# BoxLib-Codes/VARDEN

Measured on AMD Instinct MI355X. Metric: cells*steps/sec on advance_timestep, higher is better.
Workload: dtype f64; 1 GPU; 3D 256x256x256 single-level variable-density bubble, 1 box(es) of 256^3, MAC+HG projection each step (BASELINE.json configs[1]); parallelism=single GPU, cells=16777216

## Files before the change

### varden_amd/csrc/advance.hip

```cpp
#include "vdn_dev.h"
#include <chrono>
#include <cmath>

static double wall() { return std::chrono::duration<double>(std::chrono::steady_clock::now().time_since_epoch()).count(); }
static void sync() { HIPCHK(hipStreamSynchronize(ctx().stream)); }


static void restrict_and_fill(int nlev, vdn_multifab **mf, int icomp, int bcomp, int nc, bool same_boundary, const vdn_bc_tower *bct) {
  if (nlev == 1) mf_restrict_and_fill(mf[0], icomp, bcomp, nc, same_boundary, bct);
  else ml_restrict_and_fill(nlev, mf, icomp, bcomp, nc, same_boundary, bct);
}

static void dbg_phase_hash(const char *tag, int nlevs, vdn_multifab **mfs, int per_level = 1, bool whole = false) {
  if (!sw().phase_hash) return;
  HIPCHK(hipStreamSynchronize(ctx().stream));
  unsigned long long h = 1469598103934665603ull;
  for (int n = 0; n < nlevs; n++) for (int q = 0; q < per_level; q++) {
    const vdn_multifab *m = mfs[per_level == 1 ? n : 3 * n + q];
    if (!m) continue;
    std::vector<unsigned long long> buf(m->bytes / 8);
    HIPCHK(hipMemcpy(buf.data(), m->base, m->bytes, hipMemcpyDeviceToHost));
    for (int b = 0; b < m->nfabs(); b++) {
      const FV &f = m->fabs[b]; vdn_box vb = m->vbox[b];
      if (whole) for (int d = 0; d < 3; d++) { vb.lo[d] -= m->ng; vb.hi[d] += m->ng; }
      const size_t off = (size_t)(f.p - m->base);
      unsigned long long hb = 1469598103934665603ull;
      for (int c = 0; c < m->nc; c++)
        for (int k = vb.lo[2]; k <= vb.hi[2] + m->nodal[2]; k++) for (int j = vb.lo[1]; j <= vb.hi[1] + m->nodal[1]; j++) for (int i = vb.lo[0]; i <= vb.hi[0] + m->nodal[0]; i++) {
          { const unsigned long long v_ = buf[off + (size_t)(i - f.a0) + (size_t)f.n0 * ((size_t)(j - f.a1) + (size_t)f.n1 * (size_t)(k - f.a2)) + (size_t)c * (size_t)f.sc]; hb ^= v_; hb *= 1099511628211ull; }
          const unsigned long long v = buf[off + (size_t)(i - f.a0) + (size_t)f.n0 * ((size_t)(j - f.a1) + (size_t)f.n1 * (size_t)(k - f.a2)) + (size_t)c * (size_t)f.sc];
          h ^= v; h *= 1099511628211ull;
        }
      if (whole) fprintf(stderr, "PHASEBOX %-20s lev %d box %3d (%d,%d,%d)-(%d,%d,%d) %016llx\n", tag, n, b, m->vbox[b].lo[0], m->vbox[b].lo[1], m->vbox[b].lo[2], m->vbox[b].hi[0], m->vbox[b].hi[1], m->vbox[b].hi[2], hb);
    }
  }
  fprintf(stderr, "PHASE %-22s %016llx\n", tag, h);
  if (per_level == 3) {
    for (int n = 0; n < nlevs; n++) for (int q = 0; q < 3; q++) {
      const vdn_multifab *m = mfs[3 * n + q];
      std::vector<unsigned long long> buf(m->bytes / 8);
      HIPCHK(hipMemcpy(buf.data(), m->base, m->bytes, hipMemcpyDeviceToHost));
      for (int b = 0; b < m->nfabs(); b++) {
        const FV &f = m->fabs[b]; const vdn_box &vb = m->vbox[b];
        const size_t off = (size_t)(f.p - m->base);
        unsigned long long hb = 1469598103934665603ull; long nan = 0;
        for (int k = vb.lo[2]; k <= vb.hi[2] + m->nodal[2]; k++) for (int j = vb.lo[1]; j <= vb.hi[1] + m->nodal[1]; j++) for (int i = vb.lo[0]; i <= vb.hi[0] + m->nodal[0]; i++) {
          const unsigned long long v = buf[off + (size_t)(i - f.a0) + (size_t)f.n0 * ((size_t)(j - f.a1) + (size_t)f.n1 * (size_t)(k - f.a2))];
          hb ^= v; hb *= 1099511628211ull;
          double dv; memcpy(&dv, &v, 8); if (dv != dv) nan++;
        }
        fprintf(stderr, "PHASEBOX %-20s lev %d dir %d box %3d (%d,%d,%d)-(%d,%d,%d) %016llx nan %ld\n", tag, n, q, b, vb.lo[0], vb.lo[1], vb.lo[2], vb.hi[0], vb.hi[1], vb.hi[2], hb, nan);
      }
    }
  }
}
extern "C" int vdn_advance_timestep(int istep, vdn_layout *mla, vdn_multifab **sold, vdn_multifab **uold,
                                    vdn_multifab **snew, vdn_multifab **unew, vdn_multifab **gp, vdn_multifab **p,
                                    vdn_multifab **ext_vel_force, vdn_multifab **ext_scal_force,
                                    const vdn_bc_tower *bct, double dt, double time, const double *dx,
                                    int press_comp, int proj_type) {
  VDN_TRY
  (void)istep; (void)time;
  REQUIRE(ctx().inited, "vdn_init has not been called");
  REQUIRE(mla && mla->nlev >= 1 && mla->nlev <= VDN_MAXLEV, "advance_timestep: 1..%d levels are implemented (nlevel = %d)", VDN_MAXLEV, mla ? mla->nlev : -1);
  const vdn_params &P = ctx().prm;
  const int dm = P.dm, nscal = P.nscal, nlevs = mla->nlev;
  const bool viscous = P.visc_coef > 0.0, diffusive = P.diff_coef > 0.0;
  REQUIRE(nlevs == 1 || dm == 3, "advance_timestep: multi-level hierarchies are implemented for dm = 3");
  REQUIRE(press_comp == dm + nscal + 1, "press_comp must be dm+nscal+1 (got %d)", press_comp);
  for (int n = 0; n < nlevs; n++) {
    REQUIRE(uold[n]->ng >= 3 && sold[n]->ng >= 3 && unew[n]->ng >= 3 && snew[n]->ng >= 3, "state needs ng_cell = 3");
    REQUIRE(gp[n]->ng >= 1 && p[n]->ng >= 1 && ext_vel_force[n]->ng >= 1 && ext_scal_force[n]->ng >= 1, "gp/p/ext forces need ng = 1");
    REQUIRE(sold[n]->nc == nscal, "sold must have nscal (= %d) components (got %d)", nscal, sold[n]->nc);
  }
  dbg_phase_hash("uold at entry", nlevs, uold); dbg_phase_hash("sold at entry", nlevs, sold); dbg_phase_hash("gp at entry", nlevs, gp);
  dbg_phase_hash("uold+ghosts at entry", nlevs, uold, 1, true); dbg_phase_hash("sold+ghosts at entry", nlevs, sold, 1, true); dbg_phase_hash("gp+ghosts at entry", nlevs, gp, 1, true);
  Prof prof_advance("advance");
  arena_reset();
  arena_reserve_for(mla);
  const double t_begin = wall();
  #define DXL(n) (dx + (n) * dm)

  vdn_multifab *mac_rhs[VDN_MAXLEV], *rhohalf[VDN_MAXLEV], *umac[3 * VDN_MAXLEV] = { nullptr }, *lapu[VDN_MAXLEV] = { nullptr };
  for (int n = 0; n < nlevs; n++) {
    mac_rhs[n] = mf_temp(mla, n, 1, 1, -1, true, 0.0);
    rhohalf[n] = mf_temp(mla, n, dm, 1, -1, false, 0.0);
    mf_setval(rhohalf[n], 0.0, 0, 1, true);
    for (int d = 0; d < dm; d++) umac[3 * n + d] = mf_temp(mla, n, 1, 1, d, true, 1.e20);
    if (viscous) {
      lapu[n] = mf_temp(mla, n, dm, 0, -1, true, 0.0);
      for (int c = 0; c < dm; c++) k_explicit_diffusive_term(lapu[n], uold[n], c, c, DXL(n), bct);
    }
  }
  if (viscous) for (int n = nlevs - 1; n >= 1; n--) ml_cc_restriction(lapu[n - 1], lapu[n], 0, dm);
  ctx().drop_step_caches();
  if (nlevs == 1 && dm == 3 && god_per_box(uold[0]) && !sw().no_slope_cache) {
    const int nb = uold[0]->nfabs();
    for (int d = 0; d < 3; d++) ctx().slope_cache[d].assign(nb, nullptr);
    ctx().slope_src.assign(nb, nullptr); ctx().macmax_cache.assign(nb, nullptr); ctx().macmax_src.assign(nb, nullptr);
    for (int ib = 0; ib < nb; ib++) {
      const vdn_box &b = uold[0]->vbox[ib];
      const size_t fld = (size_t)(b.hi[0] - b.lo[0] + 3) * (b.hi[1] - b.lo[1] + 3) * (b.hi[2] - b.lo[2] + 3) * sizeof(double);
      for (int d = 0; d < 3; d++) ctx().slope_cache[d][ib] = (double *)arena_alloc(fld * 3);
      ctx().macmax_cache[ib] = (double *)arena_alloc(256);
    }
  }

  const bool force_reuse = !sw().no_force_reuse;
  const bool keep_vel_force = force_reuse && !(viscous && P.diffusion_type == 2);
  vdn_multifab *vel_force0[VDN_MAXLEV] = { nullptr };
  if (keep_vel_force) for (int n = 0; n < nlevs; n++) vel_force0[n] = mf_temp(mla, n, dm, 1, -1, false, 0.0);
  {
    Prof pr("advance_premac");
    size_t mark = arena_mark();
    vdn_multifab *vel_force[VDN_MAXLEV];
    for (int n = 0; n < nlevs; n++) {
      vel_force[n] = keep_vel_force ? vel_force0[n] : mf_temp(mla, n, dm, 1, -1, false, 0.0);
      k_mkvelforce(vel_force[n], ext_vel_force[n], sold[n], gp[n], lapu[n], 1.0);
    }
    restrict_and_fill(nlevs, vel_force, 0, bct->extrap_comp0(), dm, true, bct);
    for (int n = 0; n < nlevs; n++) k_velpred(uold[n], umac + 3 * n, vel_force[n], DXL(n), dt, bct);
    for (int d = 0; d < dm; d++) mf_fill_boundary(umac[d]);
    for (int n = 1; n < nlevs; n++) for (int d = 0; d < dm; d++) { ml_create_umac_grown(umac[3 * n + d], umac[3 * (n - 1) + d], d); mf_fill_boundary(umac[3 * n + d]); }
    for (int n = nlevs - 1; n >= 1; n--) for (int d = 0; d < dm; d++) ml_edge_restriction(umac[3 * (n - 1) + d], umac[3 * n + d], d);
    dbg_phase_hash("vel_force", nlevs, vel_force); dbg_phase_hash("umac after velpred", nlevs, umac, 3);
    if (!keep_vel_force) for (int n = nlevs - 1; n >= 0; n--) mf_temp_free(vel_force[n]);
    arena_release(mark);
  }

  sync(); double t0 = wall();
  { Prof pr("MAC_Project");
  do_macproject(mla, umac, sold, mac_rhs, dx, bct, press_comp - 1);
  }
  sync(); ctx().step_sec[2] = wall() - t0;
  dbg_phase_hash("umac after MAC", nlevs, umac, 3);

  t0 = wall();
  {
    Prof pr("Scalar_update");
    size_t mark = arena_mark();
    int is_cons[VDN_MAXCOMP]; is_cons[0] = 1; for (int c = 1; c < nscal; c++) is_cons[c] = 0;
    vdn_multifab *scal_force[VDN_MAXLEV], *divu[VDN_MAXLEV], *sflux[3 * VDN_MAXLEV], *sedge[3 * VDN_MAXLEV], *laps[VDN_MAXLEV] = { nullptr };
    if (diffusive) {
      for (int n = 0; n < nlevs; n++) {
        laps[n] = mf_temp(mla, n, nscal, 0, -1, true, 0.0);
        for (int c = 1; c < nscal; c++) k_explicit_diffusive_term(laps[n], sold[n], c, dm + c, DXL(n), bct);
      }
      for (int n = nlevs - 1; n >= 1; n--) ml_cc_restriction(laps[n - 1], laps[n], 1, nscal - 1);
    }
    for (int n = 0; n < nlevs; n++) {
      scal_force[n] = mf_temp(mla, n, nscal, 1, -1, false, 0.0);
      divu[n] = mac_rhs[n];
      for (int d = 0; d < dm; d++) { sflux[3 * n + d] = mf_temp(mla, n, nscal, 0, d, nlevs > 1, 0.0); sedge[3 * n + d] = mf_temp(mla, n, nscal, 0, d, false, 0.0); }
      k_mkscalforce(scal_force[n], ext_scal_force[n], laps[n], 1.0);
    }
    restrict_and_fill(nlevs, scal_force, 0, bct->extrap_comp0(), nscal, true, bct);
    bool s_updated = false;
    for (int n = 0; n < nlevs; n++) {
      MkUpdate U; U.snew = snew[n]; U.fmode = 0;
      const bool try_upd = force_reuse && nlevs == 1 && dm == 3 && !diffusive;
      s_updated = k_mkflux(sold[n], sedge + 3 * n, sflux + 3 * n, umac + 3 * n, scal_force[n], divu[n], DXL(n), dt, bct, false, is_cons, try_upd ? &U : nullptr);
      if (diffusive || !force_reuse) k_mkscalforce(scal_force[n], ext_scal_force[n], laps[n], 0.0);
    }
    for (int n = nlevs - 1; n >= 1; n--) for (int c = 0; c < nscal; c++) if (is_cons[c]) for (int d = 0; d < dm; d++) ml_edge_restriction(sflux[3 * (n - 1) + d], sflux[3 * n + d], d, c);
    if (diffusive || !force_reuse) restrict_and_fill(nlevs, scal_force, 0, bct->extrap_comp0(), nscal, true, bct);
    dbg_phase_hash("sedge after mkflux", nlevs, sedge, 3); dbg_phase_hash("sflux restricted", nlevs, sflux, 3); dbg_phase_hash("scal_force", nlevs, scal_force);
    if (!s_updated) for (int n = 0; n < nlevs; n++) k_update(sold[n], umac + 3 * n, sedge + 3 * n, sflux + 3 * n, scal_force[n], snew[n], DXL(n), dt, false, is_cons);
    dbg_phase_hash("snew before r_and_f", nlevs, snew);
    restrict_and_fill(nlevs, snew, 0, dm, nscal, false, bct);
    if (diffusive) {
      const double visc_mu = (P.diffusion_type == 1) ? 0.5 * dt * P.diff_coef : dt * P.diff_coef;
      for (int c = 1; c < nscal; c++) {
        if (nlevs == 1) do_diff_scalar_solve(mla, snew[0], laps[0], dx, visc_mu, bct, c, dm + c);
        else do_ml_diff_scalar_solve(mla, snew, laps, dx, visc_mu, bct, c, dm + c);
      }
    }
    arena_release(mark);
  }
  sync(); ctx().step_sec[0] = wall() - t0;
  dbg_phase_hash("snew after scalars", nlevs, snew);

  { Prof pr("make_at_halftime"); for (int n = 0; n < nlevs; n++) k_make_at_halftime(rhohalf[n], sold[n], snew[n], 0, 0); }
  restrict_and_fill(nlevs, rhohalf, 0, dm + 0, 1, false, bct);
  if (viscous && P.diffusion_type == 2) for (int n = 0; n < nlevs; n++) mf_setval(lapu[n], 0.0, 0, dm, true);

  t0 = wall();
  {
    Prof pr("Velocity_update");
    size_t mark = arena_mark();
    int is_cons[3] = { 0, 0, 0 };
    vdn_multifab *vel_force[VDN_MAXLEV], *uflux[3 * VDN_MAXLEV], *uedge[3 * VDN_MAXLEV];
    for (int n = 0; n < nlevs; n++) {
      vel_force[n] = keep_vel_force ? vel_force0[n] : mf_temp(mla, n, dm, 1, -1, false, 0.0);
      for (int d = 0; d < dm; d++) { uflux[3 * n + d] = mf_temp(mla, n, dm, 0, d, false, 0.0); uedge[3 * n + d] = mf_temp(mla, n, dm, 0, d, false, 0.0); }
      if (!keep_vel_force) k_mkvelforce(vel_force[n], ext_vel_force[n], sold[n], gp[n], lapu[n], 1.0);
    }
    if (!keep_vel_force) restrict_and_fill(nlevs, vel_force, 0, bct->extrap_comp0(), dm, true, bct);
    const bool fuse_force = force_reuse && nlevs == 1 && dm == 3;
    bool u_updated = false;
    for (int n = 0; n < nlevs; n++) {
      MkUpdate U; U.snew = unew[n]; U.fmode = 1; U.ext = ext_vel_force[n]; U.gp = gp[n]; U.rho = rhohalf[n]; U.lapu0 = P.visc_coef * 0.0 * 0.0;
      const bool try_upd = fuse_force && !viscous && P.boussinesq == 0;
      u_updated = k_mkflux(uold[n], uedge + 3 * n, uflux + 3 * n, umac + 3 * n, vel_force[n], mac_rhs[n], DXL(n), dt, bct, true, is_cons, try_upd ? &U : nullptr);
      if (!fuse_force) k_mkvelforce(vel_force[n], ext_vel_force[n], rhohalf[n], gp[n], lapu[n], 0.0);
    }
    dbg_phase_hash("uedge after mkflux", nlevs, uedge, 3); dbg_phase_hash("vel_force (update)", nlevs, vel_force);
    if (u_updated) {  }
    else if (fuse_force) k_update_velforce(uold[0], umac, uedge, ext_vel_force[0], rhohalf[0], gp[0], lapu[0], 0.0, unew[0], DXL(0), dt);
    else {
      restrict_and_fill(nlevs, vel_force, 0, bct->extrap_comp0(), dm, true, bct);
      for (int n = 0; n < nlevs; n++) k_update(uold[n], umac + 3 * n, uedge + 3 * n, uflux + 3 * n, vel_force[n], unew[n], DXL(n), dt, true, is_cons);
    }
    dbg_phase_hash("unew before r_and_f", nlevs, unew);
    restrict_and_fill(nlevs, unew, 0, 0, dm, false, bct);
    dbg_phase_hash("unew after update", nlevs, unew);
    if (viscous) {
      const double visc_mu = (P.diffusion_type == 1) ? 0.5 * dt * P.visc_coef : dt * P.visc_coef;
      if (nlevs == 1) do_visc_solve(mla, unew[0], lapu[0], rhohalf[0], mac_rhs[0], dx, visc_mu, bct);
      else do_ml_visc_solve(mla, unew, lapu, rhohalf, mac_rhs, dx, visc_mu, bct);
    }
    arena_release(mark);
  }
  sync(); ctx().step_sec[1] = wall() - t0;
  dbg_phase_hash("unew after viscous", nlevs, unew);

  t0 = wall();
  { Prof pr("HG_Project");
  do_hgproject(proj_type, mla, unew, uold, rhohalf, p, gp, dx, dt, bct, press_comp - 1); }
  sync(); ctx().step_sec[3] = wall() - t0;
  dbg_phase_hash("unew after HG", nlevs, unew); dbg_phase_hash("p after HG", nlevs, p); dbg_phase_hash("gp after HG", nlevs, gp);
  #undef DXL

  arena_reset();
  ctx().drop_step_caches();
  ctx().step_sec[4] = wall() - t_begin;
  if (P.verbose >= 1 && ctx().rank == 0) {
    printf(" Timing summary:\n Scalar   update: %g seconds\n Velocity update: %g seconds\n  MAC Projection: %g seconds\n   HG Projection: %g seconds\n\n",
           ctx().step_sec[0], ctx().step_sec[1], ctx().step_sec[2], ctx().step_sec[3]);
  }
  VDN_CATCH
}

extern "C" int vdn_estdt(int lev, const vdn_multifab *u, const vdn_multifab *s, const vdn_multifab *gp,
                         const vdn_multifab *ext, const double *dx, double dtold, double *dt_out) {
  VDN_TRY
  (void)lev;
  double m[6];
  k_estdt_max(u, s, gp, ext, m);
  for (int q = 0; q < 6; q++) REQUIRE(m[q] < HUGE_VAL, "estdt: non-finite velocity or pressure-gradient term (the state has blown up)");
  const double eps = (double)1.0e-8f;
  double dt = 1.e20;
  if (m[0] > eps) dt = fmin(dt, dx[0] / m[0]);
  if (m[1] > eps) dt = fmin(dt, dx[1] / m[1]);
  const int dm = ctx().prm.dm;
  if (dm == 3 && m[2] > eps) dt = fmin(dt, dx[2] / m[2]);
  if (m[3] > eps) dt = fmin(dt, sqrt(2.0 * dx[0] / m[3]));
  if (m[4] > eps) dt = fmin(dt, sqrt(2.0 * dx[1] / m[4]));
  if (dm == 3 && m[5] > eps) dt = fmin(dt, sqrt(2.0 * dx[2] / m[5]));
  if (dt == 1.e20) { dt = fmin(dx[0], dx[1]); if (dm == 3) dt = fmin(dt, dx[2]); }
  dt = dt * ctx().prm.cflfac;
  if (dtold > 0.0) dt = fmin(dt, ctx().prm.max_dt_growth * dtold);
  *dt_out = dt;
  VDN_CATCH
}

extern "C" int vdn_hgproject(int proj_type, vdn_layout *mla, vdn_multifab **unew, vdn_multifab **uold,
                             vdn_multifab **rhohalf, vdn_multifab **p, vdn_multifab **gp,
                             const double *dx, double dt, const vdn_bc_tower *bct, int press_comp) {
  VDN_TRY
  REQUIRE(mla && mla->nlev <= VDN_MAXLEV, "hgproject: at most %d levels are implemented (nlevel = %d)", VDN_MAXLEV, mla ? mla->nlev : -1);
  arena_reset(); arena_reserve_for(mla);
  do_hgproject(proj_type, mla, unew, uold, rhohalf, p, gp, dx, dt, bct, press_comp - 1);
  arena_reset();
  VDN_CATCH
}
extern "C" int vdn_macproject(vdn_layout *mla, vdn_multifab **umac, vdn_multifab **rho, vdn_multifab **mac_rhs,
                              const double *dx, const vdn_bc_tower *bct, int bc_comp) {
  VDN_TRY
  REQUIRE(mla && mla->nlev <= VDN_MAXLEV, "macproject: at most %d levels are implemented (nlevel = %d)", VDN_MAXLEV, mla ? mla->nlev : -1);
  arena_reset(); arena_reserve_for(mla);
  do_macproject(mla, umac, rho, mac_rhs, dx, bct, bc_comp - 1);
  arena_reset();
  VDN_CATCH
}

#define HOOK_BEGIN(mf) VDN_TRY REQUIRE(ctx().inited, "vdn_init has not been called"); arena_reset(); arena_reserve_for((mf)->la);
#define HOOK_END arena_reset(); VDN_CATCH

extern "C" int vdn_k_slope(const vdn_multifab *s, vdn_multifab *slope, int dir, int bccomp, const vdn_bc_tower *bct) {
  HOOK_BEGIN(s) k_slope(s, slope, dir, bccomp, bct); HOOK_END
}
extern "C" int vdn_k_velpred(const vdn_multifab *u, vdn_multifab **umac, const vdn_multifab *force, const double *dx, double dt,
                             const vdn_bc_tower *bct) {
  HOOK_BEGIN(u)
  k_velpred(u, umac, force, dx, dt, bct);
  for (int d = 0; d < ctx().prm.dm; d++) mf_fill_boundary(umac[d]);
  HOOK_END
}
extern "C" int vdn_k_mkflux(const vdn_multifab *s, vdn_multifab **sedge, vdn_multifab **flux, vdn_multifab **umac,
                            const vdn_multifab *force, const vdn_multifab *mac_rhs, const double *dx, double dt,
                            const vdn_bc_tower *bct, int is_vel, const int *is_cons) {
  HOOK_BEGIN(s) k_mkflux(s, sedge, flux, umac, force, mac_rhs, dx, dt, bct, is_vel != 0, is_cons); HOOK_END
}
extern "C" int vdn_k_update(const vdn_multifab *sold, vdn_multifab **umac, vdn_multifab **sedge, vdn_multifab **flux,
                            const vdn_multifab *force, vdn_multifab *snew, const double *dx, double dt,
                            int is_vel, const int *is_cons, const vdn_bc_tower *bct) {
  HOOK_BEGIN(sold)
  k_update(sold, umac, sedge, flux, force, snew, dx, dt, is_vel != 0, is_cons);
  mf_restrict_and_fill(snew, 0, is_vel ? 0 : bct->dm, snew->nc, false, bct);
  HOOK_END
}
extern "C" int vdn_k_mkvelforce(vdn_multifab *vf, const vdn_multifab *ext, const vdn_multifab *s, const vdn_multifab *gp,
                                const vdn_multifab *lapu, double visc_fac, const vdn_bc_tower *bct) {
  HOOK_BEGIN(vf)
  k_mkvelforce(vf, ext, s, gp, lapu, visc_fac);
  mf_restrict_and_fill(vf, 0, bct->extrap_comp0(), vf->nc, true, bct);
  HOOK_END
}
// ... 71 lines not shown
```

### varden_amd/csrc/mg_cc.hip

```cpp
#include "vdn_dev.h"
#include "mg_stop.h"
#include "krylov_wg.h"
#include "krylov_grid.h"
#include <chrono>
#include <tuple>
#include <algorithm>

struct CLev {
  int n[3]; int PX, PY; long sz;
  double hi2[3];
  double *phi, *rh, *res, *b[3];
  double *alpha;
  const double *rho;
  int fold[3][2];
  double cmu;
};
DEVI long cidx(const CLev &L, int i, int j, int k) { return (long)(i + 16) + (long)L.PX * ((long)(j + 1) + (long)L.PY * (long)(k + 1)); }

DEVI double beta_of(double ra, double rb, bool at_face, int e) {
  double v = 2.0 / (ra + rb);
  if (at_face) { if (e == VDN_BC_NEU) v = 0.0; else if (e == VDN_BC_DIR) v = 2.0 * v; }
  return v;
}
template <bool RHO = false> DEVI void cc_apply(const CLev &L, long c, double &Ap, double &diag, int i = 0, int j = 0, int k = 0) {
// ... 868 lines not shown
  const long sy = F.PX, sz = (long)F.PX * F.PY;
  const long f = cidx(F, 2 * i, 2 * j, 2 * k);
  double s = src[f] + src[f + 1] + src[f + sy] + src[f + sy + 1] + src[f + sz] + src[f + sz + 1] + src[f + sz + sy] + src[f + sz + sy + 1];
  dst[cidx(C, i, j, k)] = s * 0.125;
}

__global__ void kk_cc_store(CLev L, FV phi, int lo0, int lo1, int lo2, int ebc00, int ebc01, int ebc10, int ebc11, int ebc20, int ebc21, int add = 0, FV acc = FV()) {
  const int i = (int)(blockIdx.x * blockDim.x + threadIdx.x) - 1;
  const int j = (int)(blockIdx.y * blockDim.y + threadIdx.y) - 1;
  const int k = (int)blockIdx.z - 1;
  if (i > L.n[0] || j > L.n[1] || k > L.n[2]) return;
  const int out = (i < 0) + (i == L.n[0]) + (j < 0) + (j == L.n[1]) + (k < 0) + (k == L.n[2]);
  if (out > 1) return;
  double v;
  if (out == 0) v = L.phi[cidx(L, i, j, k)];
  else {
    int e; int qi = i, qj = j, qk = k;
    if (i < 0) { e = ebc00; qi = 0; } else if (i == L.n[0]) { e = ebc01; qi = L.n[0] - 1; }
    else if (j < 0) { e = ebc10; qj = 0; } else if (j == L.n[1]) { e = ebc11; qj = L.n[1] - 1; }
    else if (k < 0) { e = ebc20; qk = 0; } else { e = ebc21; qk = L.n[2] - 1; }
    if (e == VDN_BC_NEU) v = L.phi[cidx(L, qi, qj, qk)];
    else if (e == VDN_BC_DIR) v = -L.phi[cidx(L, qi, qj, qk)];
    else v = L.phi[cidx(L, i, j, k)];
  }
  fv_at(phi, lo0 + i, lo1 + j, lo2 + k) = v;
  if (add && out == 0) fv_at(acc, lo0 + i, lo1 + j, lo2 + k) = fv_get(acc, lo0 + i, lo1 + j, lo2 + k) + v;
}


__global__ void kk_cc_restrict_pack(CLev F, const double *r, double *buf, long off, int nx, int ny, int nz) {
  const int i = blockIdx.x * blockDim.x + threadIdx.x;
  const int j = blockIdx.y * blockDim.y + threadIdx.y;
  const int k = blockIdx.z;
  if (i >= nx || j >= ny) return;
  const long sy = F.PX, sz = (long)F.PX * F.PY;
  const long f = cidx(F, 2 * i, 2 * j, 2 * k);
  double s = r[f] + r[f + 1] + r[f + sy] + r[f + sy + 1] + r[f + sz] + r[f + sz + 1] + r[f + sz + sy] + r[f + sz + sy + 1];
  buf[off + i + (long)nx * (j + (long)ny * k)] = s * 0.125;
}
__global__ void kk_cc_coarsen_b_pack(CLev F, double *buf, long off, int nx, int ny, int nz) {
  const int i = blockIdx.x * blockDim.x + threadIdx.x;
  const int j = blockIdx.y * blockDim.y + threadIdx.y;
  const int k = blockIdx.z;
  if (i > nx || j > ny || k > nz) return;
  const long sy = F.PX, sz = (long)F.PX * F.PY;
  const long f = cidx(F, 2 * i, 2 * j, 2 * k);
  const long o1 = off + (long)(nx + 1) * ny * nz, o2 = o1 + (long)nx * (ny + 1) * nz;
  if (j < ny && k < nz) buf[off + i + (long)(nx + 1) * (j + (long)ny * k)] = (F.b[0][f] + F.b[0][f + sy] + F.b[0][f + sz] + F.b[0][f + sz + sy]) * 0.25;
  if (i < nx && k < nz) buf[o1 + i + (long)nx * (j + (long)(ny + 1) * k)] = (F.b[1][f] + F.b[1][f + 1] + F.b[1][f + sz] + F.b[1][f + sz + 1]) * 0.25;
  if (i < nx && j < ny) buf[o2 + i + (long)nx * (j + (long)ny * k)] = (F.b[2][f] + F.b[2][f + 1] + F.b[2][f + sy] + F.b[2][f + sy + 1]) * 0.25;
}
__global__ void kk_cc_unpack_rh(CLev T, double *dst, const double *buf, const GBox *gb) {
  const GBox g = gb[blockIdx.z];
  const int tot = g.n[0] * g.n[1] * g.n[2];
  for (int t = blockIdx.x * blockDim.x + threadIdx.x; t < tot; t += gridDim.x * blockDim.x) {
    const int i = t % g.n[0], j = (t / g.n[0]) % g.n[1], k = t / (g.n[0] * g.n[1]);
    const long cc = cidx(T, g.c0[0] + i, g.c0[1] + j, g.c0[2] + k);
    dst[cc] = buf[g.off + t];
    T.phi[cc] = 0.0;
  }
}
__global__ void kk_cc_unpack_b(CLev T, const double *buf, const GBox *gb) {
  const GBox g = gb[blockIdx.z];
  const int nx = g.n[0], ny = g.n[1], nz = g.n[2];
  const long n0 = (long)(nx + 1) * ny * nz, n1 = (long)nx * (ny + 1) * nz, n2 = (long)nx * ny * (nz + 1);
  for (long t = blockIdx.x * blockDim.x + threadIdx.x; t < n0 + n1 + n2; t += gridDim.x * blockDim.x) {
    int d; long u = t;
    if (u < n0) d = 0; else if (u < n0 + n1) { d = 1; u -= n0; } else { d = 2; u -= n0 + n1; }
    const int ex = nx + (d == 0), ey = ny + (d == 1);
    const int i = (int)(u % ex), j = (int)((u / ex) % ey), k = (int)(u / ((long)ex * ey));
    T.b[d][cidx(T, g.c0[0] + i, g.c0[1] + j, g.c0[2] + k)] = buf[g.off + t];
  }
}
__global__ void kk_cc_prolong_tail(CLev F, CLev T, int c00, int c01, int c02) {
  const int i = blockIdx.x * blockDim.x + threadIdx.x;
  const int j = blockIdx.y * blockDim.y + threadIdx.y;
  const int k = blockIdx.z;
  if (i >= F.n[0] || j >= F.n[1]) return;
  const long f = cidx(F, i, j, k);
  F.phi[f] = F.phi[f] + T.phi[cidx(T, c00 + (i >> 1), c01 + (j >> 1), c02 + (k >> 1))];
}

struct ProlongLinArgs { int c0[3]; int e[3][2]; };
__global__ void kk_cc_prolong_lin(CLev F, CLev C, ProlongLinArgs A) {
  const int i = blockIdx.x * blockDim.x + threadIdx.x;
  const int j = blockIdx.y * blockDim.y + threadIdx.y;
  const int k = blockIdx.z;
  if (i >= F.n[0] || j >= F.n[1]) return;
  const int I = A.c0[0] + (i >> 1), J = A.c0[1] + (j >> 1), K = A.c0[2] + (k >> 1);
  const long sy = C.PX, sz = (long)C.PX * C.PY;
  const long c = cidx(C, I, J, K);
  const double p0 = C.phi[c];
  double px, py, pz;
  #define NBV(out, q, odd, n, elo, ehi, stride)                                                             \
    { const int m = (q) + ((odd) ? 1 : -1);                                                                 \
      const int t = m < 0 ? (elo) : (m >= (n) ? (ehi) : VDN_BC_INT);                                         \
      out = (t == VDN_BC_NEU) ? p0 : ((t == VDN_BC_DIR) ? -p0 : C.phi[c + ((odd) ? (stride) : -(stride))]); }
  NBV(px, I, i & 1, C.n[0], A.e[0][0], A.e[0][1], 1L)
  NBV(py, J, j & 1, C.n[1], A.e[1][0], A.e[1][1], sy)
  NBV(pz, K, k & 1, C.n[2], A.e[2][0], A.e[2][1], sz)
  #undef NBV
  F.phi[cidx(F, i, j, k)] = 0.25 * (((p0 + px) + py) + pz);
}

struct CBox { CLev L; int lo[3]; int gidx; int hmask = 63;
              CSplit sp;  };
struct CDLev { std::vector<CBox> boxes; XPlan *halo = nullptr; int ng[3];  bool single_box = false;
               bool res_restricted = false;
               bool split = false;
               XPlan *shalo[2] = { nullptr, nullptr };
               std::vector<XBoxInfo> xb; vdn_box lpd; unsigned long la_uid = 0; int la_lev = 0;       };
struct CCMG {
  std::vector<CDLev> dlev;
  std::vector<CLev> tail;
  int per[3];
  double *d_nrm;
  MgGather g_rh, g_b; GBox *d_gb_rh = nullptr, *d_gb_b = nullptr;
  double *sendbuf = nullptr, *recvbuf = nullptr;
  MgKrylov kry; int kry_singular = 0;
  CcKrylov krylov(const CLev &L) const { return CcKrylov{ L, { per[0], per[1], per[2] }, kry_singular }; }
};

static dim3 g3(int nx, int ny, int nz, dim3 b) { return dim3((nx + b.x - 1) / b.x, (ny + b.y - 1) / b.y, nz); }
static const dim3 BLK(64, 4, 1);

template <int ADD> static inline void launch_gsrb_split(const CBox &B, int color, hipStream_t st, const CLev &C, int k0 = 0, int k1 = -1, int hm = 0) {
  const CLev &L = B.L;
  if (k1 < 0) k1 = L.n[2];
  const dim3 g((unsigned)((L.n[0] / 4 + 63) / 64), (unsigned)((L.n[1] + 7) / 8), (unsigned)(k1 - k0));
  if (L.cmu > 0.0) hipLaunchKernelGGL((kk_cc_gsrb_rho_split<ADD, true>), g, dim3(64, 8, 1), 0, st, L, B.sp, color, C, (sw().mac_kflip && color) ? 1 : 0, k0, hm);
  else hipLaunchKernelGGL((kk_cc_gsrb_rho_split<ADD, false>), g, dim3(64, 8, 1), 0, st, L, B.sp, color, C, (sw().mac_kflip && color) ? 1 : 0, k0, hm);
}
static inline void launch_residual_split_rst(const CLev &L, const CSplit &S, double *nrm, const CLev &C, int Ka, int Kb, hipStream_t st) {
  const dim3 g((unsigned)((L.n[0] / 4 + 63) / 64), (unsigned)((L.n[1] / 2 + 3) / 4), (unsigned)std::min(Kb - Ka, 16));
  if (L.cmu > 0.0) hipLaunchKernelGGL(kk_cc_residual_rho_split_rst<true>, g, BLK, 0, st, L, S, nrm, C, Ka, Kb);
  else hipLaunchKernelGGL(kk_cc_residual_rho_split_rst<false>, g, BLK, 0, st, L, S, nrm, C, Ka, Kb);
}
static inline void launch_gsrb_split_shell(const CBox &B, int color, hipStream_t st, int hm) {
  if (!hm) return;
  const CLev &L = B.L;
  const int m = std::max(L.n[0], std::max(L.n[1], L.n[2]));
  hipLaunchKernelGGL(kk_cc_gsrb_split_shell, dim3((unsigned)((m + 63) / 64), (unsigned)((m + 3) / 4), (unsigned)__builtin_popcount(hm)), dim3(64, 4, 1), 0, st, L, B.sp, color, hm);
}
static void cc_to_split(const CDLev &DL, int what) {
  for (const CBox &B : DL.boxes) {
    const CLev &L = B.L;
    const dim3 g((unsigned)((B.sp.PXH + 63) / 64), (unsigned)((L.n[1] + 2 + 3) / 4), (unsigned)(L.n[2] + 2));
    hipLaunchKernelGGL(kk_cc_to_split, g, BLK, 0, ctx().stream, L, B.sp, what);
  }
}
static void cc_from_split(const CDLev &DL) {
  for (const CBox &B : DL.boxes) hipLaunchKernelGGL(kk_cc_from_split, g3(B.L.n[0] / 2, B.L.n[1], B.L.n[2], BLK), BLK, 0, ctx().stream, B.L, B.sp);
}
static void split_halo(const CDLev &DL, int colour, hipStream_t st = nullptr) { if (DL.shalo[colour]) xplan_run(DL.shalo[colour], st); }
static bool cc_split_ok(const CCMG &M) {
  if (!sw().mac_split || !sw().mg_restrict_fused || !sw().mg_prolong_fused || M.dlev.size() < 2 || ctx().prm.mg_nu1 < 1 || ctx().prm.mg_nu2 < 1) return false;
  const CDLev &D0 = M.dlev[0];
  if (D0.boxes.empty() || D0.boxes.size() != M.dlev[1].boxes.size()) return false;
  long cells = 0;
  for (const CBox &B : D0.boxes) {
    const CLev &L = B.L;
    if (!((L.rho || (L.cmu > 0.0 && L.alpha)) && cc_pair_level_z(L) && L.n[0] % 4 == 0)) return false;
    for (int d = 0; d < 3; d++) if (B.lo[d] & 1) return false;
    cells += (long)L.n[0] * L.n[1] * L.n[2];
  }
  for (int d = 0; d < 3; d++) if (D0.ng[d] & 1) return false;
  return cells >= sw().mac_split_min;
}
static int g_mac_level_form = 0;
extern "C" int vdn_last_mac_level_form(void) { return g_mac_level_form; }
static XPlan *cc_split_plan(const CDLev &D0, int colour, const int per[3]);
static void cc_split_setup(CCMG &M) {
  CDLev &D0 = M.dlev[0];
  for (CBox &B : D0.boxes) {
    const CLev &L = B.L;
    CSplit &S = B.sp;
    const int off = 16, rnd = 16;
    S.off = off;
    S.PXH = ((L.n[0] / 2 + off + 2 + rnd - 1) / rnd) * rnd; S.sy = S.PXH; S.sz = (long)S.PXH * (L.n[1] + 2); S.tot = S.sz * (L.n[2] + 2);
    double *base = (double *)arena_alloc(sizeof(double) * S.tot * 6);
    for (int c = 0; c < 2; c++) { S.phi[c] = base + c * S.tot; S.rh[c] = base + (2 + c) * S.tot; S.rho[c] = base + (4 + c) * S.tot; }
  }
  D0.split = true;
  if (D0.halo) for (int c = 0; c < 2; c++) D0.shalo[c] = cc_split_plan(D0, c, M.per);
  cc_to_split(D0, 2 | 4);
// ... 24 lines not shown
static const int CC_HALO = 4;

static XPlan *cc_split_plan(const CDLev &D0, int colour, const int per[3]) {
  std::vector<XBoxInfo> xb = D0.xb;
  size_t li = 0;
  GraphKey hk;
  for (XBoxInfo &x : xb) {
    const int nh = (x.vhi[0] - x.vlo[0] + 1) / 2;
    x.vlo[0] /= 2; x.vhi[0] = x.vlo[0] + nh - 1;
    if (x.owner == ctx().rank) {
      const CBox &B = D0.boxes[li++];
      const CSplit &S = B.sp;
      FV f; f.p = S.phi[colour]; f.a0 = x.vlo[0] - S.off; f.a1 = x.vlo[1] - 1; f.a2 = x.vlo[2] - 1; f.n0 = S.PXH; f.n1 = B.L.n[1] + 2; f.n2 = B.L.n[2] + 2; f.sc = S.tot;
      x.fv = f; hk.put(f.p); hk.put(S.tot);
    }
  }
  vdn_box lpd = D0.lpd; lpd.hi[0] = (lpd.hi[0] + 1) / 2 - 1;
  const MgHaloKey key{ D0.la_uid, (const void *)D0.boxes[0].sp.phi[colour], D0.la_lev, 1000 + colour, CC_HALO, per[0] | (per[1] << 1) | (per[2] << 2), hk.h };
  return mg_halo_plan(key, xb, lpd, per, sw().cc_halo_faces);
}

int mg_agglom(const vdn_layout *la, int lev) {
  if (sw().mg_agglom > 0) return sw().mg_agglom;
  bool all_local = true;
  for (int o : la->owner[lev]) if (o != ctx().rank) all_local = false;
  return (all_local && !comm_active()) ? 128 : 64;
}

MgPlan mg_plan_of(const vdn_layout *la, int lev) {
  return mg_plan(la->boxes[lev].data(), la->owner[lev].data(), (int)la->boxes[lev].size(), la->pd[lev], ctx().nranks, ctx().rank, mg_agglom(la, lev));
}
static void cc_build(CCMG &M, const vdn_multifab *rh, const double *dx, const int bc[3][2], bool has_alpha) {
  Prof prof_("cc_build");
  const vdn_layout *la = rh->la; const int lev = rh->lev;
  const int nb = (int)la->boxes[lev].size();
  for (int d = 0; d < 3; d++) M.per[d] = (bc[d][0] == VDN_BC_PER);
  const MgPlan P = mg_plan_of(la, lev);
  REQUIRE(P.err.empty(), "cc multigrid: %s", P.err.c_str());
  double h[3] = { dx[0], dx[1], dx[2] };
  for (const MgDistLevel &PL : P.dist) {
    const int *n = PL.n;
    CDLev DL;
    std::vector<XBoxInfo> xb;
    for (int g = 0; g < nb; g++) {
      XBoxInfo x; memset(&x, 0, sizeof x);
      const int *lo = PL.lo[g].data();
      for (int d = 0; d < 3; d++) { x.vlo[d] = lo[d]; x.vhi[d] = lo[d] + n[d] - 1; }
      x.owner = la->owner[lev][g];
      if (x.owner == ctx().rank) {
        CBox B; B.L = cc_alloc_lev(n, h, has_alpha); B.gidx = g;
        for (int d = 0; d < 3; d++) B.lo[d] = lo[d];
        x.fv = cc_phi_view(B.L, lo);
        DL.boxes.push_back(B);
      }
      xb.push_back(x);
    }
    vdn_box lpd; for (int d = 0; d < 3; d++) { lpd.lo[d] = 0; lpd.hi[d] = PL.ng[d] - 1; DL.ng[d] = PL.ng[d]; }
    for (CBox &B : DL.boxes) {
      B.hmask = 0;
      for (int d = 0; d < 3; d++) {
        if (B.lo[d] > 0 || M.per[d]) B.hmask |= 1 << (2 * d);
        if (B.lo[d] + B.L.n[d] < DL.ng[d] || M.per[d]) B.hmask |= 2 << (2 * d);
      }
    }
    if (nb > 1 || M.per[0] || M.per[1] || M.per[2]) {
      GraphKey hk; for (const CBox &B : DL.boxes) { hk.put(B.L.phi); hk.put(B.L.sz); }
      const MgHaloKey key{ la->uid, DL.boxes.empty() ? nullptr : (const void *)DL.boxes[0].L.phi, lev, (int)M.dlev.size(), CC_HALO, M.per[0] | (M.per[1] << 1) | (M.per[2] << 2), hk.h };
      DL.halo = mg_halo_plan(key, xb, lpd, M.per, sw().cc_halo_faces);
    }
    DL.single_box = (nb == 1);
    DL.xb = xb; DL.lpd = lpd; DL.la_uid = la->uid; DL.la_lev = lev;
    M.dlev.push_back(DL);
    for (int d = 0; d < 3; d++) h[d] *= 2.0;
  }
  if (!P.tail.empty()) {
    for (const auto &tn : P.tail) {
      M.tail.push_back(cc_alloc_lev(tn.data(), h, has_alpha));
      for (int d = 0; d < 3; d++) h[d] *= 2.0;
    }
    const int *cn = P.cn;
    M.g_rh = P.gather((long)cn[0] * cn[1] * cn[2]);
    M.g_b = P.gather((long)(cn[0] + 1) * cn[1] * cn[2] + (long)cn[0] * (cn[1] + 1) * cn[2] + (long)cn[0] * cn[1] * (cn[2] + 1));
    M.d_gb_rh = (GBox *)arena_alloc(nb * sizeof(GBox)); M.d_gb_b = (GBox *)arena_alloc(nb * sizeof(GBox));
    HIPCHK(hipMemcpyAsync(M.d_gb_rh, M.g_rh.gb.data(), nb * sizeof(GBox), hipMemcpyHostToDevice, ctx().stream));
    HIPCHK(hipMemcpyAsync(M.d_gb_b, M.g_b.gb.data(), nb * sizeof(GBox), hipMemcpyHostToDevice, ctx().stream));
    HIPCHK(hipStreamSynchronize(ctx().stream));
    M.sendbuf = (double *)arena_alloc(sizeof(double) * M.g_b.cnt);
    M.recvbuf = (double *)arena_alloc(sizeof(double) * M.g_b.cnt * ctx().nranks);
  }
  M.d_nrm = (double *)arena_alloc(256);
  const int method = mg_krylov_method(ctx().prm.mg_bottom_solver);
  if (method && P.whole_bottom) {
    const CLev &B = !M.tail.empty() ? M.tail.back() : M.dlev.back().boxes[0].L;
    bool dir = false;
    for (int d = 0; d < 3; d++) for (int sd = 0; sd < 2; sd++) if (bc[d][sd] == VDN_BC_DIR) dir = true;
    M.kry_singular = (!has_alpha && !dir) ? 1 : 0;
    GraphKey k; k.put(0); k.put(method); k.put(B.n); k.put(has_alpha); k.put(M.kry_singular); k.put(ctx().prm.mg_bottom_solver_eps);
    mg_krylov_setup(M.kry, method, B.sz, std::max(B.n[0], std::max(B.n[1], B.n[2])), (long)B.n[0] * B.n[1] * B.n[2], k);
  }
}
static void cc_halo(CCMG &M, CDLev &DL) { if (DL.halo) xplan_run(DL.halo); }
static const long SMALL_LEVEL_CELLS = 8L * 8 * 8;
static void cc_gsrb_d(CCMG &M, CDLev &DL, int nsweeps) {
  if (DL.single_box && DL.boxes.size() == 1 && (long)DL.ng[0] * DL.ng[1] * DL.ng[2] <= SMALL_LEVEL_CELLS) {
    hipLaunchKernelGGL(kk_cc_bottom, dim3(1), dim3(1024), 0, ctx().stream, DL.boxes[0].L, nsweeps, M.per[0], M.per[1], M.per[2]);
    return;
  }
  const int ov_env = sw().overlap;
  static const long ov_min = 1L << 20;
  bool overlap = DL.halo && (ov_env == 1 || (ov_env != 0 && xplan_has_remote(DL.halo)));
  if (overlap) {
    long cells = 0;
    for (const CBox &B : DL.boxes) cells = std::max(cells, (long)B.L.n[0] * B.L.n[1] * B.L.n[2]);
    if (cells < ov_min && ov_env != 1) overlap = false;
  }
  VdnCtx &c = ctx();
  if (DL.split) {
    for (int s = 0; s < nsweeps; s++) for (int color = 0; color < 2; color++) {
      if (!overlap) {
        split_halo(DL, 1 - color);
        for (const CBox &B : DL.boxes) launch_gsrb_split<0>(B, color, c.stream, B.L);
        continue;
      }
      HIPCHK(hipEventRecord(c.ev_main, c.stream));
      HIPCHK(hipStreamWaitEvent(c.halo_stream, c.ev_main, 0));
      split_halo(DL, 1 - color, c.halo_stream);
      HIPCHK(hipEventRecord(c.ev_halo, c.halo_stream));
      for (const CBox &B : DL.boxes) launch_gsrb_split<0>(B, color, c.stream, B.L, 0, -1, B.hmask);
      HIPCHK(hipStreamWaitEvent(c.stream, c.ev_halo, 0));
      for (const CBox &B : DL.boxes) launch_gsrb_split_shell(B, color, c.stream, B.hmask);
    }
    return;
  }
  for (int s = 0; s < nsweeps; s++) for (int color = 0; color < 2; color++) {
    if (!overlap) {
      cc_halo(M, DL);
      for (const CBox &B : DL.boxes) launch_gsrb(B.L, (color + B.lo[0] + B.lo[1] + B.lo[2]) & 1, c.stream);
      continue;
    }
    HIPCHK(hipEventRecord(c.ev_main, c.stream));
    HIPCHK(hipStreamWaitEvent(c.halo_stream, c.ev_main, 0));
    xplan_run(DL.halo, c.halo_stream);
    HIPCHK(hipEventRecord(c.ev_halo, c.halo_stream));
    for (const CBox &B : DL.boxes) launch_gsrb(B.L, (color + B.lo[0] + B.lo[1] + B.lo[2]) & 1, c.stream, B.hmask);
    HIPCHK(hipStreamWaitEvent(c.stream, c.ev_halo, 0));
    for (const CBox &B : DL.boxes) launch_gsrb_shell(B.L, (color + B.lo[0] + B.lo[1] + B.lo[2]) & 1, c.stream, B.hmask);
  }
}
static void cc_residual_d(CCMG &M, CDLev &DL, bool norm, bool reduce = true) {
  if (norm) HIPCHK(hipMemsetAsync(M.d_nrm, 0, sizeof(double), ctx().stream));
  DL.res_restricted = false;
  if (DL.split) {
    split_halo(DL, 1);
    for (size_t b = 0; b < DL.boxes.size(); b++) {
      const CBox &B = DL.boxes[b]; const CLev &L = B.L;
      launch_residual_split_rst(L, B.sp, norm ? M.d_nrm : nullptr, M.dlev[1].boxes[b].L, 0, L.n[2] / 2, ctx().stream);
    }
    DL.res_restricted = true;
    if (norm && reduce) comm_allreduce_max_dev(M.d_nrm, 1);
    return;
  }
  cc_halo(M, DL);
  {
    const size_t l = &DL - &M.dlev[0];
    if (sw().mg_restrict_fused && DL.single_box && DL.boxes.size() == 1 && l + 1 < M.dlev.size() && M.dlev[l + 1].boxes.size() == 1) {
      const CLev &L = DL.boxes[0].L;
      if (L.rho && cc_pair_level_z(L)) {
        const dim3 g((unsigned)((L.n[0] / 2 + 63) / 64), (unsigned)((L.n[1] / 2 + 3) / 4), (unsigned)std::min(L.n[2] / 2, 16));
        hipLaunchKernelGGL(kk_cc_residual_rho_pair_rst, g, BLK, 0, ctx().stream, L, norm ? M.d_nrm : nullptr, M.dlev[l + 1].boxes[0].L);
        DL.res_restricted = true;
        if (norm && reduce) comm_allreduce_max_dev(M.d_nrm, 1);
        return;
      }
    }
  }
  for (const CBox &B : DL.boxes) {
    const dim3 g = g3(B.L.n[0], B.L.n[1], norm ? std::min(B.L.n[2], 16) : B.L.n[2], BLK);
    if (B.L.rho && cc_pair_level(B.L))
      hipLaunchKernelGGL(kk_cc_residual_rho_pair, dim3((unsigned)((B.L.n[0] / 2 + 63) / 64), (unsigned)((B.L.n[1] / 2 + 3) / 4), g.z), BLK, 0, ctx().stream, B.L, norm ? M.d_nrm : nullptr);
    else if (B.L.rho) hipLaunchKernelGGL(kk_cc_residual_rho, g, BLK, 0, ctx().stream, B.L, norm ? M.d_nrm : nullptr);
    else hipLaunchKernelGGL(kk_cc_residual, g, BLK, 0, ctx().stream, B.L, norm ? M.d_nrm : nullptr);
  }
  if (norm && reduce) comm_allreduce_max_dev(M.d_nrm, 1);
}

static void cc_periodic_t(const CCMG &M, const CLev &L) {
  if (!(M.per[0] || M.per[1] || M.per[2])) return;
  int m = std::max(L.n[0], std::max(L.n[1], L.n[2]));
  hipLaunchKernelGGL(kk_cc_periodic, g3(m, m, 6, BLK), BLK, 0, ctx().stream, L, M.per[0], M.per[1], M.per[2]);
}
static void cc_gsrb_t(const CCMG &M, const CLev &L, int nsweeps) {
  if ((long)L.n[0] * L.n[1] * L.n[2] <= SMALL_LEVEL_CELLS) {
    hipLaunchKernelGGL(kk_cc_bottom, dim3(1), dim3(1024), 0, ctx().stream, L, nsweeps, M.per[0], M.per[1], M.per[2]);
    return;
  }
  for (int s = 0; s < nsweeps; s++) for (int color = 0; color < 2; color++) {
    cc_periodic_t(M, L);
    launch_gsrb(L, color, ctx().stream);
  }
}
static void cc_bottom_t(const CCMG &M, const CLev &L) {
  if (M.kry.w) { mg_krylov_visit(M.kry, 0, ctx().prm.mg_bottom_solver_eps, M.krylov(L)); return; }
  const int N = std::max(L.n[0], std::max(L.n[1], L.n[2]));
  const int ns = std::max(ctx().prm.mg_nub, N * N);
  hipLaunchKernelGGL(kk_cc_bottom, dim3(1), dim3(1024), 0, ctx().stream, L, ns, M.per[0], M.per[1], M.per[2]);
}
static bool cc_small_end(const CCMG &M, int dl, int tl) {
  if (!sw().mg_tailcycle) return false;
  static const long tail_cells = SMALL_LEVEL_CELLS;
  const vdn_params &P = ctx().prm;
  CcTailArgs T; memset(&T, 0, sizeof T);
  int nl = 0;
  if (dl >= 0) {
    if (!M.tail.empty() && !(ctx().nranks == 1 && M.dlev.back().single_box)) return false;
    for (int m = dl; m < (int)M.dlev.size(); m++) {
      const CDLev &D = M.dlev[m];
      if (!(D.single_box && D.boxes.size() == 1 && !D.boxes[0].L.rho && (long)D.ng[0] * D.ng[1] * D.ng[2] <= tail_cells) || nl == CC_TAIL_MAX) return false;
      T.L[nl++] = D.boxes[0].L;
    }
  }
  for (int m = tl; m < (int)M.tail.size(); m++) {
    const CLev &L = M.tail[m];
    if ((long)L.n[0] * L.n[1] * L.n[2] > tail_cells || nl == CC_TAIL_MAX) return false;
    T.L[nl++] = L;
  }
  if (nl < 2) return false;
  const CLev &B = T.L[nl - 1];
  const int N = std::max(B.n[0], std::max(B.n[1], B.n[2]));
  T.nlev = nl; T.nu1 = P.mg_nu1; T.nu2 = P.mg_nu2; T.nbot = std::max(P.mg_nub, N * N);
  for (int d = 0; d < 3; d++) T.per[d] = M.per[d];
  if (M.kry.w) hipLaunchKernelGGL(kk_cc_tailcycle<true>, dim3(1), dim3(1024), 0, ctx().stream, T, KrylovTailArgs{ mg_krylov_args(M.kry, 0, P.mg_bottom_solver_eps), M.kry.method, M.kry_singular });
  else hipLaunchKernelGGL(kk_cc_tailcycle<false>, dim3(1), dim3(1024), 0, ctx().stream, T, NoKrylovTailArgs{});
  return true;
// ... 9 lines not shown
static void cc_vcycle_t(const CCMG &M, int l) {
  const vdn_params &P = ctx().prm;
  if (cc_small_end(M, -1, l)) return;
  const CLev &L = M.tail[l];
  if (l == (int)M.tail.size() - 1) { cc_bottom_t(M, L); return; }
  const CLev &C = M.tail[l + 1];
  if (cc_lds_tail_level(M, l)) {
    const dim3 g((unsigned)(L.n[0] / LT), (unsigned)(L.n[1] / LT), (unsigned)(L.n[2] / LT));
    if (L.alpha) hipLaunchKernelGGL(kk_cc_lds_down<true>, g, dim3(1024), 0, ctx().stream, L, C);
    else hipLaunchKernelGGL(kk_cc_lds_down<false>, g, dim3(1024), 0, ctx().stream, L, C);
    cc_vcycle_t(M, l + 1);
    if (L.alpha) hipLaunchKernelGGL(kk_cc_lds_up<true>, g, dim3(1024), 0, ctx().stream, L, C);
    else hipLaunchKernelGGL(kk_cc_lds_up<false>, g, dim3(1024), 0, ctx().stream, L, C);
    return;
  }
  cc_gsrb_t(M, L, P.mg_nu1);
  cc_periodic_t(M, L);
  hipLaunchKernelGGL(kk_cc_residual, g3(L.n[0], L.n[1], L.n[2], BLK), BLK, 0, ctx().stream, L, (double *)nullptr);
  hipLaunchKernelGGL(kk_cc_restrict, g3(C.n[0], C.n[1], C.n[2], BLK), BLK, 0, ctx().stream, L, C);
  cc_vcycle_t(M, l + 1);
  hipLaunchKernelGGL(kk_cc_prolong, g3(L.n[0], L.n[1], L.n[2], BLK), BLK, 0, ctx().stream, L, C);
  cc_gsrb_t(M, L, P.mg_nu2);
}

static void cc_restrict_down(CCMG &M, int l) {
  CDLev &DL = M.dlev[l];
  if (DL.res_restricted) { DL.res_restricted = false; return; }
  if (l + 1 < (int)M.dlev.size()) {
    CDLev &DC = M.dlev[l + 1];
    for (size_t b = 0; b < DL.boxes.size(); b++) {
      const CLev &C = DC.boxes[b].L;
      hipLaunchKernelGGL(kk_cc_restrict, g3(C.n[0], C.n[1], C.n[2], BLK), BLK, 0, ctx().stream, DL.boxes[b].L, C);
    }
  } else {
    const CLev &T = M.tail[0];
    for (size_t b = 0; b < DL.boxes.size(); b++) {
      const CLev &F = DL.boxes[b].L;
      const int nx = F.n[0] / 2, ny = F.n[1] / 2, nz = F.n[2] / 2;
      hipLaunchKernelGGL(kk_cc_restrict_pack, g3(nx, ny, nz, BLK), BLK, 0, ctx().stream, F, (const double *)F.res, M.sendbuf, M.g_rh.loc_off[b], nx, ny, nz);
    }
    comm_allgather_dev(M.sendbuf, M.recvbuf, M.g_rh.cnt);
    hipLaunchKernelGGL(kk_cc_unpack_rh, dim3(4, 1, (unsigned)M.g_rh.gb.size()), dim3(256), 0, ctx().stream, T, T.rh, M.recvbuf, M.d_gb_rh);
  }
}
static void cc_prolong_up(CCMG &M, int l) {
  CDLev &DL = M.dlev[l];
  for (size_t b = 0; b < DL.boxes.size(); b++) {
    const CBox &B = DL.boxes[b];
    if (l + 1 < (int)M.dlev.size())
      hipLaunchKernelGGL(kk_cc_prolong, g3(B.L.n[0], B.L.n[1], B.L.n[2], BLK), BLK, 0, ctx().stream, B.L, M.dlev[l + 1].boxes[b].L);
    else
      hipLaunchKernelGGL(kk_cc_prolong_tail, g3(B.L.n[0], B.L.n[1], B.L.n[2], BLK), BLK, 0, ctx().stream, B.L, M.tail[0], B.lo[0] / 2, B.lo[1] / 2, B.lo[2] / 2);
  }
}
static void cc_prolong_smooth(CCMG &M, int l, int nsweeps) {
  CDLev &DL = M.dlev[l];
  if (DL.split) {
    if (DL.halo) cc_halo(M, M.dlev[l + 1]);
    for (size_t b = 0; b < DL.boxes.size(); b++) launch_gsrb_split<1>(DL.boxes[b], 0, ctx().stream, M.dlev[l + 1].boxes[b].L);
    split_halo(DL, 0);
    for (size_t b = 0; b < DL.boxes.size(); b++) launch_gsrb_split<2>(DL.boxes[b], 1, ctx().stream, M.dlev[l + 1].boxes[b].L);
    if (nsweeps > 1) cc_gsrb_d(M, DL, nsweeps - 1);
    return;
  }
  const bool ok = sw().mg_prolong_fused && nsweeps >= 1 && DL.single_box && DL.boxes.size() == 1 && !DL.halo && l + 1 < (int)M.dlev.size() && M.dlev[l + 1].boxes.size() == 1 &&
                  !(M.per[0] || M.per[1] || M.per[2]) && DL.boxes[0].L.rho && cc_pair_level_z(DL.boxes[0].L);
  if (!ok) { cc_prolong_up(M, l); cc_gsrb_d(M, DL, nsweeps); return; }
  const CLev &L = DL.boxes[0].L, &C = M.dlev[l + 1].boxes[0].L;
  const dim3 g((unsigned)((L.n[0] / 2 + 63) / 64), (unsigned)((L.n[1] / 2 + 3) / 4), (unsigned)L.n[2]), blk(64, 4, 1);
  hipLaunchKernelGGL(kk_cc_gsrb_rho_pair_t<1>, g, blk, 0, ctx().stream, L, 0, 0, C, 0);
  hipLaunchKernelGGL(kk_cc_gsrb_rho_pair_t<2>, g, blk, 0, ctx().stream, L, 1, 0, C, sw().mac_kflip ? 1 : 0);
  if (nsweeps > 1) cc_gsrb_d(M, DL, nsweeps - 1);
}
static int mac_slab(const CLev &L) {
  if (sw().mac_slab >= 0) return sw().mac_slab;
  const long fit = (long)(200.0e6 / (24.0 * L.n[0] * L.n[1]));
  return (int)std::max(8L, std::min((long)(L.n[2] + 1) / 2, fit));
}
static void cc_split_run(CCMG &M, CDLev &DL, bool prolong, int nsweeps, bool residual, bool norm, bool reduce) {
  const CBox &B0 = DL.boxes[0];
  const CLev &L = B0.L, &C = M.dlev[1].boxes[0].L;
  hipStream_t st = ctx().stream;
  const int R = 2 * nsweeps, n2 = L.n[2], nK = n2 / 2, slab = mac_slab(L);
  if (residual && norm) HIPCHK(hipMemsetAsync(M.d_nrm, 0, sizeof(double), st));
  DL.res_restricted = false;
  std::vector<int> done(R + 1, 0);
  for (int top = slab + R; ; top += slab) {
    for (int p = 0; p < R; p++) {
      const int hi = p == 0 ? std::min(top, n2) : (done[p - 1] == n2 ? n2 : done[p - 1] - 1);
      if (hi <= done[p]) continue;
      const int add = prolong ? (p == 0 ? 1 : p == 1 ? 2 : 0) : 0;
      if (add == 1) launch_gsrb_split<1>(B0, p & 1, st, C, done[p], hi);
      else if (add == 2) launch_gsrb_split<2>(B0, p & 1, st, C, done[p], hi);
      else launch_gsrb_split<0>(B0, p & 1, st, L, done[p], hi);
      done[p] = hi;
    }
    if (residual) {
      const int hiK = done[R - 1] == n2 ? nK : std::max(0, (done[R - 1] - 1) / 2);
      if (hiK > done[R]) {
        launch_residual_split_rst(L, B0.sp, norm ? M.d_nrm : nullptr, C, done[R], hiK, st);
        done[R] = hiK;
      }
    }
    if (done[R - 1] == n2 && (!residual || done[R] == nK)) break;
  }
  if (residual) { DL.res_restricted = true; if (norm && reduce) comm_allreduce_max_dev(M.d_nrm, 1); }
}
static void cc_fine_seq(CCMG &M, bool after_coarse, bool residual, bool norm, bool reduce = true) {
  const vdn_params &P = ctx().prm;
  CDLev &D0 = M.dlev[0];
  if (D0.split && !D0.halo && D0.boxes.size() == 1 && mac_slab(D0.boxes[0].L) > 0 && residual) { cc_split_run(M, D0, after_coarse, (after_coarse ? P.mg_nu2 : 0) + P.mg_nu1, true, norm, reduce); return; }
  if (after_coarse) cc_prolong_smooth(M, 0, P.mg_nu2);
  cc_gsrb_d(M, D0, P.mg_nu1);
  if (residual) cc_residual_d(M, D0, norm, reduce);
}
static bool cc_lds_level(const CCMG &M, int l) {
  static const int nmax_ = 64;
  const vdn_params &P = ctx().prm;
  if (!sw().mg_lds || l < 1 || l + 1 >= (int)M.dlev.size() || P.mg_nu1 != 2 || P.mg_nu2 != 2 || M.per[0] || M.per[1] || M.per[2]) return false;
  const CDLev &D = M.dlev[l], &DC = M.dlev[l + 1];
  if (!(D.single_box && D.boxes.size() == 1 && !D.halo && DC.single_box && DC.boxes.size() == 1)) return false;
  const CLev &L = D.boxes[0].L;
  if (L.rho) return false;
  for (int d = 0; d < 3; d++) if (L.n[d] % LT || L.n[d] < 2 * LT || L.n[d] > nmax_ || D.boxes[0].lo[d] != 0 || DC.boxes[0].L.n[d] * 2 != L.n[d]) return false;
  return true;
}
static void cc_vcycle_d(CCMG &M, int l) {
  const vdn_params &P = ctx().prm;
  CDLev &DL = M.dlev[l];
  const bool last = (l == (int)M.dlev.size() - 1);
  if (cc_small_end(M, l, 0)) return;
  if (last && M.tail.empty()) {
    if (M.kry.w && DL.single_box && DL.boxes.size() == 1) {
      mg_krylov_visit(M.kry, 0, P.mg_bottom_solver_eps, M.krylov(DL.boxes[0].L));
      return;
    }
    const int N = std::max(DL.ng[0], std::max(DL.ng[1], DL.ng[2]));
    cc_gsrb_d(M, DL, std::max(P.mg_nub, N * N));
    return;
  }
  if (!last && cc_lds_level(M, l)) {
    const CLev &L = DL.boxes[0].L, &C = M.dlev[l + 1].boxes[0].L;
    const dim3 g((unsigned)(L.n[0] / LT), (unsigned)(L.n[1] / LT), (unsigned)(L.n[2] / LT));
    if (L.alpha) hipLaunchKernelGGL(kk_cc_lds_down<true>, g, dim3(1024), 0, ctx().stream, L, C);
    else hipLaunchKernelGGL(kk_cc_lds_down<false>, g, dim3(1024), 0, ctx().stream, L, C);
    cc_vcycle_d(M, l + 1);
    if (L.alpha) hipLaunchKernelGGL(kk_cc_lds_up<true>, g, dim3(1024), 0, ctx().stream, L, C);
    else hipLaunchKernelGGL(kk_cc_lds_up<false>, g, dim3(1024), 0, ctx().stream, L, C);
    return;
  }
  cc_gsrb_d(M, DL, P.mg_nu1);
  cc_residual_d(M, DL, false);
  cc_restrict_down(M, l);
  if (last) cc_vcycle_t(M, 0); else cc_vcycle_d(M, l + 1);
  cc_prolong_smooth(M, l, P.mg_nu2);
}

static long cc_level_cells(const CCMG &M, int g) {
  const int nd = (int)M.dlev.size();
  if (g < nd) return (long)M.dlev[g].ng[0] * M.dlev[g].ng[1] * M.dlev[g].ng[2];
  const CLev &T = M.tail[g - nd];
  return (long)T.n[0] * T.n[1] * T.n[2];
}
static void cc_cycle_at(CCMG &M, int g) {
  const vdn_params &P = ctx().prm;
  const int nd = (int)M.dlev.size();
  if (g < nd) {
    CDLev &DL = M.dlev[g];
    cc_gsrb_d(M, DL, P.mg_nu1);
    cc_residual_d(M, DL, false);
    cc_restrict_down(M, g);
    if (g + 1 < nd) cc_vcycle_d(M, g + 1); else cc_vcycle_t(M, 0);
    cc_prolong_up(M, g); cc_gsrb_d(M, DL, P.mg_nu2);
    return;
  }
  const CLev &L = M.tail[g - nd], &C = M.tail[g - nd + 1];
  cc_gsrb_t(M, L, P.mg_nu1);
  cc_periodic_t(M, L);
  hipLaunchKernelGGL(kk_cc_residual, g3(L.n[0], L.n[1], L.n[2], BLK), BLK, 0, ctx().stream, L, (double *)nullptr);
  hipLaunchKernelGGL(kk_cc_restrict, g3(C.n[0], C.n[1], C.n[2], BLK), BLK, 0, ctx().stream, L, C);
  cc_vcycle_t(M, g - nd + 1);
  hipLaunchKernelGGL(kk_cc_prolong, g3(L.n[0], L.n[1], L.n[2], BLK), BLK, 0, ctx().stream, L, C);
  cc_gsrb_t(M, L, P.mg_nu2);
}
static void cc_fmg(CCMG &M, const int bc[3][2]) {
  const int nd = (int)M.dlev.size(), ntot = nd + (int)M.tail.size();
  int ls = -1;
  for (int g = 1; g < ntot; g++) if (cc_level_cells(M, g) >= 4096) ls = g;
  if (ls < 1 || ls + 1 >= ntot) return;
  hipStream_t st = ctx().stream;
  for (int g = 0; g < ls; g++) {
    if (g + 1 < nd) {
      for (size_t b = 0; b < M.dlev[g].boxes.size(); b++) {
        CLev F = M.dlev[g].boxes[b].L; F.res = F.rh;
        const CLev &C = M.dlev[g + 1].boxes[b].L;
        hipLaunchKernelGGL(kk_cc_restrict, g3(C.n[0], C.n[1], C.n[2], BLK), BLK, 0, st, F, C);
      }
    } else if (g + 1 == nd) {
      const CDLev &DL = M.dlev[g]; const CLev &T = M.tail[0];
      for (size_t b = 0; b < DL.boxes.size(); b++) {
        const CLev &F = DL.boxes[b].L;
        const int nx = F.n[0] / 2, ny = F.n[1] / 2, nz = F.n[2] / 2;
        hipLaunchKernelGGL(kk_cc_restrict_pack, g3(nx, ny, nz, BLK), BLK, 0, st, F, (const double *)F.rh, M.sendbuf, M.g_rh.loc_off[b], nx, ny, nz);
      }
      comm_allgather_dev(M.sendbuf, M.recvbuf, M.g_rh.cnt);
      hipLaunchKernelGGL(kk_cc_unpack_rh, dim3(4, 1, (unsigned)M.g_rh.gb.size()), dim3(256), 0, st, T, T.rh, M.recvbuf, M.d_gb_rh);
    } else {
      CLev F = M.tail[g - nd]; F.res = F.rh;
      const CLev &C = M.tail[g - nd + 1];
      hipLaunchKernelGGL(kk_cc_restrict, g3(C.n[0], C.n[1], C.n[2], BLK), BLK, 0, st, F, C);
    }
  }
  if (ls < nd) cc_vcycle_d(M, ls); else cc_vcycle_t(M, ls - nd);
  cc_cycle_at(M, ls);
  for (int g = ls - 1; g >= 0; g--) {
    if (g + 1 < nd) {
      CDLev &DC = M.dlev[g + 1];
      cc_halo(M, DC);
      for (size_t b = 0; b < M.dlev[g].boxes.size(); b++) {
        const CLev &F = M.dlev[g].boxes[b].L; const CBox &CB = DC.boxes[b];
        ProlongLinArgs A;
        for (int d = 0; d < 3; d++) { A.c0[d] = 0; A.e[d][0] = (CB.lo[d] == 0) ? bc[d][0] : VDN_BC_INT; A.e[d][1] = (CB.lo[d] + CB.L.n[d] == DC.ng[d]) ? bc[d][1] : VDN_BC_INT; }
        hipLaunchKernelGGL(kk_cc_prolong_lin, g3(F.n[0], F.n[1], F.n[2], BLK), BLK, 0, st, F, CB.L, A);
      }
    } else {
      const CLev &T = M.tail[g + 1 - nd];
      cc_periodic_t(M, T);
      ProlongLinArgs A;
      for (int d = 0; d < 3; d++) { A.c0[d] = 0; A.e[d][0] = bc[d][0]; A.e[d][1] = bc[d][1]; }
      if (g >= nd) { const CLev &F = M.tail[g - nd]; hipLaunchKernelGGL(kk_cc_prolong_lin, g3(F.n[0], F.n[1], F.n[2], BLK), BLK, 0, st, F, T, A); }
      else for (const CBox &B : M.dlev[g].boxes) {
        for (int d = 0; d < 3; d++) A.c0[d] = B.lo[d] / 2;
        hipLaunchKernelGGL(kk_cc_prolong_lin, g3(B.L.n[0], B.L.n[1], B.L.n[2], BLK), BLK, 0, st, B.L, T, A);
      }
    }
    if (g > 0) cc_cycle_at(M, g);
  }
}

struct CcKeep { bool built = false; CCMG M; };
CcKeep *cc_keep_new() { return new CcKeep; }
void cc_keep_free(CcKeep *k) { delete k; }

static void cc_key_lev(GraphKey &k, const CLev &L) {
  k.put(L.n); k.put(L.PX); k.put(L.PY); k.put(L.sz); k.put(L.hi2); k.put(L.phi); k.put(L.rh); k.put(L.res); k.put(L.b); k.put(L.alpha);
  k.put(L.rho); k.put(L.fold); k.put(L.cmu);
}
static unsigned long long cc_graph_key(const CCMG &M, int what) {
  const vdn_params &P = ctx().prm;
  GraphKey k; k.put(what); k.put(P.mg_nu1); k.put(P.mg_nu2); k.put(P.mg_nub); k.put(M.per); k.put(M.d_nrm);
  k.put(M.sendbuf); k.put(M.recvbuf); k.put(M.d_gb_rh); k.put(M.d_gb_b); k.put(M.g_rh.cnt); k.put(M.g_b.cnt);
  for (const CDLev &DL : M.dlev) {
    k.put(xplan_serial(DL.halo)); k.put(DL.ng); k.put(DL.single_box); k.put(DL.res_restricted);
    k.put(DL.split); k.put(xplan_serial(DL.shalo[0])); k.put(xplan_serial(DL.shalo[1]));
    for (const CBox &B : DL.boxes) { cc_key_lev(k, B.L); k.put(B.lo); if (DL.split) { k.put(B.sp.PXH); k.put(B.sp.off); k.put(B.sp.phi); k.put(B.sp.rh); k.put(B.sp.rho); } }
  }
  for (const CLev &L : M.tail) cc_key_lev(k, L);
  for (long o : M.g_rh.loc_off) k.put(o);
  if (M.kry.w) { k.put(M.kry.w); k.put(M.kry.method); k.put(M.kry_singular); k.put(M.kry.maxit); k.put(P.mg_bottom_solver_eps); }
  if (M.kry.part) { k.put(M.kry.part); k.put(M.kry.budget); }
  return k.h;
}
template <class Body> static void cc_run_cycle(CCMG &M, int what, Body body) {
  if (!graphs_enabled()) { body(); return; }
  const unsigned long long key = cc_graph_key(M, what);
  if (graph_replay(key)) return;
  graph_begin();
  try { body(); } catch (...) { graph_abort(); throw; }
  graph_end(key);
}

static int cc_fmg_what(const int bc[3][2]) {
  int code = 0;
  for (int d = 0; d < 3; d++) for (int sd = 0; sd < 2; sd++) code = code * 4 + (bc[d][sd] + 1);
  return 3 + 4 * code;
}
struct CcFaces { int e[3][2]; };
static CcFaces cc_domain_faces(const vdn_multifab *mf, size_t b, const int bc[3][2]) {
  const vdn_box &bx = mf->vbox[b], &pd = mf->la->pd[mf->lev];
  CcFaces F;
  for (int d = 0; d < 3; d++) {
    F.e[d][0] = (bx.lo[d] == pd.lo[d]) ? bc[d][0] : VDN_BC_INT;
    F.e[d][1] = (bx.hi[d] == pd.hi[d]) ? bc[d][1] : VDN_BC_INT;
  }
  return F;
}
static void cc_coarsen_coeffs(CCMG &M, bool has_alpha, bool from_rho) {
  for (size_t l = 1; l < M.dlev.size(); l++)
    for (size_t b = 0; b < M.dlev[l].boxes.size(); b++) {
      const CLev &F = M.dlev[l - 1].boxes[b].L, &C = M.dlev[l].boxes[b].L;
      if (l == 1 && from_rho) hipLaunchKernelGGL(kk_cc_coarsen_b_rho, g3(C.n[0] + 1, C.n[1] + 1, C.n[2] + 1, BLK), BLK, 0, ctx().stream, F, C);
      else hipLaunchKernelGGL(kk_cc_coarsen_b, g3(C.n[0] + 1, C.n[1] + 1, C.n[2] + 1, BLK), BLK, 0, ctx().stream, F, C);
      if (has_alpha) hipLaunchKernelGGL(kk_cc_coarsen_cell, g3(C.n[0], C.n[1], C.n[2], BLK), BLK, 0, ctx().stream, F, (const double *)F.alpha, C, C.alpha);
    }
  if (M.tail.empty()) return;
  CDLev &DL = M.dlev.back();
  for (size_t b = 0; b < DL.boxes.size(); b++) {
    const CLev &F = DL.boxes[b].L;
    const int nx = F.n[0] / 2, ny = F.n[1] / 2, nz = F.n[2] / 2;
    hipLaunchKernelGGL(kk_cc_coarsen_b_pack, g3(nx + 1, ny + 1, nz + 1, BLK), BLK, 0, ctx().stream, F, M.sendbuf, M.g_b.loc_off[b], nx, ny, nz);
  }
  comm_allgather_dev(M.sendbuf, M.recvbuf, M.g_b.cnt);
  hipLaunchKernelGGL(kk_cc_unpack_b, dim3(4, 1, (unsigned)M.g_b.gb.size()), dim3(256), 0, ctx().stream, M.tail[0], M.recvbuf, M.d_gb_b);
  if (has_alpha) {
    for (size_t b = 0; b < DL.boxes.size(); b++) {
      const CLev &F = DL.boxes[b].L;
      const int nx = F.n[0] / 2, ny = F.n[1] / 2, nz = F.n[2] / 2;
      hipLaunchKernelGGL(kk_cc_restrict_pack, g3(nx, ny, nz, BLK), BLK, 0, ctx().stream, F, (const double *)F.alpha, M.sendbuf, M.g_rh.loc_off[b], nx, ny, nz);
    }
    comm_allgather_dev(M.sendbuf, M.recvbuf, M.g_rh.cnt);
    hipLaunchKernelGGL(kk_cc_unpack_rh, dim3(4, 1, (unsigned)M.g_rh.gb.size()), dim3(256), 0, ctx().stream, M.tail[0], M.tail[0].alpha, M.recvbuf, M.d_gb_rh);
  }
  for (size_t l = 1; l < M.tail.size(); l++) {
    const CLev &C = M.tail[l];
    hipLaunchKernelGGL(kk_cc_coarsen_b, g3(C.n[0] + 1, C.n[1] + 1, C.n[2] + 1, BLK), BLK, 0, ctx().stream, M.tail[l - 1], C);
    if (has_alpha) hipLaunchKernelGGL(kk_cc_coarsen_cell, g3(C.n[0], C.n[1], C.n[2], BLK), BLK, 0, ctx().stream, M.tail[l - 1], (const double *)M.tail[l - 1].alpha, C, C.alpha);
  }
}
static void cc_setup(CCMG &M, vdn_multifab *rh, vdn_multifab *phi, const vdn_multifab *alpha, vdn_multifab **beta, const double *dx, const int bc[3][2],
                     const vdn_multifab *rho = nullptr, double const_beta = 0.0) {
  REQUIRE(phi->ng >= 1, "cc multigrid: phi needs one ghost cell");
  cc_build(M, rh, dx, bc, alpha != nullptr);
  CDLev &D0 = M.dlev[0];
  const bool from_rho = rho && !alpha && !sw().mac_stored_beta && rho->ng >= 1;
  for (size_t b = 0; b < D0.boxes.size(); b++) {
    CLev &L0 = D0.boxes[b].L;
    const vdn_box &bx = rh->vbox[b];
    const CcFaces F = cc_domain_faces(rh, b, bc);
    const auto &e = F.e;
    hipLaunchKernelGGL(kk_cc_load, g3(L0.n[0] + 1, L0.n[1] + 1, L0.n[2] + 1, BLK), BLK, 0, ctx().stream, L0, rh->fabs[b], phi->fabs[b],
                       alpha ? alpha->fabs[b] : rh->fabs[b], beta[0]->fabs[b], beta[1]->fabs[b], beta[2]->fabs[b], bx.lo[0], bx.lo[1], bx.lo[2],
                       e[0][0], e[0][1], e[1][0], e[1][1], e[2][0], e[2][1]);
    hipLaunchKernelGGL(kk_cc_load_rh, g3(L0.n[0], L0.n[1], L0.n[2], BLK), BLK, 0, ctx().stream, L0, rh->fabs[b], phi->fabs[b],
                       bx.lo[0], bx.lo[1], bx.lo[2], e[0][0], e[0][1], e[1][0], e[1][1], e[2][0], e[2][1]);
    if (from_rho) {
      double *r = (double *)arena_alloc(sizeof(double) * L0.sz);
      hipLaunchKernelGGL(kk_cc_load_rho, g3(L0.n[0] + 2, L0.n[1] + 2, L0.n[2] + 2, BLK), BLK, 0, ctx().stream, L0, r, rho->fabs[b], bx.lo[0], bx.lo[1], bx.lo[2]);
      L0.rho = r;
      for (int d = 0; d < 3; d++) { L0.fold[d][0] = e[d][0]; L0.fold[d][1] = e[d][1]; }
    }
    if (const_beta > 0.0 && alpha) {
      L0.cmu = const_beta;
      for (int d = 0; d < 3; d++) { L0.fold[d][0] = e[d][0]; L0.fold[d][1] = e[d][1]; }
    }
  }
  cc_coarsen_coeffs(M, alpha != nullptr, false);
}
static double cc_setup_fast(CCMG &M, CcFast *fast, const double *dx, const int bc[3][2]) {
  const vdn_multifab *rho = fast->rho;
  cc_build(M, rho, dx, bc, false);
  REQUIRE(M.dlev.size() >= 2, "cc_setup_fast: needs a second distributed level");
  CDLev &D0 = M.dlev[0];
  HIPCHK(hipMemsetAsync(M.d_nrm, 0, sizeof(double), ctx().stream));
  for (size_t b = 0; b < D0.boxes.size(); b++) {
    CLev &L0 = D0.boxes[b].L;
    const vdn_box &bx = rho->vbox[b];
    const CcFaces F = cc_domain_faces(rho, b, bc);
    const auto &e = F.e;
    double *r = (double *)arena_alloc(sizeof(double) * L0.sz);
    hipLaunchKernelGGL(kk_cc_load_rho, g3(L0.n[0] + 2, L0.n[1] + 2, L0.n[2] + 2, BLK), BLK, 0, ctx().stream, L0, r, rho->fabs[b], bx.lo[0], bx.lo[1], bx.lo[2]);
    L0.rho = r;
    for (int d = 0; d < 3; d++) { L0.fold[d][0] = e[d][0]; L0.fold[d][1] = e[d][1]; }
    hipLaunchKernelGGL(kk_cc_load_divumac, g3(L0.n[0], L0.n[1], std::min(L0.n[2], 16), BLK), BLK, 0, ctx().stream, L0, fast->um[0]->fabs[b], fast->um[1]->fabs[b], fast->um[2]->fabs[b],
                       fast->mac_rhs->fabs[b], 1.0 / dx[0], 1.0 / dx[1], 1.0 / dx[2], bx.lo[0], bx.lo[1], bx.lo[2], e[0][0], e[0][1], e[1][0], e[1][1], e[2][0], e[2][1], M.d_nrm);
  }
  comm_allreduce_max_dev(M.d_nrm, 1);
  const double bnorm = read_scalar1(M.d_nrm);
  cc_coarsen_coeffs(M, false, true);
  return bnorm;
}
static void cc_reload(CCMG &M, vdn_multifab *rh, vdn_multifab *phi, const int bc[3][2], bool zero_guess = false) {
  CDLev &D0 = M.dlev[0];
  for (size_t b = 0; b < D0.boxes.size(); b++) {
    CLev &L0 = D0.boxes[b].L;
    const vdn_box &bx = rh->vbox[b];
    const CcFaces F = cc_domain_faces(rh, b, bc);
    const auto &e = F.e;
    if (zero_guess) { if (!D0.split) HIPCHK(hipMemsetAsync(L0.phi, 0, sizeof(double) * L0.sz, ctx().stream)); }
    else hipLaunchKernelGGL(kk_cc_load_phi, g3(L0.n[0], L0.n[1], L0.n[2], BLK), BLK, 0, ctx().stream, L0, phi->fabs[b], bx.lo[0], bx.lo[1], bx.lo[2]);
    hipLaunchKernelGGL(kk_cc_load_rh, g3(L0.n[0], L0.n[1], L0.n[2], BLK), BLK, 0, ctx().stream, L0, rh->fabs[b], phi->fabs[b],
                       bx.lo[0], bx.lo[1], bx.lo[2], e[0][0], e[0][1], e[1][0], e[1][1], e[2][0], e[2][1], zero_guess ? 1 : 0);
  }
  if (D0.split) {
    cc_to_split(D0, zero_guess ? 2 : 3);
    if (zero_guess) for (const CBox &B : D0.boxes) HIPCHK(hipMemsetAsync(B.sp.phi[0], 0, sizeof(double) * 2 * B.sp.tot, ctx().stream));
  }
}
static void cc_store(CCMG &M, vdn_multifab *phi, const int bc[3][2], vdn_multifab *add_to = nullptr) {
  CDLev &D0 = M.dlev[0];
  cc_halo(M, D0);
  for (size_t b = 0; b < D0.boxes.size(); b++) {
    const CLev &L0 = D0.boxes[b].L;
    const vdn_box &bx = phi->vbox[b];
    const CcFaces F = cc_domain_faces(phi, b, bc);
    const auto &e = F.e;
    hipLaunchKernelGGL(kk_cc_store, g3(L0.n[0] + 2, L0.n[1] + 2, L0.n[2] + 2, BLK), BLK, 0, ctx().stream, L0, phi->fabs[b],
                       bx.lo[0], bx.lo[1], bx.lo[2], e[0][0], e[0][1], e[1][0], e[1][1], e[2][0], e[2][1], add_to ? 1 : 0, add_to ? add_to->fabs[b] : phi->fabs[b]);
  }
}

static void cc_coarse_correction(CCMG &M) {
  cc_restrict_down(M, 0);
  if (M.dlev.size() > 1) cc_vcycle_d(M, 1); else cc_vcycle_t(M, 0);
}
int cc_solve(CcRequest &q) {
  Prof prof_("mac_multigrid");
  if (ctx().prm.dm == 2) return cc2_solve(q);
  const vdn_params &P = ctx().prm;
  CcKeep *keep = q.keep; CcFast *fast = q.fast;
  const bool fixed = q.fixed_cycles > 0;
  REQUIRE(q.dx && q.bc && q.fixed_cycles >= 0, "cc_solve: dx, bc and fixed_cycles >= 0");
  if (fast) REQUIRE(!keep && !q.alpha && !fixed && fast->rho && fast->rho->ng >= 1, "cc_solve: bad use of the fast path");
  else REQUIRE(q.rh && q.phi && q.beta, "cc_solve: rh, phi and beta");
  size_t mark = arena_mark();
  CCMG M_local;
  CCMG &M = keep ? keep->M : M_local;
  double bnorm_fast = 0.0;
  if (fast) {
    bnorm_fast = cc_setup_fast(M, fast, q.dx, q.bc);
    if (cc_split_ok(M)) cc_split_setup(M);
    g_mac_level_form = M.dlev[0].split ? 1 : 0;
  }
  else if (keep && keep->built) { cc_reload(M, q.rh, q.phi, q.bc, q.zero_guess); g_mac_level_form = M.dlev[0].split ? 1 : 0; }
  else {
    cc_setup(M, q.rh, q.phi, q.alpha, q.beta, q.dx, q.bc, q.rho, q.const_beta);
    g_mac_level_form = 0;
    if (keep && fixed && (!q.alpha || q.const_beta > 0.0) && cc_split_ok(M)) { cc_split_setup(M); cc_to_split(M.dlev[0], 1); g_mac_level_form = 1; }
    else if (!keep && !fixed && q.alpha && q.const_beta > 0.0 && cc_split_ok(M)) { cc_split_setup(M); g_mac_level_form = 1; }
  }
  if (!fixed || !(keep && keep->built)) mg_krylov_begin(M.kry, 0, M.kry.w != nullptr);
  if (keep) keep->built = true;
  CDLev &D0 = M.dlev[0];
  const bool single = (M.dlev.size() == 1 && M.tail.empty());
  const int nbot = std::max(P.mg_nub, std::max(D0.ng[0], std::max(D0.ng[1], D0.ng[2])) * std::max(D0.ng[0], std::max(D0.ng[1], D0.ng[2])));
  if (fixed) {
    for (int c = 0; c < q.fixed_cycles; c++) {
      if (single) { cc_gsrb_d(M, D0, nbot); continue; }
      cc_run_cycle(M, 2, [&] {
        const bool slabs = D0.split && !D0.halo && D0.boxes.size() == 1 && mac_slab(D0.boxes[0].L) > 0;
        if (slabs) cc_split_run(M, D0, false, P.mg_nu1, true, false, false);
        else { cc_gsrb_d(M, D0, P.mg_nu1); cc_residual_d(M, D0, false); }
        cc_coarse_correction(M);
        if (slabs) cc_split_run(M, D0, true, P.mg_nu2, false, false, false);
        else cc_prolong_smooth(M, 0, P.mg_nu2);
      });
    }
    if (D0.split) cc_from_split(D0);
    cc_store(M, q.phi, q.bc, q.add_to);
    q.cycles = q.fixed_cycles; q.res0 = 0.0; q.res = 0.0;
    if (!keep) arena_release(mark);
    return 0;
  }
  const double bnorm = fast ? bnorm_fast : mf_norm_inf(q.rh, 0, 1);
  const bool fmg = fast ? P.mac_fmg != 0 : q.fmg;
  if (fmg && bnorm != 0.0 && !single && bnorm < HUGE_VAL) cc_run_cycle(M, cc_fmg_what(q.bc), [&] { cc_fmg(M, q.bc); });
  if (D0.split) cc_to_split(D0, 1);
  const int gn[3] = { D0.ng[0], D0.ng[1], D0.ng[2] };
  const MgStop s = mg_stop_loop(0, gn, fast && !single && bnorm < HUGE_VAL, fast && !single, q, bnorm, M.d_nrm,
    [&](bool blind) {
      if (single) cc_gsrb_d(M, D0, nbot); else cc_fine_seq(M, false, blind, true, false);
      if (!blind) cc_residual_d(M, D0, true);
    },
    [&] {
      if (single) { cc_gsrb_d(M, D0, nbot); cc_residual_d(M, D0, true); }
      else cc_run_cycle(M, 1, [&] { cc_coarse_correction(M); cc_fine_seq(M, true, true, true); });
    },
    [&](int n) {
      cc_run_cycle(M, 8 + 4 * n, [&] {
        for (int c = 0; c < n; c++) { cc_coarse_correction(M); cc_fine_seq(M, true, true, true, false); norm_hist_push(M.d_nrm); }
      });
    },
    [&] { return read_scalar1(M.d_nrm); });
  if (s.overshot) { arena_release(mark); return mg_repeat_unpredicted([&] { return cc_solve(q); }); }
  if (D0.split) cc_from_split(D0);
  if (fast) {
    cc_halo(M, D0);
    fast->phi_view.clear();
    for (size_t b = 0; b < D0.boxes.size(); b++) fast->phi_view.push_back(cc_phi_view(D0.boxes[b].L, fast->rho->vbox[b].lo));
  } else cc_store(M, q.phi, q.bc);
  q.cycles = s.cycles; q.res0 = bnorm; q.res = s.res;
  if (!keep && !fast) arena_release(mark);
  return s.conv ? 0 : 1;
}

void cc_smooth(vdn_multifab *rh, vdn_multifab *phi, vdn_multifab **beta, const double *dx, const int bc[3][2], int nsweeps) {
  size_t mark = arena_mark();
  CCMG M; cc_setup(M, rh, phi, nullptr, beta, dx, bc);
  cc_gsrb_d(M, M.dlev[0], nsweeps);
  cc_store(M, phi, bc);
  arena_release(mark);
}

void cc_bench_smoother(vdn_multifab *rh, vdn_multifab *phi, vdn_multifab **beta, const vdn_multifab *rho, const double *dx, const int bc[3][2],
                       int nlaunch, double *avg_ms, long *cells, int slab_sweeps) {
  size_t mark = arena_mark();
  CCMG M; cc_setup(M, rh, phi, nullptr, beta, dx, bc, rho);
  REQUIRE(M.dlev[0].boxes.size() == 1, "smoother probe: one local box expected");
  const CLev &L = M.dlev[0].boxes[0].L;
  hipStream_t st = ctx().stream;
  hipEvent_t e0, e1; HIPCHK(hipEventCreate(&e0)); HIPCHK(hipEventCreate(&e1));
  CDLev &D0 = M.dlev[0];
  if (cc_split_ok(M)) { cc_split_setup(M); cc_to_split(D0, 1); }
  g_mac_level_form = D0.split ? 1 : 0;
  auto pass = [&](int w) { if (D0.split) launch_gsrb_split<0>(D0.boxes[0], w & 1, st, L); else launch_gsrb(L, w & 1, st); };
  const bool slabs = slab_sweeps > 0 && D0.split && !D0.halo && mac_slab(L) > 0;
  if (slab_sweeps > 0 && !slabs) { *avg_ms = 0.0; *cells = 0; HIPCHK(hipEventDestroy(e0)); HIPCHK(hipEventDestroy(e1)); arena_release(mark); return; }
  const int nrun = slabs ? std::max(1, nlaunch / (2 * slab_sweeps)) : 0;
  if (slabs) nlaunch = nrun * 2 * slab_sweeps;
  for (int w = 0; w < 4; w++) pass(w);
  HIPCHK(hipEventRecord(e0, st));
  if (slabs) for (int w = 0; w < nrun; w++) cc_split_run(M, D0, false, slab_sweeps, false, false, false);
  else for (int w = 0; w < nlaunch; w++) pass(w);
  HIPCHK(hipEventRecord(e1, st));
  HIPCHK(hipEventSynchronize(e1));
  float ms = 0; HIPCHK(hipEventElapsedTime(&ms, e0, e1));
  *avg_ms = (double)ms / nlaunch; *cells = (long)L.n[0] * L.n[1] * L.n[2];
  HIPCHK(hipEventDestroy(e0)); HIPCHK(hipEventDestroy(e1));
  arena_release(mark);
}

struct divumac_K { FV um; FV vm; FV wm; FV macrhs; FV rh; double dxi0; double dxi1; double dxi2;
  __device__ void cell(int i, int j, int k) const {
    double div = (fv_get(um, i + 1, j, k) - fv_get(um, i, j, k)) * dxi0
               + (fv_get(vm, i, j + 1, k) - fv_get(vm, i, j, k)) * dxi1
               + (fv_get(wm, i, j, k + 1) - fv_get(wm, i, j, k)) * dxi2;
    fv_at(rh, i, j, k) = div * -1.0 + fv_get(macrhs, i, j, k);
  } };

struct mk_mac_coeffs_K { FV rho; FV bx; FV by; FV bz; int h0; int h1; int h2;
  __device__ void cell(int i, int j, int k) const {
    const double r0 = fv_get(rho, i, j, k);
    if (j <= h1 && k <= h2) fv_at(bx, i, j, k) = 2.0 / (r0 + fv_get(rho, i - 1, j, k));
    if (i <= h0 && k <= h2) fv_at(by, i, j, k) = 2.0 / (r0 + fv_get(rho, i, j - 1, k));
    if (i <= h0 && j <= h1) fv_at(bz, i, j, k) = 2.0 / (r0 + fv_get(rho, i, j, k - 1));
  } };

struct UmacArgs { int lo[3], hi[3]; int ebc[3][2]; double dx[3]; };
struct mkumac_K { FV um; FV vm; FV wm; FV phi; FV bx; FV by; FV bz; UmacArgs A;
  __device__ void cell(int i, int j, int k) const {
    const double p0 = fv_get(phi, i, j, k);
    if (j <= A.hi[1] && k <= A.hi[2]) {
      int side = (i == A.lo[0]) ? 0 : (i == A.hi[0] + 1 ? 1 : -1);
      if (!(side >= 0 && A.ebc[0][side] == VDN_BC_NEU)) {
        double g = (p0 - fv_get(phi, i - 1, j, k)) / A.dx[0];
        fv_at(um, i, j, k) = fv_get(um, i, j, k) - fv_get(bx, i, j, k) * g;
      }
    }
    if (i <= A.hi[0] && k <= A.hi[2]) {
      int side = (j == A.lo[1]) ? 0 : (j == A.hi[1] + 1 ? 1 : -1);
      if (!(side >= 0 && A.ebc[1][side] == VDN_BC_NEU)) {
        double g = (p0 - fv_get(phi, i, j - 1, k)) / A.dx[1];
        fv_at(vm, i, j, k) = fv_get(vm, i, j, k) - fv_get(by, i, j, k) * g;
      }
    }
    if (i <= A.hi[0] && j <= A.hi[1]) {
// ... 159 lines not shown
```

### varden_amd/csrc/mg_nd.hip

```cpp
#include "vdn_dev.h"
#include "mg_stop.h"
#include "krylov_wg.h"
#include "krylov_grid.h"
#include "nd_lds_plan.h"
#include <tuple>
#include <algorithm>

struct NLev {
  int n[3]; int PX, PY; long sz;
  double f[3];
  double *phi, *tmp, *b, *res, *sig;
  int dirlo[3], dirhi[3];
  int per[3];
};
DEVI long nidx(const NLev &L, int i, int j, int k) { return (long)(i + 16) + (long)L.PX * ((long)(j + 1) + (long)L.PY * (long)(k + 1)); }
DEVI bool nd_is_dir(const NLev &L, int i, int j, int k) {
  return (i == 0 && L.dirlo[0]) || (i == L.n[0] && L.dirhi[0]) || (j == 0 && L.dirlo[1]) || (j == L.n[1] && L.dirhi[1]) ||
         (k == 0 && L.dirlo[2]) || (k == L.n[2] && L.dirhi[2]);
}
DEVI bool nd_is_shell(const NLev &L, int i, int j, int k, int hm) {
  return ((hm & 1) && i == 0) || ((hm & 2) && i == L.n[0]) || ((hm & 4) && j == 0) || ((hm & 8) && j == L.n[1]) ||
         ((hm & 16) && k == 0) || ((hm & 32) && k == L.n[2]);
}

// ... 1057 lines not shown
  const int u = (int)(blockIdx.x * blockDim.x + threadIdx.x) - 1, v = (int)(blockIdx.y * blockDim.y + threadIdx.y) - 1;
  const int face = blockIdx.z, d = face >> 1, side = face & 1;
  const int da = d == 0 ? 1 : 0, db = d == 2 ? 1 : 2;
  if (u > L.n[da] + 1 || v > L.n[db] + 1) return;
  int q[3]; q[d] = side ? L.n[d] + 1 : -1; q[da] = u; q[db] = v;
  const long c = nidx(L, q[0], q[1], q[2]);
  a0[c] = 0.0; if (a1) a1[c] = 0.0; if (a2) a2[c] = 0.0;
}
static NLev nd_alloc_lev(const int n[3], const double h[3]) {
  NLev L;
  for (int d = 0; d < 3; d++) { L.n[d] = n[d]; L.f[d] = 1.0 / (36.0 * (h[d] * h[d])); L.dirlo[d] = L.dirhi[d] = L.per[d] = 0; }
  L.PX = ((n[0] + 18 + 15) / 16) * 16; L.PY = n[1] + 3; L.sz = (long)L.PX * L.PY * (n[2] + 3);
  double *base = (double *)arena_alloc(sizeof(double) * L.sz * 5);
  L.phi = base; L.tmp = base + L.sz; L.b = base + 2 * L.sz; L.res = base + 3 * L.sz; L.sig = base + 4 * L.sz;
  if (sw().nd_lean && (long)(n[0] + 1) * (n[1] + 1) * (n[2] + 1) >= (1L << 21)) {
    const int m = std::max(n[0], std::max(n[1], n[2])) + 3;
    hipLaunchKernelGGL(kk_nd_zero_shell, dim3((m + 63) / 64, (m + 3) / 4, 6), dim3(64, 4, 1), 0, ctx().stream, L, L.phi, L.tmp, L.res);
    HIPCHK(hipMemsetAsync(L.sig, 0, sizeof(double) * L.sz, ctx().stream));
  } else HIPCHK(hipMemsetAsync(base, 0, sizeof(double) * L.sz * 5, ctx().stream));
  return L;
}
static FV nd_view(const NLev &L, double *p, const int lo[3], int extra ) {
  FV f; f.p = p; f.a0 = lo[0] - 16; f.a1 = lo[1] - 1; f.a2 = lo[2] - 1; f.n0 = L.PX; f.n1 = L.PY; f.n2 = L.n[2] + extra; f.sc = L.sz;
  return f;
}

static void nd_build(NDMG &M, const vdn_multifab *coeffs, const double *dx, const int bc[3][2]) {
  Prof prof_("nd_build");
  const vdn_layout *la = coeffs->la; const int lev = coeffs->lev;
  const int nb = (int)la->boxes[lev].size();
  for (int d = 0; d < 3; d++) M.per[d] = (bc[d][0] == VDN_BC_PER);
  const MgPlan P = mg_plan_of(la, lev);
  REQUIRE(P.err.empty(), "nodal multigrid: %s", P.err.c_str());
  const int perbits = M.per[0] | (M.per[1] << 1) | (M.per[2] << 2);
  double h[3] = { dx[0], dx[1], dx[2] };
  for (const MgDistLevel &PL : P.dist) {
    const int *n = PL.n;
    NDLev DL;
    std::vector<XBoxInfo> xa, xb2, xr, xs;
    vdn_box lpd; for (int d = 0; d < 3; d++) { lpd.lo[d] = 0; lpd.hi[d] = PL.ng[d] - 1; DL.ng[d] = PL.ng[d]; }
    for (int g = 0; g < nb; g++) {
      XBoxInfo x; memset(&x, 0, sizeof x);
      const int *lo = PL.lo[g].data();
      for (int d = 0; d < 3; d++) { x.vlo[d] = lo[d]; x.vhi[d] = lo[d] + n[d]; }
      x.owner = la->owner[lev][g];
      XBoxInfo xc = x; for (int d = 0; d < 3; d++) xc.vhi[d] = lo[d] + n[d] - 1;
      XBoxInfo xA = x, xB = x, xR = x;
      if (x.owner == ctx().rank) {
        NBox B; B.L = nd_alloc_lev(n, h); for (int d = 0; d < 3; d++) B.lo[d] = lo[d];
        for (int d = 0; d < 3; d++) {
          B.L.dirlo[d] = (lo[d] == 0 && bc[d][0] == VDN_BC_DIR); B.L.dirhi[d] = (lo[d] + n[d] == lpd.hi[d] + 1 && bc[d][1] == VDN_BC_DIR);
        }
        B.hmask = 0;
        for (int d = 0; d < 3; d++) {
          if (lo[d] > 0 || M.per[d]) B.hmask |= 1 << (2 * d);
          if (lo[d] + n[d] < lpd.hi[d] + 1 || M.per[d]) B.hmask |= 2 << (2 * d);
        }
        B.A = B.L.phi; B.B = B.L.tmp;
        xA.fv = nd_view(B.L, B.A, lo, 3); xB.fv = nd_view(B.L, B.B, lo, 3); xR.fv = nd_view(B.L, B.L.res, lo, 3); xc.fv = nd_view(B.L, B.L.sig, lo, 3);
        DL.boxes.push_back(B);
      }
      xa.push_back(xA); xb2.push_back(xB); xr.push_back(xR); xs.push_back(xc);
    }
    if (nb > 1 || perbits) {
      const void *p0 = DL.boxes.empty() ? nullptr : (const void *)DL.boxes[0].A;
      GraphKey hk; for (const NBox &B : DL.boxes) { hk.put(B.A); hk.put(B.L.sz); }
      auto get = [&](int which, const std::vector<XBoxInfo> &xv) { return mg_halo_plan(MgHaloKey{ la->uid, p0, lev, (int)M.dlev.size(), which, perbits, hk.h }, xv, lpd, M.per, false); };
      DL.halo_A = get(0, xa); DL.halo_B = get(1, xb2); DL.halo_res = get(2, xr); DL.halo_sig = get(3, xs);
    }
    DL.single_box = (nb == 1); for (int d = 0; d < 3; d++) DL.per[d] = M.per[d];
    M.dlev.push_back(DL);
    for (int d = 0; d < 3; d++) h[d] *= 2.0;
  }
  if (!P.tail.empty()) {
    for (const auto &tn : P.tail) {
      NLev T = nd_alloc_lev(tn.data(), h);
      for (int d = 0; d < 3; d++) { T.dirlo[d] = (bc[d][0] == VDN_BC_DIR); T.dirhi[d] = (bc[d][1] == VDN_BC_DIR); T.per[d] = M.per[d]; h[d] *= 2.0; }
      M.tail.push_back(T);
    }
    const int *cn = P.cn;
    M.g_nodes = P.gather((long)(cn[0] + 1) * (cn[1] + 1) * (cn[2] + 1)); M.g_cells = P.gather((long)cn[0] * cn[1] * cn[2]);
    std::vector<GBox> gb = M.g_nodes.gb; gb.insert(gb.end(), M.g_cells.gb.begin(), M.g_cells.gb.end());
    M.d_gb = (GBox *)arena_alloc(2 * nb * sizeof(GBox));
    HIPCHK(hipMemcpyAsync(M.d_gb, gb.data(), 2 * nb * sizeof(GBox), hipMemcpyHostToDevice, ctx().stream));
    HIPCHK(hipStreamSynchronize(ctx().stream));
    M.sendbuf = (double *)arena_alloc(sizeof(double) * M.g_nodes.cnt);
    M.recvbuf = (double *)arena_alloc(sizeof(double) * M.g_nodes.cnt * ctx().nranks);
  }
  M.d_nrm = (double *)arena_alloc(256);
  const int method = mg_krylov_method(ctx().prm.hg_bottom_solver);
  if (method && P.whole_bottom) {
    const NLev &B = !M.tail.empty() ? M.tail.back() : M.dlev.back().boxes[0].L;
    GraphKey k; k.put(1); k.put(method); k.put(B.n); k.put(B.dirlo); k.put(B.dirhi); k.put(ctx().prm.hg_bottom_solver_eps);
    mg_krylov_setup(M.kry, method, B.sz, std::max(B.n[0], std::max(B.n[1], B.n[2])) + 1, (long)(B.n[0] + 1) * (B.n[1] + 1) * (B.n[2] + 1), k);
  }
}

static void nd_halo_phi(NDLev &DL) { XPlan *P = DL.flip ? DL.halo_B : DL.halo_A; if (P) xplan_run(P); }
static bool nd_halo_begin(NDLev &DL) {
  XPlan *P = DL.flip ? DL.halo_B : DL.halo_A;
  if (!P) return false;
  const int ov_env = sw().overlap;
  static const long ov_min = 1L << 20;
  long nodes = 0;
  for (const NBox &B : DL.boxes) nodes = std::max(nodes, (long)B.L.n[0] * B.L.n[1] * B.L.n[2]);
  if (!(ov_env == 1 || (ov_env != 0 && xplan_has_remote(P) && nodes >= ov_min))) { xplan_run(P); return false; }
  VdnCtx &c = ctx();
  HIPCHK(hipEventRecord(c.ev_main, c.stream));
  HIPCHK(hipStreamWaitEvent(c.halo_stream, c.ev_main, 0));
  xplan_run(P, c.halo_stream);
  HIPCHK(hipEventRecord(c.ev_halo, c.halo_stream));
  return true;
}
static void nd_halo_end() { VdnCtx &c = ctx(); HIPCHK(hipStreamWaitEvent(c.stream, c.ev_halo, 0)); }
static const long SMALL_LEVEL_NODES = 9L * 9 * 9;
struct NdOm { double om, om1, om2; int nsp; double at(int s) const { return s < nsp ? (s == 0 ? om1 : om2) : om; } };
static bool g_nd_iso = true;
static bool nd_isotropic(const double *dx) {
  const double lo = std::min(dx[0], std::min(dx[1], dx[2])), hi = std::max(dx[0], std::max(dx[1], dx[2]));
  return hi <= 1.25 * lo;
}
static NdOm nd_om(bool pre, int nsweeps) {
  const vdn_params &P = ctx().prm;
  NdOm o{ P.hg_omega, 0.0, 0.0, 0 };
  if (g_nd_iso && pre && nsweeps == 2 && P.hg_nu1 == 2 && P.hg_omega_pre1 > 0.0 && P.hg_omega_pre2 > 0.0) { o.om1 = P.hg_omega_pre1; o.om2 = P.hg_omega_pre2; o.nsp = 2; }
  return o;
}
static void nd_jacobi_d(NDLev &DL, int nsweeps, bool pre = false, const NLev *pro = nullptr) {
  const NdOm om = nd_om(pre, nsweeps);
  NdOmegaScope scope_;
  if (DL.single_box && DL.boxes.size() == 1 && (long)(DL.ng[0] + 1) * (DL.ng[1] + 1) * (DL.ng[2] + 1) <= SMALL_LEVEL_NODES) {
    NBox &B = DL.boxes[0];
    NLev Lp = B.L;
    for (int d = 0; d < 3; d++) Lp.per[d] = DL.per[d];
    hipLaunchKernelGGL(kk_nd_bottom, dim3(1), dim3(1024), 0, ctx().stream, Lp, B.L.phi, B.L.tmp, nsweeps, om.om, om.om1, om.om2, om.nsp);
    if (nsweeps & 1) { std::swap(B.L.phi, B.L.tmp); DL.flip = !DL.flip; }
    return;
  }
  for (int s = 0; s < nsweeps; s++) {
    g_nd_omega_now = om.at(s);
    const bool ov = nd_halo_begin(DL);
    for (NBox &B : DL.boxes) nd_launch_march<0>(B.L, B.L.phi, B.L.tmp, nullptr, 0, DL.rev, s == 0 ? pro : nullptr);
    DL.rev ^= 1;
    if (ov) {
      nd_halo_end();
      for (NBox &B : DL.boxes) nd_launch_shell<0>(B.L, B.L.phi, B.L.tmp, nullptr, B.hmask);
    }
    for (NBox &B : DL.boxes) std::swap(B.L.phi, B.L.tmp);
    DL.flip = !DL.flip;
  }
}
static void nd_residual_d(NDMG &M, NDLev &DL, bool norm, bool reduce = true) {
  if (norm) HIPCHK(hipMemsetAsync(M.d_nrm, 0, sizeof(double), ctx().stream));
  DL.res_restricted = false;
  {
    const size_t l = &DL - &M.dlev[0];
    if (sw().nd_restrict_fused && DL.single_box && DL.boxes.size() == 1 && !DL.halo_res && !(DL.per[0] || DL.per[1] || DL.per[2]) && l + 1 < M.dlev.size() && M.dlev[l + 1].boxes.size() == 1) {
      const NLev &L = DL.boxes[0].L;
      if (nd_wide_even_level(L)) {
        nd_halo_phi(DL);
        NdPairGrid G = nd_pair_grid(L, 4, L.n[2] / 2 + 1, true, 2048, 0);
        G.rev = sw().nd_rev ? DL.rev : 0; DL.rev ^= 1;
        hipLaunchKernelGGL((kk_nd_march_pair_rst<4>), dim3(G.nmain + G.gyr * G.gz), NBLK, 0, ctx().stream, L, (const double *)L.phi, L.res, G, norm ? M.d_nrm : nullptr);
        DL.res_restricted = true;
        if (norm && reduce) comm_allreduce_max_dev(M.d_nrm, 1);
        return;
      }
    }
  }
  const bool ov = nd_halo_begin(DL);
  for (NBox &B : DL.boxes)
    nd_launch_march<1>(B.L, B.L.phi, B.L.res, norm ? M.d_nrm : nullptr, ov ? B.hmask : 0, DL.rev);
  DL.rev ^= 1;
  if (ov) {
    nd_halo_end();
    for (NBox &B : DL.boxes) nd_launch_shell<1>(B.L, B.L.phi, B.L.res, norm ? M.d_nrm : nullptr, B.hmask);
  }
  if (DL.halo_res) xplan_run(DL.halo_res);
  if (norm && reduce) comm_allreduce_max_dev(M.d_nrm, 1);
}

static void nd_fill_nodes(const NLev &L, double *a) {
  if (!(L.per[0] || L.per[1] || L.per[2])) return;
  hipLaunchKernelGGL(kk_nd_fill_nodes, ng3(L.n[0] + 3, L.n[1] + 3, L.n[2] + 3), NBLK, 0, ctx().stream, L, a);
}
static void nd_jacobi_t(NLev &L, int nsweeps, bool pre = false) {
  const NdOm om = nd_om(pre, nsweeps);
  NdOmegaScope scope_;
  if ((long)(L.n[0] + 1) * (L.n[1] + 1) * (L.n[2] + 1) <= SMALL_LEVEL_NODES) {
    hipLaunchKernelGGL(kk_nd_bottom, dim3(1), dim3(1024), 0, ctx().stream, L, L.phi, L.tmp, nsweeps, om.om, om.om1, om.om2, om.nsp);
    if (nsweeps & 1) std::swap(L.phi, L.tmp);
    return;
  }
  for (int s = 0; s < nsweeps; s++) {
    g_nd_omega_now = om.at(s);
    nd_fill_nodes(L, L.phi);
    nd_launch_march<0>(L, L.phi, L.tmp, nullptr);
    std::swap(L.phi, L.tmp);
  }
}
static void nd_bottom_t(const NDMG &M, NLev &L) {
  if (M.kry.w) { mg_krylov_visit(M.kry, 1, ctx().prm.hg_bottom_solver_eps, NdKrylov{ L, L.phi }); return; }
  const int N = std::max(L.n[0], std::max(L.n[1], L.n[2]));
  const int ns = std::max(ctx().prm.hg_nub, 2 * N * N);
  hipLaunchKernelGGL(kk_nd_bottom, dim3(1), dim3(1024), 0, ctx().stream, L, L.phi, L.tmp, ns, ctx().prm.hg_omega);
  if (ns & 1) std::swap(L.phi, L.tmp);
}
static bool nd_small_end(NDMG &M, int dl, int tl);
static void nd_vcycle_t(NDMG &M, int l) {
  const vdn_params &P = ctx().prm;
  NLev &L = M.tail[l];
  if (l == 0) HIPCHK(hipMemsetAsync(L.phi, 0, sizeof(double) * L.sz, ctx().stream));
  if (nd_small_end(M, -1, l)) return;
  if (l == (int)M.tail.size() - 1) { nd_bottom_t(M, L); return; }
  NLev &C = M.tail[l + 1];
  nd_jacobi_t(L, P.hg_nu1, true);
  nd_fill_nodes(L, L.phi);
  nd_launch_march<1>(L, L.phi, L.res, nullptr);
  nd_fill_nodes(L, L.res);
  hipLaunchKernelGGL(kk_nd_restrict, ng3(C.n[0] + 1, C.n[1] + 1, C.n[2] + 1), NBLK, 0, ctx().stream, L, C);
  nd_vcycle_t(M, l + 1);
  nd_fill_nodes(C, C.phi);
  nd_launch_prolong(L, C, 0, 0, 0);
  nd_jacobi_t(L, P.hg_nu2);
}

static void nd_restrict_down(NDMG &M, int l) {
  NDLev &DL = M.dlev[l];
  if (l + 1 < (int)M.dlev.size()) {
    NDLev &DC = M.dlev[l + 1];
    for (size_t b = 0; b < DL.boxes.size(); b++) {
      NLev &C = DC.boxes[b].L;
      if (DL.res_restricted) hipLaunchKernelGGL(kk_nd_rst_y, ng3(C.n[0] + 1, C.n[1] + 1, C.n[2] + 1), NBLK, 0, ctx().stream, DL.boxes[b].L, (const double *)DL.boxes[b].L.res, C);
      else hipLaunchKernelGGL(kk_nd_restrict, ng3(C.n[0] + 1, C.n[1] + 1, C.n[2] + 1), NBLK, 0, ctx().stream, DL.boxes[b].L, C);
    }
    DL.res_restricted = false;
// ... 224 lines not shown
NdKeep *nd_keep_new() { return new NdKeep; }
void nd_keep_free(NdKeep *k) { delete k; }
int nd_solve(NdRequest &q) {
  Prof prof_("hg_multigrid");
  if (ctx().prm.dm == 2) return nd2_solve(q);
  const vdn_params &P = ctx().prm;
  vdn_multifab *rh = q.rh, *phi = q.phi, *add_to = q.add_to; const vdn_multifab *u = q.u; const double *dx = q.dx;
  NdKeep *keep = q.keep; NdFast *fast = q.fast;
  const bool fixed_cycles = q.fixed_cycles > 0;
  REQUIRE(dx && q.bc && q.fixed_cycles >= 0, "nodal multigrid: dx, bc and fixed_cycles >= 0");
  if (fast) REQUIRE(fast->rhohalf && u && u->ng >= 1 && u->nc >= 3 && !keep && !fixed_cycles, "nodal multigrid: the fast path needs rhohalf and u with a ghost cell");
  else REQUIRE(rh && phi && q.coeffs && rh->ng >= 1 && phi->ng >= 1 && q.coeffs->ng >= 1, "nodal multigrid: rh, phi, coeffs need one ghost layer");
  if (u && !fast) REQUIRE(u->ng >= 1 && u->nc >= 3, "nodal multigrid: u needs a ghost cell");
  if (q.rh_is_b) REQUIRE(fixed_cycles && !u && !fast, "nodal multigrid: rh_is_b is the fixed-cycle correction solve's");
  const vdn_multifab *coeffs = fast ? fast->rhohalf : q.coeffs;
  g_nd_iso = nd_isotropic(dx);
  hipStream_t st = ctx().stream;
  size_t mark = arena_mark();
  NDMG M_local;
  NDMG &M = keep ? keep->M : M_local;
  const bool rebuild = !(keep && keep->built);
  if (rebuild) nd_build(M, coeffs, dx, q.bc);
  NDLev &D0 = M.dlev[0];
  if (!fixed_cycles || rebuild) mg_krylov_begin(M.kry, 1, M.kry.w != nullptr);
  M.pro_levels = 0; g_nd_pro_levels = 0;
  M.lds_levels = 0; g_nd_lds_levels = 0;
  if (rebuild) {
  for (size_t b = 0; b < D0.boxes.size(); b++) {
    NLev &L0 = D0.boxes[b].L; const vdn_box &bx = coeffs->vbox[b];
    if (fast) {
      hipLaunchKernelGGL(kk_nd_load_sigma_rho, ng3(L0.n[0] + 2, L0.n[1] + 2, L0.n[2] + 2), NBLK, 0, st, L0, fast->rhohalf->fabs[b], bx.lo[0], bx.lo[1], bx.lo[2]);
    } else
    hipLaunchKernelGGL(kk_nd_load_sigma, ng3(L0.n[0] + 2, L0.n[1] + 2, L0.n[2] + 2), NBLK, 0, st, L0, coeffs->fabs[b], bx.lo[0], bx.lo[1], bx.lo[2]);
  }
  if (fast && D0.halo_sig) xplan_run(D0.halo_sig);
  for (size_t l = 1; l < M.dlev.size(); l++) {
    for (size_t b = 0; b < M.dlev[l].boxes.size(); b++) {
      NLev &C = M.dlev[l].boxes[b].L;
      hipLaunchKernelGGL(kk_nd_coarsen_sigma, ng3(C.n[0], C.n[1], C.n[2]), NBLK, 0, st, M.dlev[l - 1].boxes[b].L, C);
    }
    if (M.dlev[l].halo_sig) xplan_run(M.dlev[l].halo_sig);
  }
  if (!M.tail.empty()) {
    NDLev &DL = M.dlev.back();
    const int nb = (int)M.g_nodes.gb.size();
    for (size_t b = 0; b < DL.boxes.size(); b++) {
      const NLev &F = DL.boxes[b].L;
      hipLaunchKernelGGL(kk_nd_coarsen_sigma_pack, ng3(F.n[0] / 2, F.n[1] / 2, F.n[2] / 2), NBLK, 0, st, F, M.sendbuf, M.g_cells.loc_off[b], F.n[0] / 2, F.n[1] / 2, F.n[2] / 2);
    }
    comm_allgather_dev(M.sendbuf, M.recvbuf, M.g_cells.cnt);
    hipLaunchKernelGGL(kk_nd_unpack, dim3(4, 1, (unsigned)nb), dim3(256), 0, st, M.tail[0], M.tail[0].sig, M.recvbuf, M.d_gb + nb, 0);
    hipLaunchKernelGGL(kk_nd_fill_cells, ng3(M.tail[0].n[0] + 2, M.tail[0].n[1] + 2, M.tail[0].n[2] + 2), NBLK, 0, st, M.tail[0], M.tail[0].sig);
    for (size_t l = 1; l < M.tail.size(); l++) {
      NLev &C = M.tail[l];
      hipLaunchKernelGGL(kk_nd_coarsen_sigma, ng3(C.n[0], C.n[1], C.n[2]), NBLK, 0, st, M.tail[l - 1], C);
      hipLaunchKernelGGL(kk_nd_fill_cells, ng3(C.n[0] + 2, C.n[1] + 2, C.n[2] + 2), NBLK, 0, st, C, C.sig);
    }
  }
  }
  if (keep) keep->built = true;
  if (u && !fast) {
    std::vector<std::pair<nd_divu_K, Range3>> v;
    for (size_t b = 0; b < D0.boxes.size(); b++) {
      const vdn_box &bx = coeffs->vbox[b];
      Range3 r; for (int d = 0; d < 3; d++) { r.lo[d] = bx.lo[d]; r.hi[d] = bx.hi[d] + 1; }
      v.push_back({ nd_divu_K{ u->fabs[b], rh->fabs[b], 0.25 / dx[0], 0.25 / dx[1], 0.25 / dx[2] }, r });
    }
    launch_cells(v, st);
  }
  HIPCHK(hipMemsetAsync(M.d_nrm, 0, 2 * sizeof(double), st));
  for (size_t b = 0; b < D0.boxes.size(); b++) {
    NLev &L0 = D0.boxes[b].L; const vdn_box &bx = coeffs->vbox[b];
    if (fast) {
      hipLaunchKernelGGL(kk_nd_load_divu, ng3(L0.n[0] + 1, L0.n[1] + 1, std::min(L0.n[2] + 1, 16)), NBLK, 0, st, L0, u->fabs[b], 0.25 / dx[0], 0.25 / dx[1], 0.25 / dx[2],
                         bx.lo[0], bx.lo[1], bx.lo[2], M.d_nrm);
    } else if (q.rh_is_b) {
      hipLaunchKernelGGL(kk_nd_load_b, ng3(L0.n[0] + 1, L0.n[1] + 1, std::min(L0.n[2] + 1, 16)), NBLK, 0, st, L0, rh->fabs[b], bx.lo[0], bx.lo[1], bx.lo[2]);
    } else
    hipLaunchKernelGGL(kk_nd_load, ng3(L0.n[0] + 1, L0.n[1] + 1, std::min(L0.n[2] + 1, 16)), NBLK, 0, st, L0, rh->fabs[b], phi->fabs[b], bx.lo[0], bx.lo[1], bx.lo[2], M.d_nrm);
  }
  comm_allreduce_max_dev(M.d_nrm, 2);
  const bool single = (M.dlev.size() == 1 && M.tail.empty());
  double bnorm = 1.0, p0max = 1.0;
  if (!fixed_cycles) { const double *sc = read_scalars(M.d_nrm, 2); bnorm = sc[0]; p0max = sc[1]; }
  if (P.hg_fmg && bnorm != 0.0 && !single && (fixed_cycles ? q.fmg_start : (p0max == 0.0 && bnorm < HUGE_VAL))) nd_fmg(M);
  auto correct = [&] {
    nd_restrict_down(M, 0);
    if (M.dlev.size() > 1) nd_vcycle_d(M, 1); else nd_vcycle_t(M, 0);
    nd_prolong_smooth(M, 0);
  };
  MgStop s;
  if (fixed_cycles) {
    for (int c = 0; c < q.fixed_cycles; c++) {
      if (single) { nd_jacobi_d(M.dlev[0], nd_bottom_sweeps_global(M.dlev[0])); continue; }
      nd_run_cycle(M, 2, [&] { nd_jacobi_d(M.dlev[0], P.hg_nu1, true); nd_residual_d(M, M.dlev[0], false); correct(); });
      s.cycles++;
    }
    s.conv = true;
  } else {
    const int gn[3] = { M.dlev[0].ng[0], M.dlev[0].ng[1], M.dlev[0].ng[2] };
    s = mg_stop_loop(1, gn, fast && !single && p0max == 0.0, fast && !single, q, bnorm, M.d_nrm,
      [&](bool blind) {
        nd_jacobi_d(M.dlev[0], single ? nd_bottom_sweeps_global(M.dlev[0]) : P.hg_nu1, !single);
        nd_residual_d(M, M.dlev[0], true, !blind);
      },
      [&] {
        if (single) { nd_jacobi_d(M.dlev[0], nd_bottom_sweeps_global(M.dlev[0])); nd_residual_d(M, M.dlev[0], true); }
        else nd_run_cycle(M, 1, [&] { correct(); nd_jacobi_d(M.dlev[0], P.hg_nu1, true); nd_residual_d(M, M.dlev[0], true); });
      },
      [&](int n) {
        nd_run_cycle(M, 8 + 4 * n, [&] {
          for (int c = 0; c < n; c++) { correct(); nd_jacobi_d(M.dlev[0], P.hg_nu1, true); nd_residual_d(M, M.dlev[0], true, false); norm_hist_push(M.d_nrm); }
        });
      },
      [&] { return read_scalar1(M.d_nrm); });
    if (s.overshot) { arena_release(mark); return mg_repeat_unpredicted([&] { return nd_solve(q); }); }
  }
  NDLev &DF = M.dlev[0];
  nd_halo_phi(DF);
  if (fast) fast->phi_view.clear();
  for (size_t b = 0; b < DF.boxes.size(); b++) {
    NLev &L0 = DF.boxes[b].L; const vdn_box &bx = coeffs->vbox[b];
    if (fast) { fast->phi_view.push_back(nd_view(L0, L0.phi, bx.lo, 3)); continue; }
    if (add_to) hipLaunchKernelGGL(kk_nd_store_add, ng3(L0.n[0] + 3, L0.n[1] + 3, L0.n[2] + 3), NBLK, 0, st, L0, phi->fabs[b], add_to->fabs[b], bx.lo[0], bx.lo[1], bx.lo[2]);
    else
    hipLaunchKernelGGL(kk_nd_store, ng3(L0.n[0] + 3, L0.n[1] + 3, L0.n[2] + 3), NBLK, 0, st, L0, phi->fabs[b], bx.lo[0], bx.lo[1], bx.lo[2]);
  }
  q.cycles = s.cycles; q.res0 = bnorm; q.res = s.res;
  g_nd_pro_levels = M.pro_levels;
  g_nd_lds_levels = M.lds_levels;
  if (!keep && !fast) arena_release(mark);
  return s.conv ? 0 : 1;
}

struct UvecArgs { int lo[3], hi[3], ng; int phys[3][2]; double dt, dtinv; int proj_type; };
struct create_uvec_K { FV unew; FV uold; FV rhohalf; FV gp; UvecArgs A;
  __device__ void cell(int i, int j, int k) const {
    const int q[3] = { i, j, k };
    bool g1 = true;
  #pragma unroll
    for (int d = 0; d < 3; d++) if (q[d] < A.lo[d] - 1 || q[d] > A.hi[d] + 1) g1 = false;
    bool wall_plane = false, inlet_plane = false;
  #pragma unroll
    for (int d = 0; d < 3; d++) {
      if (q[d] == A.lo[d] - 1) { int p = A.phys[d][0]; if (p == VDN_SLIP_WALL || p == VDN_NO_SLIP_WALL) wall_plane = true; if (p == VDN_INLET) inlet_plane = true; }
      if (q[d] == A.hi[d] + 1) { int p = A.phys[d][1]; if (p == VDN_SLIP_WALL || p == VDN_NO_SLIP_WALL) wall_plane = true; if (p == VDN_INLET) inlet_plane = true; }
    }
  #pragma unroll
    for (int m = 0; m < 3; m++) {
      double gpv = 0.0;
      if (g1) { gpv = fv_get(gp, i, j, k, m); if (inlet_plane) { gpv = 0.0; fv_at(gp, i, j, k, m) = 0.0; } }
      if (wall_plane) { fv_at(unew, i, j, k, m) = 0.0; continue; }
      if (!g1) continue;
      double v = fv_get(unew, i, j, k, m);
      if (A.proj_type == VDN_PRESSURE_ITERS) v = (v - fv_get(uold, i, j, k, m)) * A.dtinv;
      else if (A.proj_type == VDN_REGULAR_TIMESTEP) v = v + A.dt * gpv / fv_get(rhohalf, i, j, k, 0);
      fv_at(unew, i, j, k, m) = v;
    }
  } };

struct coeffs_K { FV coeffs; FV rhohalf;
  __device__ void cell(int i, int j, int k) const {
    fv_at(coeffs, i, j, k) = 1.0 / fv_get(rhohalf, i, j, k, 0);
  } };

DEVI double gphi_of(const FV &phi, int i, int j, int k, int m, double dxi) {
  #define P(a, b, c) fv_get(phi, i + (a), j + (b), k + (c))
  if (m == 0) return 0.25 * (P(1, 0, 0) + P(1, 1, 0) + P(1, 0, 1) + P(1, 1, 1) - P(0, 0, 0) - P(0, 1, 0) - P(0, 0, 1) - P(0, 1, 1)) * dxi;
  if (m == 1) return 0.25 * (P(0, 1, 0) + P(1, 1, 0) + P(0, 1, 1) + P(1, 1, 1) - P(0, 0, 0) - P(1, 0, 0) - P(0, 0, 1) - P(1, 0, 1)) * dxi;
  return 0.25 * (P(0, 0, 1) + P(1, 0, 1) + P(0, 1, 1) + P(1, 1, 1) - P(0, 0, 0) - P(1, 0, 0) - P(0, 1, 0) - P(1, 1, 0)) * dxi;
  #undef P
}

struct HgUpdArgs { int hi[3]; double dt, dtinv, dxi[3]; int proj_type; };
struct hg_update_K { FV unew; FV uold; FV gp; FV rhohalf; FV p; FV phi; HgUpdArgs A;
  __device__ void cell(int i, int j, int k) const {
    const bool cell = i <= A.hi[0] && j <= A.hi[1] && k <= A.hi[2];
    if (cell) {
      const double rho = fv_get(rhohalf, i, j, k, 0);
    #pragma unroll
      for (int m = 0; m < 3; m++) {
        const double gph = gphi_of(phi, i, j, k, m, A.dxi[m]);
        double v = fv_get(unew, i, j, k, m) - gph / rho;
        if (A.proj_type == VDN_PRESSURE_ITERS) v = fv_get(uold, i, j, k, m) + A.dt * v;
        fv_at(unew, i, j, k, m) = v;
        if (A.proj_type == VDN_PRESSURE_ITERS) fv_at(gp, i, j, k, m) = fv_get(gp, i, j, k, m) + gph;
        else if (A.proj_type == VDN_REGULAR_TIMESTEP) fv_at(gp, i, j, k, m) = A.dtinv * gph;
      }
    }
    if (A.proj_type == VDN_PRESSURE_ITERS) fv_at(p, i, j, k) = fv_get(p, i, j, k) + fv_get(phi, i, j, k);
    else if (A.proj_type == VDN_REGULAR_TIMESTEP) fv_at(p, i, j, k) = A.dtinv * fv_get(phi, i, j, k);
  } };


static void hg_level_pre(int proj_type, vdn_multifab *un, const vdn_multifab *uo, const vdn_multifab *rhh, vdn_multifab *gpp, vdn_multifab *coeffs,
                         double dt, const vdn_bc_tower *bct) {
  hipStream_t st = ctx().stream;
  REQUIRE(un->ng >= 1 && gpp->ng >= 1 && rhh->ng >= 1, "hgproject: ghost widths");
// ... 768 lines not shown
```

### varden_amd/csrc/mg_stop.h

```cpp
#pragma once
#include "vdn_internal.h"

inline bool mg_converged(double rn, double bnorm, double rel_eps, double abs_eps) { return (rn <= rel_eps * bnorm && bnorm < HUGE_VAL) || rn <= abs_eps; }

struct MgStop { int cycles = 0; double res = 0.0; bool conv = false, overshot = false; };
template <class First, class Cycle, class Blind, class Read>
MgStop mg_stop_loop(int solver, const int gn[3], bool predict, bool remember, const MgRequest &q, double bnorm, const double *d_nrm,
                    First first, Cycle cycle, Blind blind, Read read) {
  MgStop s;
  s.conv = (bnorm == 0.0);
  const int pred = (predict && !s.conv) ? std::min(mg_predict_get(solver, gn), std::min(q.max_iter, 63)) : 0;
  if (!s.conv) {
    first(pred >= 2);
    if (pred >= 2) {
      norm_hist_reset(); norm_hist_push(d_nrm);
      blind(pred - 1);
      const double *h = norm_hist_read(pred);
      int stop = -1;
      for (int c = 0; c < pred && stop < 0; c++)
        if (mg_converged(h[c], bnorm, q.rel_eps, q.abs_eps) || !(h[c] < HUGE_VAL)) stop = c;
      if (stop >= 0 && stop < pred - 1) { s.overshot = true; return s; }
      s.cycles = pred - 1; s.res = h[pred - 1];
    } else s.res = read();
  }
  while (!s.conv) {
    if (mg_converged(s.res, bnorm, q.rel_eps, q.abs_eps)) { s.conv = true; break; }
    if (s.cycles >= q.max_iter || !(s.res < HUGE_VAL) || !(bnorm < HUGE_VAL)) break;
    cycle();
    s.cycles++;
    s.res = read();
  }
  if (s.conv && remember && s.cycles >= 1) mg_predict_set(solver, gn, s.cycles);
  return s;
}
template <class Solve> int mg_repeat_unpredicted(Solve solve) {
  struct Off { Off() { g_mg_predict_off++; } ~Off() { g_mg_predict_off--; } } off_;
  return solve();
}
```

### varden_amd/csrc/runtime.hip

```cpp
#include "vdn_dev.h"
#include <algorithm>
#include <chrono>
#include <map>
#include <tuple>

static VdnCtx g_ctx;
VdnCtx &ctx() { return g_ctx; }
static thread_local char g_err[1024] = "";

void vdn_set_error(const char *fmt, ...) { va_list ap; va_start(ap, fmt); vsnprintf(g_err, sizeof g_err, fmt, ap); va_end(ap); }
void vdn_fail(const char *fmt, ...) {
  char buf[1024]; va_list ap; va_start(ap, fmt); vsnprintf(buf, sizeof buf, fmt, ap); va_end(ap);
  throw VdnErr(buf);
}

static std::vector<vdn_multifab *> g_temp_mfs;
void arena_reset() {
  dbg_sync(16);
  for (vdn_multifab *m : g_temp_mfs) delete m;
  g_temp_mfs.clear();
  if (sw().arena_poison && g_ctx.arena && g_ctx.arena_peak > 0) HIPCHK(hipMemsetAsync(g_ctx.arena, 0xFF, std::min(g_ctx.arena_peak + (size_t)(64 << 20), g_ctx.arena_bytes), g_ctx.stream));
  g_ctx.arena_off = 0;
  g_ctx.drop_step_caches();
}
// ... 92 lines not shown
  if (off + bytes > c.arena_bytes) arena_map_to(off + bytes);
  c.arena_off = off + bytes;
  if (c.arena_off > c.arena_peak) c.arena_peak = c.arena_off;
  return c.arena + off;
}

extern "C" void vdn_params_default(vdn_params *p) {
  memset(p, 0, sizeof *p);
  p->dm = 3; p->nscal = 2; p->slope_order = 4; p->use_minion = 0; p->boussinesq = 0;
  p->stencil_order = 2; p->diffusion_type = 1; p->verbose = 0; p->mg_verbose = 0; p->prob_type = 1;
  p->visc_coef = 0.0; p->diff_coef = 0.0; p->cflfac = 0.8; p->max_dt_growth = 1.1;
  p->mg_nu1 = 2; p->mg_nu2 = 2; p->mg_nub = 8; p->mg_max_iter = 100;
  p->hg_max_iter = 100; p->hg_nu1 = 2; p->hg_nu2 = 1; p->hg_nub = 8; p->hg_omega = 0.9;
  p->mac_rel_eps = 1.0e-10; p->hg_rel_eps = -1.0; p->abort_on_max_iter = 1; p->hg_fmg = 1; p->mac_fmg = 1; p->hg_omega_pre1 = 1.45; p->hg_omega_pre2 = 0.7; p->hg_omega_fac1 = 1.6; p->hg_omega_fac2 = 0.9; p->hg_omega_fac3 = 0.65; p->mg_predict = 1;
  p->mg_bottom_solver = -1; p->hg_bottom_solver = -1; p->max_mg_bottom_nlevels = 1000;
  p->mg_bottom_solver_eps = 1.0e-3; p->hg_bottom_solver_eps = 1.0e-3;
}

#include <dlfcn.h>
#include <thread>
static int (*g_roctx_push)(const char *) = nullptr;
static int (*g_roctx_pop)() = nullptr;
void prof_load() {
  static bool tried = false;
  if (tried) return;
  tried = true;
  if (sw().no_roctx) return;
  for (const char *n : { "librocprofiler-sdk-roctx.so.1", "librocprofiler-sdk-roctx.so", "libroctx64.so.4", "libroctx64.so" }) {
    void *h = dlopen(n, RTLD_NOW | RTLD_LOCAL);
    if (!h) continue;
    *(void **)(&g_roctx_push) = dlsym(h, "roctxRangePushA");
    *(void **)(&g_roctx_pop) = dlsym(h, "roctxRangePop");
    if (g_roctx_push && g_roctx_pop) return;
    g_roctx_push = nullptr; g_roctx_pop = nullptr;
  }
}
Prof::Prof(const char *name) : on(g_roctx_push != nullptr) { if (on) g_roctx_push(name); }
Prof::~Prof() { if (on) g_roctx_pop(); }

static Switches g_sw;
const Switches &sw() { static const bool filled = (switches_read(g_sw), true); (void)filled; return g_sw; }
const Switches &sw_live() { sw(); switches_read(g_sw, true); return g_sw; }
extern "C" const char *vdn_build_flavour(void) {
#ifdef VDN_TESTING_BUILD
  return "testing";
#else
  return "release";
#endif
}
extern char **environ;
static void env_warn_unknown() {
  static bool done = false;
  if (done) return;
  done = true;
  for (char **e = environ; e && *e; e++) {
    if (strncmp(*e, "VDN_", 4) != 0 || !strncmp(*e, "VDN_BENCH_", 10) || !strncmp(*e, "VDN_WORKER_", 11)) continue;
    const char *eq = strchr(*e, '=');
    const size_t len = eq ? (size_t)(eq - *e) : strlen(*e);
    bool known = false;
    for (const SwitchInfo &s : switch_table) if (strlen(s.name) == len && !strncmp(s.name, *e, len)) known = true;
    if (!strncmp(*e, "VDN_LIB_FLAVOUR", 15)) continue;
    if (!known) fprintf(stderr, "varden_amd: warning: environment variable %.*s is not a switch of this library (vdn_debug_switches lists them)\n", (int)len, *e);
#ifndef VDN_TESTING_BUILD
    else fprintf(stderr, "varden_amd: note: %.*s is set but this is the release build: launch-form switches are compiled out (libvarden_amd_testing.so reads them)\n", (int)len, *e);
#endif
  }
}
#ifdef VDN_TESTING_BUILD
unsigned nd_last_prolong_levels();
extern "C" unsigned vdn_nd_prolong_fused_levels(void) { return nd_last_prolong_levels(); }
unsigned nd_last_lds_levels();
extern "C" unsigned vdn_nd_lds_levels(void) { return nd_last_lds_levels(); }
#endif
extern "C" const char *vdn_debug_switches(void) {
  static std::string out;
#ifndef VDN_TESTING_BUILD
  if (out.empty()) out = "release build: the switches below are compiled out, every launch form is the default one (libvarden_amd_testing.so reads them)\n";
#endif
  if (out.find(std::string(switch_table[0].name) + " ") == std::string::npos) for (const SwitchInfo &s : switch_table) { const char *v = switch_raw(s); out += s.name; out += v ? std::string(" = ") + v : std::string(" (unset)"); out += ": "; out += s.doc; out += "\n"; }
  return out.c_str();
}

bool g_capturing_now();
__global__ void k_publish(double *host_view, const double *dev, int n, unsigned long long seq) {
  if ((int)threadIdx.x < n) host_view[threadIdx.x] = dev[threadIdx.x];
  __syncthreads();
  if (threadIdx.x == 0) { __threadfence_system(); *reinterpret_cast<volatile unsigned long long *>(host_view + 64) = seq; }
}
const double *read_scalars(const double *dev, int n) {
  VdnCtx &c = g_ctx;
  REQUIRE(n >= 1 && n <= 64, "read_scalars: 1..64 values");
  static unsigned long long seq = 0;
  const bool poll = sw().poll >= 0 ? sw().poll != 0 : c.nranks == 1;
  ++seq;
  dbg_sync(8);
  hipLaunchKernelGGL(k_publish, dim3(1), dim3(64), 0, c.stream, c.h_scal_dev, dev, n, seq);
  if (poll && !g_capturing_now()) {
    volatile unsigned long long *flag = reinterpret_cast<volatile unsigned long long *>(c.h_scal + 64);
    for (unsigned long spins = 1;; spins++) {
      if (*flag == seq) { __sync_synchronize(); return c.h_scal; }
      __builtin_ia32_pause();
      if ((spins & 0xfff) == 0) {
        const hipError_t q = hipStreamQuery(c.stream);
        if (q == hipSuccess) break;
        if (q != hipErrorNotReady) HIPCHK(q);
        if (spins > 0x40000) std::this_thread::yield();
      }
    }
  }
  HIPCHK(hipStreamSynchronize(c.stream));
  return c.h_scal;
}

__global__ void k_hist_push(double *hist, const double *nrm) {
  int *cnt = reinterpret_cast<int *>(hist + 64);
  const int c = *cnt;
  if (c < 64) hist[c] = *nrm;
  *cnt = c + 1;
}
void norm_hist_reset() { HIPCHK(hipMemsetAsync(g_ctx.d_hist + 64, 0, sizeof(double), g_ctx.stream)); }
void norm_hist_push(const double *d_nrm) { hipLaunchKernelGGL(k_hist_push, dim3(1), dim3(1), 0, g_ctx.stream, g_ctx.d_hist, d_nrm); }
const double *norm_hist_read(int n) {
  REQUIRE(n >= 1 && n <= 64, "norm_hist_read: 1..64 entries");
  comm_allreduce_max_dev(g_ctx.d_hist, n);
  return read_scalars(g_ctx.d_hist, n);
}
int g_mg_predict_off = 0;
static std::map<unsigned long long, int> g_mg_pred;
static unsigned long long mg_pred_key(int solver, const int n[3]) { GraphKey k; k.put(solver); k.put(n[0]); k.put(n[1]); k.put(n[2]); return k.h; }
int mg_predict_get(int solver, const int n[3]) {
  if (!g_ctx.prm.mg_predict || g_mg_predict_off > 0) return 0;
  auto it = g_mg_pred.find(mg_pred_key(solver, n));
  return it == g_mg_pred.end() ? 0 : it->second;
}
void mg_predict_set(int solver, const int n[3], int cycles) { if (g_mg_pred.size() > 4096) g_mg_pred.clear(); g_mg_pred[mg_pred_key(solver, n)] = cycles; }

static std::map<unsigned long long, hipGraphExec_t> g_graphs;
static bool g_capturing = false;
bool g_capturing_now() { return g_capturing; }
bool graphs_enabled() {
  return !sw().no_graphs && !comm_active() && g_ctx.stream != 0 && !g_capturing;
}
static unsigned long g_graph_generation = 1;
unsigned long graph_generation() { return g_graph_generation; }
void graph_cache_clear() {
  if (!g_graphs.empty() && g_ctx.stream) (void)hipStreamSynchronize(g_ctx.stream);
  for (auto &kv : g_graphs) (void)hipGraphExecDestroy(kv.second);
  g_graphs.clear();
  g_graph_generation++;
}
bool graph_replay(unsigned long long key) {
  auto it = g_graphs.find(key);
  if (it == g_graphs.end()) return false;
  HIPCHK(hipGraphLaunch(it->second, g_ctx.stream));
  return true;
}
void graph_begin() {
  REQUIRE(!g_capturing, "graph_begin: nested capture");
  HIPCHK(hipStreamBeginCapture(g_ctx.stream, hipStreamCaptureModeThreadLocal));
  g_capturing = true;
}
void graph_abort() {
  if (!g_capturing) return;
  hipGraph_t g = nullptr;
  (void)hipStreamEndCapture(g_ctx.stream, &g);
  if (g) (void)hipGraphDestroy(g);
  (void)hipGetLastError();
  g_capturing = false;
}
void graph_end(unsigned long long key) {
  REQUIRE(g_capturing, "graph_end without graph_begin");
  hipGraph_t g = nullptr;
  g_capturing = false;
  HIPCHK(hipStreamEndCapture(g_ctx.stream, &g));
  hipGraphExec_t ex = nullptr;
  hipError_t e = hipGraphInstantiate(&ex, g, nullptr, nullptr, 0);
  (void)hipGraphDestroy(g);
  if (e != hipSuccess) vdn_fail("hipGraphInstantiate failed: %s", hipGetErrorString(e));
  if (g_graphs.size() >= 256) graph_cache_clear();
  auto old = g_graphs.find(key);
  if (old != g_graphs.end()) { (void)hipStreamSynchronize(g_ctx.stream); (void)hipGraphExecDestroy(old->second); }
  g_graphs[key] = ex;
  HIPCHK(hipGraphLaunch(ex, g_ctx.stream));
}

void solver_check(int rc, const char *what, int iters, double res, double res0, int comp) {
  const bool bad = !(res < HUGE_VAL) || !(res0 < HUGE_VAL);
  if (rc == 0 && !bad) return;
  char cs[32] = ""; if (comp >= 0) snprintf(cs, sizeof cs, " (component %d)", comp);
  if (ctx().prm.abort_on_max_iter)
    vdn_fail("%s%s %s after %d iterations (residual %g, right-hand side %g)", what, cs, bad ? "met a non-finite norm" : "did not converge", iters, res, res0);
  if (ctx().prm.verbose) fprintf(stderr, "varden_amd: %s%s did not converge in %d iterations (res %g / %g)\n", what, cs, iters, res, res0);
}

extern "C" const char *vdn_last_error(void) { return g_err; }
static int g_stale_hip_error = 0;
void vdn_note_stale_error(hipError_t e) {
  static bool noted = false;
  g_stale_hip_error = (int)e;
  if (!noted) { noted = true; fprintf(stderr, "varden_amd: note: the caller left a pending HIP error on this thread (%s); cleared at entry (vdn_last_stale_hip_error returns it; further ones are not printed)\n", hipGetErrorString(e)); }
}
extern "C" int vdn_last_stale_hip_error(int clear) { const int e = g_stale_hip_error; if (clear) g_stale_hip_error = 0; return e; }

static int g_bottom_form[2] = { 0, 0 };
static std::map<unsigned long long, int> g_bb_table;
static unsigned long long g_bb_last[2] = { 0, 0 };
static int g_bb_last_budget[2] = { 0, 0 };
extern "C" int vdn_init(const vdn_params *prm, int rank, int nranks, int device) {
  VDN_TRY
  env_warn_unknown();
  REQUIRE(prm != nullptr, "vdn_init: null params");
  g_ctx.extruded2d = false;
  REQUIRE(prm->dm == 3 || prm->dm == 2, "vdn_init: dm must be 2 or 3 (got %d)", prm->dm);
  REQUIRE(prm->nscal >= 1 && prm->nscal + 5 <= VDN_MAXCOMP, "vdn_init: nscal = %d is outside 1..%d (nscal + 5 <= VDN_MAXCOMP = %d: velocity, scalars, pressure and extrap components)",
          prm->nscal, VDN_MAXCOMP - 5, VDN_MAXCOMP);
  REQUIRE(prm->visc_coef >= 0.0 && prm->diff_coef >= 0.0, "vdn_init: negative visc_coef / diff_coef");
  REQUIRE(prm->diffusion_type == 1 || prm->diffusion_type == 2, "BAD DIFFUSION TYPE");
  REQUIRE(prm->slope_order == 0 || prm->slope_order == 2 || prm->slope_order == 4, "bad slope_order");
  REQUIRE(prm->mg_bottom_solver >= -1 && prm->mg_bottom_solver <= 4, "vdn_init: bad mg_bottom_solver %d (-1, 0, 4: bottom sweeps; 1, 3: BiCGStab; 2: CG)", prm->mg_bottom_solver);
  REQUIRE(prm->hg_bottom_solver >= -1 && prm->hg_bottom_solver <= 4, "vdn_init: bad hg_bottom_solver %d (-1, 0, 4: bottom sweeps; 1, 3: BiCGStab; 2: CG)", prm->hg_bottom_solver);
  REQUIRE(prm->mg_bottom_solver_eps > 0.0 && prm->mg_bottom_solver_eps < 1.0 && prm->hg_bottom_solver_eps > 0.0 && prm->hg_bottom_solver_eps < 1.0,
          "vdn_init: mg_bottom_solver_eps / hg_bottom_solver_eps must lie in (0, 1)");
  int ndev = 0;
  HIPCHK(hipGetDeviceCount(&ndev));
  REQUIRE(ndev > 0, "vdn_init: no HIP device visible -- the product path has no CPU fallback");
  REQUIRE(device >= 0 && device < ndev, "vdn_init: device %d out of range (%d devices)", device, ndev);
  HIPCHK(hipSetDevice(device));
  VdnCtx &c = g_ctx;
  c.prm = *prm; c.rank = rank; c.nranks = nranks; c.device = device;
  if (!c.d_scal) {
    HIPCHK(hipMalloc((void **)&c.d_scal, 64 * sizeof(double)));
    HIPCHK(hipMalloc((void **)&c.d_hist, 65 * sizeof(double)));
    HIPCHK(hipHostMalloc((void **)&c.h_scal, 72 * sizeof(double), hipHostMallocMapped));
    memset(c.h_scal, 0, 72 * sizeof(double));
    HIPCHK(hipHostGetDevicePointer((void **)&c.h_scal_dev, c.h_scal, 0));
  }
  if (!c.own_stream) {
    HIPCHK(hipStreamCreateWithFlags(&c.own_stream, hipStreamNonBlocking));
    HIPCHK(hipStreamCreateWithFlags(&c.halo_stream, hipStreamNonBlocking));
    HIPCHK(hipEventCreateWithFlags(&c.ev_main, hipEventDisableTiming));
    HIPCHK(hipEventCreateWithFlags(&c.ev_halo, hipEventDisableTiming));
  }
  if (c.stream == 0) c.stream = c.own_stream;
  const bool krylov = (prm->mg_bottom_solver >= 1 && prm->mg_bottom_solver <= 3) || (prm->hg_bottom_solver >= 1 && prm->hg_bottom_solver <= 3);
  if (krylov && !c.d_bstats) HIPCHK(hipMalloc((void **)&c.d_bstats, 10 * sizeof(double)));
  if (krylov) HIPCHK(hipMemsetAsync(c.d_bstats, 0, 10 * sizeof(double), c.stream));
  g_bb_last[0] = g_bb_last[1] = 0; g_bottom_form[0] = g_bottom_form[1] = 0;
  prof_load();
  c.inited = true;
  VDN_CATCH
}
extern "C" int vdn_finalize(void) {
  VDN_TRY
  VdnCtx &c = g_ctx;
  kept_purge(0);
  arena_destroy(); field_pool_release(); fabio_release();
  graph_cache_clear();
  if (c.d_hist) { HIPCHK(hipFree(c.d_hist)); c.d_hist = nullptr; }
  if (c.d_bstats) { HIPCHK(hipFree(c.d_bstats)); c.d_bstats = nullptr; }
  if (c.d_scal) { HIPCHK(hipFree(c.d_scal)); c.d_scal = nullptr; HIPCHK(hipHostFree(c.h_scal)); c.h_scal = nullptr; c.h_scal_dev = nullptr; }
  c.inited = false;
  VDN_CATCH
}
extern "C" int vdn_set_stream(void *s) {
  VDN_TRY
  if (g_ctx.inited) HIPCHK(hipStreamSynchronize(g_ctx.stream));
  graph_cache_clear();
  g_ctx.stream = s ? (hipStream_t)s : g_ctx.own_stream;
  VDN_CATCH
}
extern "C" int vdn_arena_stats(size_t *reserved_bytes, size_t *peak_bytes) { *reserved_bytes = g_ctx.arena_bytes; *peak_bytes = g_ctx.arena_peak; return 0; }
extern "C" int vdn_device_synchronize(void) { VDN_TRY HIPCHK(hipStreamSynchronize(g_ctx.stream)); VDN_CATCH }
extern "C" int vdn_get_params(vdn_params *out) { *out = g_ctx.prm; return 0; }
extern "C" int vdn_set_extruded_2d(int on) { g_ctx.extruded2d = on != 0; return 0; }
extern "C" int vdn_last_step_timing(double *s) { for (int i = 0; i < 5; i++) s[i] = g_ctx.step_sec[i]; return 0; }
extern "C" int vdn_last_solver_stats(int w, int *cyc, double *r0, double *r) {
  if (w < 0 || w > 1) return 1;
  *cyc = g_ctx.solver_cycles[w]; *r0 = g_ctx.solver_res0[w]; *r = g_ctx.solver_res[w]; return 0;
}
double *bottom_stats_dev(int which) { return g_ctx.d_bstats + 4 * which; }
double *bottom_exhausted_dev(int which) { return g_ctx.d_bstats + 8 + which; }
void bottom_stats_reset(int which) {
  HIPCHK(hipMemsetAsync(g_ctx.d_bstats + 4 * which, 0, 4 * sizeof(double), g_ctx.stream));
  HIPCHK(hipMemsetAsync(g_ctx.d_bstats + 8 + which, 0, sizeof(double), g_ctx.stream));
}
void bottom_form_set(int which, int form) { g_bottom_form[which] = form; }
extern "C" int vdn_last_bottom_form(int which) { return (which == 0 || which == 1) ? g_bottom_form[which] : -1; }
int bottom_budget_begin(int which, unsigned long long kind, int cap) {
  if (g_bb_last[which]) {
    double v[4], ex;
    { const double *h = read_scalars(g_ctx.d_bstats + 4 * which, 4); for (int q = 0; q < 4; q++) v[q] = h[q]; }
    ex = read_scalar1(g_ctx.d_bstats + 8 + which);
    if (v[0] > 0.0) {
      const int mx = (int)v[2];
      g_bb_table[g_bb_last[which]] = ex > 0.0 ? 2 * g_bb_last_budget[which] : 32 * ((mx + mx / 2 + 8 + 31) / 32);
    }
    g_bb_last[which] = 0;
  }
  if (!kind) return 0;
  const auto it = g_bb_table.find(kind);
  const int b = it == g_bb_table.end() ? cap : std::min(cap, it->second);
  g_bb_last[which] = kind; g_bb_last_budget[which] = b;
  return b;
}
extern "C" int vdn_last_bottom_stats(int which, int *calls, int *iters, int *max_iters, int *breakdowns) {
  VDN_TRY
  REQUIRE(which == 0 || which == 1, "vdn_last_bottom_stats: which must be 0 (cell-centred) or 1 (nodal)");
  REQUIRE(g_ctx.inited, "vdn_last_bottom_stats: vdn_init first");
  const int b = which == 0 ? g_ctx.prm.mg_bottom_solver : g_ctx.prm.hg_bottom_solver;
  double v[4] = { 0.0, 0.0, 0.0, 0.0 };
  if (b >= 1 && b <= 3 && g_ctx.d_bstats) { const double *h = read_scalars(g_ctx.d_bstats + 4 * which, 4); for (int q = 0; q < 4; q++) v[q] = h[q]; }
  if (calls) *calls = (int)v[0]; if (iters) *iters = (int)v[1]; if (max_iters) *max_iters = (int)v[2]; if (breakdowns) *breakdowns = (int)v[3];
  VDN_CATCH
}

extern "C" int vdn_layout_create(int nlev, const int *rr, const vdn_box *pd, const int *nboxes, const vdn_box *boxes,
                                 const int *owner, const int *pmask, vdn_layout **out) {
  VDN_TRY
  REQUIRE(nlev >= 1, "nlev must be >= 1");
  static unsigned long next_uid = 1;
  vdn_layout *la = new vdn_layout;
  la->uid = next_uid++;
  la->nlev = nlev;
  if (nlev > 1) la->rr.assign(rr, rr + 3 * (nlev - 1));
  la->pd.assign(pd, pd + nlev);
  for (int d = 0; d < 3; d++) la->pmask[d] = pmask ? pmask[d] : 0;
  int off = 0;
  la->boxes.resize(nlev); la->owner.resize(nlev); la->local.resize(nlev);
  for (int l = 0; l < nlev; l++) {
    for (int b = 0; b < nboxes[l]; b++) {
      const vdn_box &bx = boxes[off + b];
      for (int d = 0; d < g_ctx.prm.dm; d++) REQUIRE(bx.hi[d] - bx.lo[d] + 1 >= 4, "box %d of level %d is narrower than 4 cells", b, l);
      if (g_ctx.prm.dm == 2) REQUIRE(bx.lo[2] == 0 && bx.hi[2] == 0, "dm = 2: boxes must have lo(3) = hi(3) = 0");
      la->boxes[l].push_back(bx);
      int ow = owner ? owner[off + b] : 0;
      REQUIRE(ow >= 0 && ow < g_ctx.nranks, "owner %d out of range", ow);
      la->owner[l].push_back(ow);
      if (ow == g_ctx.rank) la->local[l].push_back(b);
    }
    off += nboxes[l];
  }
  *out = la;
  VDN_CATCH
}
extern "C" int vdn_layout_destroy(vdn_layout *la) { VDN_TRY if (la) { graph_cache_clear(); xplan_cache_purge(la->uid); delete la; } VDN_CATCH }
extern "C" int vdn_layout_nlevel(const vdn_layout *la) { return la->nlev; }
extern "C" int vdn_layout_nboxes(const vdn_layout *la, int lev) { return (int)la->boxes[lev].size(); }
extern "C" int vdn_layout_nlocal(const vdn_layout *la, int lev) { return (int)la->local[lev].size(); }
extern "C" int vdn_layout_global_index(const vdn_layout *la, int lev, int i) { return la->local[lev][i]; }
extern "C" int vdn_layout_get_box(const vdn_layout *la, int lev, int g, vdn_box *out) { *out = la->boxes[lev][g]; return 0; }

static void build_adv_ell(int p, int d, int dm, int nscal, int *a, int *e) {
  const int press = dm + nscal, extrap = press + 1;
  if (p == VDN_SLIP_WALL) {
    for (int c = 0; c < dm; c++) a[c] = VDN_HOEXTRAP;
    a[d] = VDN_EXT_DIR;
    for (int n = 0; n < nscal; n++) a[dm + n] = VDN_HOEXTRAP;
    a[press] = VDN_FOEXTRAP; a[extrap] = VDN_FOEXTRAP;
// ... 487 lines not shown
```

### varden_amd/csrc/vdn_internal.h

```cpp
#pragma once
#define VDN_MAXLEV 4
#include <hip/hip_runtime.h>
#include <string>
#include <vector>
#include <map>
#include <cstdio>
#include <cstdarg>
#include <cstring>
#include <cstdlib>
#include <stdexcept>
#include <cmath>
#include "../../include/varden_amd.h"
#include "vdn_switches.h"
#include "mg_plan.h"

struct FV {
  double *p;
  int a0, a1, a2;
  int n0, n1, n2;
  long sc;
};
struct BoxP {
  int lo[3], hi[3];
  int phys[3][2];
};

#define VDN_MAXCOMP 16

struct vdn_layout {
  unsigned long uid = 0;
  int nlev = 0;
  std::vector<int> rr;
  std::vector<vdn_box> pd;
  std::vector<std::vector<vdn_box>> boxes;
  std::vector<std::vector<int>> owner;
  std::vector<std::vector<int>> local;
  int pmask[3] = {0, 0, 0};
};

struct vdn_multifab {
  const vdn_layout *la = nullptr;
  int lev = 0, nc = 1, ng = 0;
  int nodal[3] = {0, 0, 0};
  double *base = nullptr;
  bool owns = true;
  size_t bytes = 0;
  std::vector<FV> fabs;
  std::vector<vdn_box> vbox;
  int nfabs() const { return (int)fabs.size(); }
  long fab_size(int i) const { return fabs[i].sc * nc; }
};

struct vdn_bc_tower {
  const vdn_layout *la = nullptr;
  unsigned long serial = 0;
  int dm = 3, nscal = 2;
  int ncomp_adv = 0, ncomp_ell = 0;
  std::vector<std::vector<BoxP>> phys;
  std::vector<std::vector<std::vector<int>>> adv;
  std::vector<std::vector<std::vector<int>>> ell;
  int domain_bc[3][2];
  int press_comp0() const { return dm + nscal; }
  int extrap_comp0() const { return dm + nscal + 1; }
  int adv_bc(int lev, int grid, int d, int s, int c) const { return adv[lev][grid][(d * 2 + s) * ncomp_adv + c]; }
  int ell_bc(int lev, int grid, int d, int s, int c) const { return ell[lev][grid][(d * 2 + s) * ncomp_ell + c]; }
};

struct VdnCtx {
  bool inited = false;
  vdn_params prm;
  int rank = 0, nranks = 1, device = 0;
  bool extruded2d = false;
  hipStream_t stream = 0;
  hipStream_t own_stream = 0, halo_stream = 0;
  hipEvent_t ev_main = nullptr, ev_halo = nullptr;
  char *arena = nullptr; size_t arena_bytes = 0, arena_off = 0, arena_peak = 0;
  double *d_scal = nullptr; double *h_scal = nullptr;
  double *h_scal_dev = nullptr;
  double *d_bstats = nullptr;
  double *d_hist = nullptr;
  double step_sec[5] = {0, 0, 0, 0, 0};
  int solver_cycles[2] = {0, 0}; double solver_res0[2] = {0, 0}, solver_res[2] = {0, 0};
  std::vector<double *> slope_cache[3]; std::vector<const double *> slope_src;
  std::vector<double *> macmax_cache; std::vector<const double *> macmax_src;
  void drop_step_caches() { for (int d = 0; d < 3; d++) slope_cache[d].clear(); slope_src.clear(); macmax_cache.clear(); macmax_src.clear(); }
};
VdnCtx &ctx();

const Switches &sw();
const Switches &sw_live();
void vdn_set_error(const char *fmt, ...);
struct VdnErr : std::runtime_error { using std::runtime_error::runtime_error; };
[[noreturn]] void vdn_fail(const char *fmt, ...);
#define HIPCHK(x) do { hipError_t e_ = (x); if (e_ != hipSuccess) vdn_fail("%s failed: %s (%s:%d)", #x, hipGetErrorString(e_), __FILE__, __LINE__); } while (0)
void vdn_note_stale_error(hipError_t e);
#define VDN_TRY try { { const hipError_t entry_err_ = hipGetLastError(); \
    if (entry_err_ != hipSuccess && entry_err_ != hipErrorNotReady) vdn_note_stale_error(entry_err_); }
#define VDN_CATCH   if (ctx().inited) { const hipError_t le_ = hipGetLastError(); \
    if (le_ != hipSuccess && le_ != hipErrorNotReady) vdn_fail("a HIP launch failed inside this call: %s", hipGetErrorString(le_)); } \
  } catch (const std::exception &e) { vdn_set_error("%s", e.what()); return 1; } return 0;
void solver_check(int rc, const char *what, int iters, double res, double res0, int comp = -1);
#define REQUIRE(c, ...) do { if (!(c)) vdn_fail(__VA_ARGS__); } while (0)

struct Prof { explicit Prof(const char *name); ~Prof(); Prof(const Prof &) = delete; bool on; };
void prof_load();

const double *read_scalars(const double *dev, int n);
inline double read_scalar1(const double *dev) { return read_scalars(dev, 1)[0]; }
void norm_hist_reset();
void norm_hist_push(const double *d_nrm);
const double *norm_hist_read(int n);
int  mg_predict_get(int solver, const int n[3]);
void mg_predict_set(int solver, const int n[3], int cycles);
extern int g_mg_predict_off;
double *bottom_stats_dev(int which);
void    bottom_stats_reset(int which);
double *bottom_exhausted_dev(int which);
int     bottom_budget_begin(int which, unsigned long long kind, int cap);
void    bottom_form_set(int which, int form);

struct GraphKey {
  unsigned long long h = 1469598103934665603ull;
  void add(const void *p, size_t n) { const unsigned char *c = (const unsigned char *)p; for (size_t i = 0; i < n; i++) { h ^= c[i]; h *= 1099511628211ull; } }
  template <class T> void put(const T &v) { add(&v, sizeof v); }
};
struct GraphKey;
struct KeptSet { void *d_args = nullptr; int *d_start = nullptr; int nbox = 0, tot = 0; unsigned long uid = 0; };
bool     kept_family_enabled(int fam);
void     dbg_sync(int bit);
KeptSet *kept_find(unsigned long long key);
KeptSet *kept_store(unsigned long long key, unsigned long uid, const void *args, size_t arg_bytes, const int *start, int nbox, int tot);
void     kept_purge(unsigned long uid);
int      kept_bound(int dflt);
struct KeeperMem { std::vector<void *> chunks; char *cur = nullptr; size_t left = 0; };
void  keeper_begin(KeeperMem *m);
void  keeper_end();
void  keeper_free(KeeperMem *m);
void *set_alloc(size_t bytes);
void  mlcc_kept_purge(unsigned long uid);
void  mlnd_kept_purge(unsigned long uid);
bool graphs_enabled();
bool graph_replay(unsigned long long key);
void graph_begin();
void graph_end(unsigned long long key);
void graph_abort();
void graph_cache_clear();
unsigned long graph_generation();

void  arena_reset();
void  arena_reserve(size_t bytes);
void  arena_reserve_for(const vdn_layout *la);
void *arena_alloc(size_t bytes);
size_t arena_mark();
void  arena_release(size_t mark);
vdn_multifab *mf_temp(const vdn_layout *la, int lev, int nc, int ng, int face_dir ,
                      bool fill, double val);
void mf_temp_free(vdn_multifab *mf);
void fabio_release();

struct XBoxInfo { FV fv; int vlo[3], vhi[3]; int owner; };
struct XPlan;
XPlan *xplan_build(const std::vector<XBoxInfo> &boxes, const vdn_box &pd, const int pmask[3], int ng, int nc, bool faces_only = false, const int *src_trim = nullptr);
void   xplan_run(XPlan *P, hipStream_t st = nullptr);
bool   xplan_has_remote(const XPlan *P);
void   xplan_free(XPlan *P);
unsigned long xplan_serial(const XPlan *P);
void   xplan_cache_purge(unsigned long layout_uid);
struct MgHaloKey { unsigned long uid; const void *p0; int lev, l, which, per; unsigned long long sig; };
XPlan *mg_halo_plan(const MgHaloKey &key, const std::vector<XBoxInfo> &boxes, const vdn_box &pd, const int pmask[3], bool faces_only);
std::vector<XBoxInfo> xboxes_of(const vdn_multifab *mf);
struct ViewPlan;
struct SrcView {
  std::vector<char> have; std::vector<FV> fv; std::vector<vdn_box> vbox;
  int ng = 0, nc = 1, nodal[3] = {0, 0, 0};
  ViewPlan *plan = nullptr;
  int nboxes() const { return (int)vbox.size(); }
  void refresh() const;
};
SrcView make_view(const vdn_multifab *src, const std::vector<vdn_box> &footprint, const std::vector<int> &dst_owner, int scomp, int nc, unsigned long cache_tag);
void view_cache_purge(unsigned long layout_uid);
bool   comm_active();
void   comm_allreduce_max_dev(double *d, int n);
void   comm_allreduce_max_u8_dev(unsigned char *d, size_t n);
void   comm_allgather_dev(const double *send, double *recv, size_t count);

#include <algorithm>
struct BoxBins {
  int lo[3] = {0, 0, 0}, w[3] = {1, 1, 1}, n[3] = {0, 0, 0};
  std::vector<int> first, items; mutable std::vector<int> out;
  explicit BoxBins(const std::vector<vdn_box> &b, const std::vector<char> *have = nullptr) {
    int hi[3] = {0, 0, 0}; bool any = false;
    for (size_t i = 0; i < b.size(); i++) {
      if (have && !(*have)[i]) continue;
// ... 156 lines not shown
```

### varden_amd/csrc/vdn_switches.h

```cpp
#pragma once
#include <algorithm>
#include <cstddef>
#include <cstdlib>
#include <cstring>

#define VDN_SWITCHES(X) \
  X(testing, "VDN_TESTING", STR, nullptr, "1: allows VDN_RCCL_LIB (the test transport of tests/fake_rccl); nothing else") \
  X(rccl_lib, "VDN_RCCL_LIB", STR, nullptr, "path of a library that stands in for librccl -- honoured only with VDN_TESTING=1 and the test double's handshake") \
  X(force_packed, "VDN_FORCE_PACKED", LIVE, 0, "1: box-to-box copies of one rank go through the packed per-peer buffers (device memcpy for send/recv); 2: through a 1-rank RCCL communicator (one-GPU rehearsal of the N > 1 transport)") \
  X(arena_poison, "VDN_ARENA_POISON", SET, false, "1: every byte handed back to the arena is overwritten with NaNs (a read of an entry nobody wrote fails the next solve)") \
  X(arena_chunk, "VDN_ARENA_CHUNK_MB", MB, (size_t)1024 << 20, "size of the physical chunks mapped into the arena's address range (default 1024)") \
  X(field_chunk, "VDN_FIELD_CHUNK_MB", MB, (size_t)64 << 20, "size of the pooled physical chunks behind the state fields (default 64)") \
  X(field_vmm, "VDN_FIELD_VMM", ON, true, "0: every state field is one hipMalloc block (rounds 1-5) instead of pooled chunks mapped into its own address range") \
  X(mlcc_trace, "VDN_MLCC_TRACE", SET, false, "1: the composite cell-centred solve prints its residual at every FAC iteration (stderr)") \
  X(keep_off, "VDN_KEEP_OFF", INT, 0, "mask of kept-descriptor families rebuilt at every call: 1 generic sets, 2 create_umac_grown, 4 composite cell-centred solve, 8 nodal prolongation") \
  X(sync_points, "VDN_SYNC_POINTS", INT, 0, "mask of points that synchronise the device (race hunting): 1 after every batched launch, 2 after every staged upload, 4 after every exchange, 8 before a scalar read-back, 16 at arena_reset, 32 after launch_cells") \
  X(phase_hash, "VDN_PHASE_HASH", SET, false, "1: advance_timestep prints a checksum of its fields at every phase boundary (stderr)") \
  X(no_roctx, "VDN_NO_ROCTX", PRESENT, false, "do not bind the roctx library (no bl_prof ranges)") \
  X(poll, "VDN_POLL", INT, -1, "scalar read-back: 1 spin on the pinned sequence number, 0 hipStreamSynchronize; default: spin on one rank, synchronise on several") \
  X(no_graphs, "VDN_NO_GRAPHS", PRESENT, false, "launch every multigrid cycle eagerly instead of replaying its hipGraph") \
  X(no_slope_cache, "VDN_NO_SLOPE_CACHE", PRESENT, false, "velocity mkflux recomputes the slopes of uold that velpred computed in the same step") \
  X(no_force_reuse, "VDN_NO_FORCE_REUSE", SET, false, "1: every forcing term is computed where the reference computes it (advance_premac AND velocity_advance, ...)") \
  X(slopes_march, "VDN_SLOPES_MARCH", ON, true, "0: the per-cell slopes kernel instead of the k-marching one") \
  X(godunov_batch, "VDN_GODUNOV_BATCH", SET, false, "1: the descriptor (box-batched) Godunov kernels also on a level of one box") \
  X(godunov_plain, "VDN_GODUNOV_PLAIN", PRESENT, false, "the face-centred one-thread-per-cell Godunov kernels of round 1 (the fused marches' bit-for-bit reference, and their fallback where they refuse the field layouts)") \
  X(god_segw, "VDN_GOD_SEGW", ON, true, "0: the box-batched fused Godunov marches use full-width (64 x 8) tiles for every box") \
  X(god_p2, "VDN_GOD_P2", ON, true, "0: the fused marches divide by dx also where every dx is a power of two (default there: scale by 1/dx, the same doubles)") \
  X(fused_kchunks, "VDN_FUSED_KCHUNKS", MIN1, 0, "k-chunks of the fused marches (default: the count that fills the last round of workgroups best)") \
  X(god_update, "VDN_GOD_UPDATE", ON, true, "0: update_3d as its own pass instead of inside the fused mkflux march") \
  X(gsrb_pair, "VDN_GSRB_PAIR", ON, true, "0: one cell per thread in the colour passes / residuals of wide levels instead of the 2 x 2 pair form") \
  X(mac_split, "VDN_MAC_SPLIT", ON, true, "0: the finest level of macproject's one-level solve stays interleaved (kk_cc_gsrb_rho_pair) instead of stored by colour (kk_cc_gsrb_rho_split)") \
  X(mac_split_min, "VDN_MAC_SPLIT_MIN", INT, 1<<23, "fewest cells (of this rank's boxes together) of a level stored by colour (default 2^23)") \
  X(nd_rev, "VDN_ND_REV", ON, true, "0: every march of a nodal level walks its tiles in the same order (default: consecutive marches alternate)") \
  X(mac_slab, "VDN_MAC_SLAB", INT, -1, "planes per slab of the time-skewed schedule of the split level's passes (cc_split_run; default: ~200 MB of pass traffic, at most half the level); 0: whole-level launches") \
  X(mac_umax, "VDN_MAC_UMAX", ON, true, "0: max |umac| by its own pass (kk_macmax) instead of inside macproject's velocity update (kk_mkumac_rho_max)") \
  X(mac_kflip, "VDN_MAC_KFLIP", ON, true, "0: both colour passes of a sweep walk the planes upwards (default: the second colour downwards; paired and split passes of the cell-centred multigrid)") \
  X(cc_halo_faces, "VDN_CC_HALO_FACES", ON, true, "0: the cell-centred multigrid exchanges the whole ghost shell instead of the faces only") \
  X(overlap, "VDN_OVERLAP", INT, -1, "halo exchange of multigrid passes next to interior work: 1 always, 0 never, default: when a plan has a remote peer and the box is large") \
  X(mg_agglom, "VDN_MG_AGGLOM", INT, 0, "box width below which a multi-box multigrid level is gathered into one box (default: 64 across ranks, 128 where every box is this rank's)") \
  X(mg_restrict_fused, "VDN_MG_RESTRICT_FUSED", ON, true, "0: cell-centred residual and restriction as two passes") \
  X(mg_tailcycle, "VDN_MG_TAILCYCLE", ON, true, "0: the smallest levels launch by launch instead of one single-workgroup cycle") \
  X(mg_prolong_fused, "VDN_MG_PROLONG_FUSED", ON, true, "0: cell-centred prolongation as its own pass instead of inside the first post-smoothing colour pass") \
  X(mg_lds, "VDN_MG_LDS", ON, true, "0: the 16^3..64^3-cell levels of both multigrids (cell-centred and nodal) launch by launch instead of the LDS-tiled down / up kernels") \
  X(mac_stored_beta, "VDN_MAC_STORED_BETA", SET, false, "1: the finest MAC level reads stored face coefficients instead of recomputing them from rho") \
  X(mac_fast, "VDN_MAC_FAST", ON, true, "0: macproject with its rh / phi / beta multifabs as the reference has them") \
  X(hg_fast, "VDN_HG_FAST", ON, true, "0: hgproject with its rh / phi / coeffs multifabs as the reference has them") \
  X(nd_pair, "VDN_ND_PAIR", ON, true, "0: one node per lane in the nodal march instead of the pair form") \
  X(nd_lean, "VDN_ND_LEAN", ON, true, "0: whole-array zero fills of the big nodal levels instead of shell-only") \
  X(nd_restrict_fused, "VDN_ND_RESTRICT_FUSED", ON, true, "0: nodal residual and full weighting as two passes") \
  X(nd_prolong_fused, "VDN_ND_PROLONG_FUSED", ON, true, "0: nodal prolongation as a pass of its own instead of inside the first post-smoothing march") \
  X(ndf_pair, "VDN_NDF_PAIR", ON, true, "0: one node per lane in the box-batched nodal march of the composite solve") \
  X(ndm_iface_faces, "VDN_NDM_IFACE_FACES", ON, true, "0: interface interpolation of the composite nodal solve over whole boxes instead of box faces") \
  X(ndm_prolong8, "VDN_NDM_PROLONG8", ON, true, "0: correction interpolation with a thread per fine node instead of per coarse node") \
  X(ndm_neg, "VDN_NDM_NEG", SET, false, "1: the composite nodal solve copies -res into the correction's right-hand side instead of loading it directly") \
  X(fb_faces, "VDN_FB_FACES", ON, true, "0: the ghost exchanges of the composite cell-centred solve fill edges and corners too") \
  X(mlcc_rho, "VDN_MLCC_RHO", ON, true, "0: the composite MAC solve reads stored face coefficients on its finest level too") \
  X(god_narrow, "VDN_GOD_NARROW", ON, true, "0: the remainder tile column of the fused mkflux + update march in full 64-lane tiles instead of narrow segments (kk_mk_F_mn)") \
  X(keep_sets, "VDN_KEEP_SETS", ON, true, "0: the descriptor arrays of the inter-level operators and composite solves are rebuilt and uploaded at every call") \
  X(kept_bound, "VDN_KEPT_BOUND", INT, 0, "n > 0: the kept descriptor tables hold at most n entries each (default 4096 / 64 / 512): the eviction paths in a test") \
  X(mlcc_glue, "VDN_MLCC_GLUE", ON, true, "0: the level-0 correction of the composite MAC solve stored and added in separate passes") \
  X(mlcc_fuse1, "VDN_MLCC_FUSE1", ON, true, "0: the composite MAC solve's finest-level residual and first colour pass as two launches") \
  X(batch_yz, "VDN_BATCH_YZ", ON, true, "0: no (j,k) / (i,k) tiles for thin ranges in the box-batched kernels") \
  X(batch_ppw, "VDN_BATCH_PPW", MIN1, 0, "planes per workgroup of the light box-batched kernels (default 8)") \
  X(batch_flat, "VDN_BATCH_FLAT", ON, true, "0: no flattened (i,j) plane mapping for badly filling tiles") \
  X(batch_chunk, "VDN_BATCH_CHUNK", ON, true, "0: box-batched workgroups take strided instead of contiguous plane chunks")

static inline bool sw_read_ON(const char *e, bool) { return !(e && atoi(e) == 0); }
static inline bool sw_read_SET(const char *e, bool) { return e && atoi(e) != 0; }
static inline bool sw_read_PRESENT(const char *e, bool) { return e != nullptr; }
static inline int sw_read_INT(const char *e, int dflt) { return e ? atoi(e) : dflt; }
static inline int sw_read_MIN1(const char *e, int dflt) { return e ? std::max(1, atoi(e)) : dflt; }
static inline size_t sw_read_MB(const char *e, size_t dflt) { const long v = e ? atol(e) : 0; return v > 0 ? (size_t)v << 20 : dflt; }
static inline const char *sw_read_STR(const char *e, const char *) { return e; }
static inline int sw_read_LIVE(const char *e, int dflt) { return sw_read_INT(e, dflt); }

struct Switches {
#define X(field, name, rule, dflt, doc) decltype(sw_read_##rule(nullptr, dflt)) field = dflt;
  VDN_SWITCHES(X)
#undef X
};
struct SwitchInfo { const char *name, *rule, *doc; };
inline constexpr SwitchInfo switch_table[] = {
#define X(field, name, rule, dflt, doc) { name, #rule, doc },
  VDN_SWITCHES(X)
#undef X
};
static inline const char *switch_raw(const SwitchInfo &s) { return getenv(s.name); }

static inline void switches_read(Switches &s, bool live_only = false) {
#ifdef VDN_TESTING_BUILD
  const Switches dflt;
#define X(field, name, rule, d, doc) if (!live_only || !strcmp(#rule, "LIVE")) s.field = sw_read_##rule(getenv(name), dflt.field);
  VDN_SWITCHES(X)
#undef X
#else
  (void)s; (void)live_only;
#endif
}
```

Baseline: 694.3 million cells*steps/s.

## Replace host phase clocks and setup drains with events, fold norm resets, prolong into split arrays

Per-phase host synchronisations in advance_timestep are replaced by recorded hipEvents that are resolved lazily, and the stream drains in multigrid setup are replaced by staged uploads. The norm accumulator is now zeroed by the kernel that reads it back (k_publish / k_hist_push), which removes a memset before each norm pass. The MAC fast path's FMG prolongs directly into the colour-split arrays, so the separate to-split conversion pass is no longer needed. The old behaviour stays reachable through bits of VDN_SYNC_POINTS. Removing host drains lets the CPU queue work ahead, at the risk of subtle ordering bugs if the norm reset or the event timing is wrong.

```diff
diff --git a/varden_amd/csrc/advance.hip b/varden_amd/csrc/advance.hip
--- a/varden_amd/csrc/advance.hip
+++ b/varden_amd/csrc/advance.hip
@@ -78,7 +78,14 @@
   Prof prof_advance("advance");
   arena_reset();
   arena_reserve_for(mla);
-  const double t_begin = wall();
+  const bool host_clocks = (step_glue_old() & 1) != 0;
+  ctx().step_clock_pending = false;
+  auto phase_clock = [&](int i) -> double {
+    if (!host_clocks) { HIPCHK(hipEventRecord(ctx().ev_phase[i], ctx().stream)); return 0.0; }
+    if (i > 0) sync();
+    return wall();
+  };
+  const double t_begin = phase_clock(0);
   #define DXL(n) (dx + (n) * dm)
 
   vdn_multifab *mac_rhs[VDN_MAXLEV], *rhohalf[VDN_MAXLEV], *umac[3 * VDN_MAXLEV] = { nullptr }, *lapu[VDN_MAXLEV] = { nullptr };
@@ -128,14 +135,14 @@
     arena_release(mark);
   }
 
-  sync(); double t0 = wall();
+  double t0 = phase_clock(1);
   { Prof pr("MAC_Project");
   do_macproject(mla, umac, sold, mac_rhs, dx, bct, press_comp - 1);
   }
-  sync(); ctx().step_sec[2] = wall() - t0;
+  { const double t1 = phase_clock(2); if (host_clocks) ctx().step_sec[2] = t1 - t0; }
   dbg_phase_hash("umac after MAC", nlevs, umac, 3);
 
-  t0 = wall();
+  if (host_clocks) t0 = wall();
   {
     Prof pr("Scalar_update");
     size_t mark = arena_mark();
@@ -177,14 +184,14 @@
     }
     arena_release(mark);
   }
-  sync(); ctx().step_sec[0] = wall() - t0;
+  { const double t1 = phase_clock(3); if (host_clocks) ctx().step_sec[0] = t1 - t0; }
   dbg_phase_hash("snew after scalars", nlevs, snew);
 
   { Prof pr("make_at_halftime"); for (int n = 0; n < nlevs; n++) k_make_at_halftime(rhohalf[n], sold[n], snew[n], 0, 0); }
   restrict_and_fill(nlevs, rhohalf, 0, dm + 0, 1, false, bct);
   if (viscous && P.diffusion_type == 2) for (int n = 0; n < nlevs; n++) mf_setval(lapu[n], 0.0, 0, dm, true);
 
-  t0 = wall();
+  if (host_clocks) t0 = wall();
   {
     Prof pr("Velocity_update");
     size_t mark = arena_mark();
@@ -221,19 +228,21 @@
     }
     arena_release(mark);
   }
-  sync(); ctx().step_sec[1] = wall() - t0;
+  { const double t1 = phase_clock(4); if (host_clocks) ctx().step_sec[1] = t1 - t0; }
   dbg_phase_hash("unew after viscous", nlevs, unew);
 
-  t0 = wall();
+  if (host_clocks) t0 = wall();
   { Prof pr("HG_Project");
   do_hgproject(proj_type, mla, unew, uold, rhohalf, p, gp, dx, dt, bct, press_comp - 1); }
-  sync(); ctx().step_sec[3] = wall() - t0;
+  { const double t1 = phase_clock(5); if (host_clocks) ctx().step_sec[3] = t1 - t0; }
+  if (!host_clocks) { ctx().step_clock_pending = true; sync(); }
   dbg_phase_hash("unew after HG", nlevs, unew); dbg_phase_hash("p after HG", nlevs, p); dbg_phase_hash("gp after HG", nlevs, gp);
   #undef DXL
 
   arena_reset();
   ctx().drop_step_caches();
-  ctx().step_sec[4] = wall() - t_begin;
+  if (host_clocks) ctx().step_sec[4] = wall() - t_begin;
+  if (P.verbose >= 1) step_timing_resolve();
   if (P.verbose >= 1 && ctx().rank == 0) {
     printf(" Timing summary:\n Scalar   update: %g seconds\n Velocity update: %g seconds\n  MAC Projection: %g seconds\n   HG Projection: %g seconds\n\n",
            ctx().step_sec[0], ctx().step_sec[1], ctx().step_sec[2], ctx().step_sec[3]);
diff --git a/varden_amd/csrc/mg_cc.hip b/varden_amd/csrc/mg_cc.hip
--- a/varden_amd/csrc/mg_cc.hip
+++ b/varden_amd/csrc/mg_cc.hip
@@ -974,11 +974,7 @@
 }
 
 struct ProlongLinArgs { int c0[3]; int e[3][2]; };
-__global__ void kk_cc_prolong_lin(CLev F, CLev C, ProlongLinArgs A) {
-  const int i = blockIdx.x * blockDim.x + threadIdx.x;
-  const int j = blockIdx.y * blockDim.y + threadIdx.y;
-  const int k = blockIdx.z;
-  if (i >= F.n[0] || j >= F.n[1]) return;
+DEVI double cc_prolong_lin_val(const CLev &C, const ProlongLinArgs &A, int i, int j, int k) {
   const int I = A.c0[0] + (i >> 1), J = A.c0[1] + (j >> 1), K = A.c0[2] + (k >> 1);
   const long sy = C.PX, sz = (long)C.PX * C.PY;
   const long c = cidx(C, I, J, K);
@@ -992,7 +988,24 @@
   NBV(py, J, j & 1, C.n[1], A.e[1][0], A.e[1][1], sy)
   NBV(pz, K, k & 1, C.n[2], A.e[2][0], A.e[2][1], sz)
   #undef NBV
-  F.phi[cidx(F, i, j, k)] = 0.25 * (((p0 + px) + py) + pz);
+  return 0.25 * (((p0 + px) + py) + pz);
+}
+__global__ void kk_cc_prolong_lin(CLev F, CLev C, ProlongLinArgs A) {
+  const int i = blockIdx.x * blockDim.x + threadIdx.x;
+  const int j = blockIdx.y * blockDim.y + threadIdx.y;
+  const int k = blockIdx.z;
+  if (i >= F.n[0] || j >= F.n[1]) return;
+  F.phi[cidx(F, i, j, k)] = cc_prolong_lin_val(C, A, i, j, k);
+}
+__global__ void __launch_bounds__(256) kk_cc_prolong_lin_split(CLev F, CSplit S, CLev C, ProlongLinArgs A) {
+  const int e = blockIdx.x * 64 + threadIdx.x, j = (int)(blockIdx.y * 4 + threadIdx.y) - 1, k = (int)blockIdx.z - 1;
+  if (e >= S.PXH || j > F.n[1]) return;
+  const int ih = e - S.off;
+  const bool in = ih >= 0 && ih < F.n[0] / 2 && j >= 0 && j < F.n[1] && k >= 0 && k < F.n[2];
+  const int c0 = (j + k) & 1;
+  const long dst = sidx(S, ih, j, k);
+  S.phi[c0][dst] = in ? cc_prolong_lin_val(C, A, 2 * ih, j, k) : 0.0;
+  S.phi[1 - c0][dst] = in ? cc_prolong_lin_val(C, A, 2 * ih + 1, j, k) : 0.0;
 }
 
 struct CBox { CLev L; int lo[3]; int gidx; int hmask = 63;
@@ -1183,13 +1196,19 @@
     M.g_rh = P.gather((long)cn[0] * cn[1] * cn[2]);
     M.g_b = P.gather((long)(cn[0] + 1) * cn[1] * cn[2] + (long)cn[0] * (cn[1] + 1) * cn[2] + (long)cn[0] * cn[1] * (cn[2] + 1));
     M.d_gb_rh = (GBox *)arena_alloc(nb * sizeof(GBox)); M.d_gb_b = (GBox *)arena_alloc(nb * sizeof(GBox));
-    HIPCHK(hipMemcpyAsync(M.d_gb_rh, M.g_rh.gb.data(), nb * sizeof(GBox), hipMemcpyHostToDevice, ctx().stream));
-    HIPCHK(hipMemcpyAsync(M.d_gb_b, M.g_b.gb.data(), nb * sizeof(GBox), hipMemcpyHostToDevice, ctx().stream));
-    HIPCHK(hipStreamSynchronize(ctx().stream));
+    if (step_glue_old() & 1) {
+      HIPCHK(hipMemcpyAsync(M.d_gb_rh, M.g_rh.gb.data(), nb * sizeof(GBox), hipMemcpyHostToDevice, ctx().stream));
+      HIPCHK(hipMemcpyAsync(M.d_gb_b, M.g_b.gb.data(), nb * sizeof(GBox), hipMemcpyHostToDevice, ctx().stream));
+      HIPCHK(hipStreamSynchronize(ctx().stream));
+    } else {
+      upload_staged(M.d_gb_rh, M.g_rh.gb.data(), nb * sizeof(GBox));
+      upload_staged(M.d_gb_b, M.g_b.gb.data(), nb * sizeof(GBox));
+    }
     M.sendbuf = (double *)arena_alloc(sizeof(double) * M.g_b.cnt);
     M.recvbuf = (double *)arena_alloc(sizeof(double) * M.g_b.cnt * ctx().nranks);
   }
   M.d_nrm = (double *)arena_alloc(256);
+  if (nrm_self_reset()) HIPCHK(hipMemsetAsync(M.d_nrm, 0, 2 * sizeof(double), ctx().stream));
   const int method = mg_krylov_method(ctx().prm.mg_bottom_solver);
   if (method && P.whole_bottom) {
     const CLev &B = !M.tail.empty() ? M.tail.back() : M.dlev.back().boxes[0].L;
@@ -1249,7 +1268,7 @@
   }
 }
 static void cc_residual_d(CCMG &M, CDLev &DL, bool norm, bool reduce = true) {
-  if (norm) HIPCHK(hipMemsetAsync(M.d_nrm, 0, sizeof(double), ctx().stream));
+  if (norm && !nrm_self_reset()) HIPCHK(hipMemsetAsync(M.d_nrm, 0, sizeof(double), ctx().stream));
   DL.res_restricted = false;
   if (DL.split) {
     split_halo(DL, 1);
@@ -1425,7 +1444,7 @@
   const CLev &L = B0.L, &C = M.dlev[1].boxes[0].L;
   hipStream_t st = ctx().stream;
   const int R = 2 * nsweeps, n2 = L.n[2], nK = n2 / 2, slab = mac_slab(L);
-  if (residual && norm) HIPCHK(hipMemsetAsync(M.d_nrm, 0, sizeof(double), st));
+  if (residual && norm && !nrm_self_reset()) HIPCHK(hipMemsetAsync(M.d_nrm, 0, sizeof(double), st));
   DL.res_restricted = false;
   std::vector<int> done(R + 1, 0);
   for (int top = slab + R; ; top += slab) {
@@ -1526,11 +1545,16 @@
   hipLaunchKernelGGL(kk_cc_prolong, g3(L.n[0], L.n[1], L.n[2], BLK), BLK, 0, ctx().stream, L, C);
   cc_gsrb_t(M, L, P.mg_nu2);
 }
-static void cc_fmg(CCMG &M, const int bc[3][2]) {
-  const int nd = (int)M.dlev.size(), ntot = nd + (int)M.tail.size();
+static int cc_fmg_start(const CCMG &M) {
+  const int ntot = (int)M.dlev.size() + (int)M.tail.size();
   int ls = -1;
   for (int g = 1; g < ntot; g++) if (cc_level_cells(M, g) >= 4096) ls = g;
-  if (ls < 1 || ls + 1 >= ntot) return;
+  return (ls < 1 || ls + 1 >= ntot) ? -1 : ls;
+}
+static void cc_fmg(CCMG &M, const int bc[3][2], bool split_phi = false) {
+  const int nd = (int)M.dlev.size();
+  const int ls = cc_fmg_start(M);
+  if (ls < 0) return;
   hipStream_t st = ctx().stream;
   for (int g = 0; g < ls; g++) {
     if (g + 1 < nd) {
@@ -1564,6 +1588,10 @@
         const CLev &F = M.dlev[g].boxes[b].L; const CBox &CB = DC.boxes[b];
         ProlongLinArgs A;
         for (int d = 0; d < 3; d++) { A.c0[d] = 0; A.e[d][0] = (CB.lo[d] == 0) ? bc[d][0] : VDN_BC_INT; A.e[d][1] = (CB.lo[d] + CB.L.n[d] == DC.ng[d]) ? bc[d][1] : VDN_BC_INT; }
+        if (g == 0 && split_phi) {
+          const CSplit &S = M.dlev[0].boxes[b].sp;
+          hipLaunchKernelGGL(kk_cc_prolong_lin_split, dim3((unsigned)((S.PXH + 63) / 64), (unsigned)((F.n[1] + 2 + 3) / 4), (unsigned)(F.n[2] + 2)), BLK, 0, st, F, S, CB.L, A);
+        } else
         hipLaunchKernelGGL(kk_cc_prolong_lin, g3(F.n[0], F.n[1], F.n[2], BLK), BLK, 0, st, F, CB.L, A);
       }
     } else {
@@ -1694,7 +1722,7 @@
   cc_build(M, rho, dx, bc, false);
   REQUIRE(M.dlev.size() >= 2, "cc_setup_fast: needs a second distributed level");
   CDLev &D0 = M.dlev[0];
-  HIPCHK(hipMemsetAsync(M.d_nrm, 0, sizeof(double), ctx().stream));
+  if (!nrm_self_reset()) HIPCHK(hipMemsetAsync(M.d_nrm, 0, sizeof(double), ctx().stream));
   for (size_t b = 0; b < D0.boxes.size(); b++) {
     CLev &L0 = D0.boxes[b].L;
     const vdn_box &bx = rho->vbox[b];
@@ -1708,7 +1736,7 @@
                        fast->mac_rhs->fabs[b], 1.0 / dx[0], 1.0 / dx[1], 1.0 / dx[2], bx.lo[0], bx.lo[1], bx.lo[2], e[0][0], e[0][1], e[1][0], e[1][1], e[2][0], e[2][1], M.d_nrm);
   }
   comm_allreduce_max_dev(M.d_nrm, 1);
-  const double bnorm = read_scalar1(M.d_nrm);
+  const double bnorm = read_scalars_reset(M.d_nrm, 1)[0];
   cc_coarsen_coeffs(M, false, true);
   return bnorm;
 }
@@ -1796,8 +1824,12 @@
   }
   const double bnorm = fast ? bnorm_fast : mf_norm_inf(q.rh, 0, 1);
   const bool fmg = fast ? P.mac_fmg != 0 : q.fmg;
-  if (fmg && bnorm != 0.0 && !single && bnorm < HUGE_VAL) cc_run_cycle(M, cc_fmg_what(q.bc), [&] { cc_fmg(M, q.bc); });
-  if (D0.split) cc_to_split(D0, 1);
+  const bool by_colour = fast && D0.split && !(step_glue_old() & 2);
+  const bool run_fmg = fmg && bnorm != 0.0 && !single && bnorm < HUGE_VAL;
+  if (run_fmg) cc_run_cycle(M, by_colour ? -cc_fmg_what(q.bc) : cc_fmg_what(q.bc), [&] { cc_fmg(M, q.bc, by_colour); });
+  if (by_colour) {
+    if (!(run_fmg && cc_fmg_start(M) >= 0)) for (const CBox &B : D0.boxes) HIPCHK(hipMemsetAsync(B.sp.phi[0], 0, sizeof(double) * 2 * B.sp.tot, ctx().stream));
+  } else if (D0.split) cc_to_split(D0, 1);
   const int gn[3] = { D0.ng[0], D0.ng[1], D0.ng[2] };
   const MgStop s = mg_stop_loop(0, gn, fast && !single && bnorm < HUGE_VAL, fast && !single, q, bnorm, M.d_nrm,
     [&](bool blind) {
@@ -1813,7 +1845,7 @@
         for (int c = 0; c < n; c++) { cc_coarse_correction(M); cc_fine_seq(M, true, true, true, false); norm_hist_push(M.d_nrm); }
       });
     },
-    [&] { return read_scalar1(M.d_nrm); });
+    [&] { return read_scalars_reset(M.d_nrm, 1)[0]; });
   if (s.overshot) { arena_release(mark); return mg_repeat_unpredicted([&] { return cc_solve(q); }); }
   if (D0.split) cc_from_split(D0);
   if (fast) {
diff --git a/varden_amd/csrc/mg_nd.hip b/varden_amd/csrc/mg_nd.hip
--- a/varden_amd/csrc/mg_nd.hip
+++ b/varden_amd/csrc/mg_nd.hip
@@ -1163,8 +1163,10 @@
     M.g_nodes = P.gather((long)(cn[0] + 1) * (cn[1] + 1) * (cn[2] + 1)); M.g_cells = P.gather((long)cn[0] * cn[1] * cn[2]);
     std::vector<GBox> gb = M.g_nodes.gb; gb.insert(gb.end(), M.g_cells.gb.begin(), M.g_cells.gb.end());
     M.d_gb = (GBox *)arena_alloc(2 * nb * sizeof(GBox));
-    HIPCHK(hipMemcpyAsync(M.d_gb, gb.data(), 2 * nb * sizeof(GBox), hipMemcpyHostToDevice, ctx().stream));
-    HIPCHK(hipStreamSynchronize(ctx().stream));
+    if (step_glue_old() & 1) {
+      HIPCHK(hipMemcpyAsync(M.d_gb, gb.data(), 2 * nb * sizeof(GBox), hipMemcpyHostToDevice, ctx().stream));
+      HIPCHK(hipStreamSynchronize(ctx().stream));
+    } else upload_staged(M.d_gb, gb.data(), 2 * nb * sizeof(GBox));
     M.sendbuf = (double *)arena_alloc(sizeof(double) * M.g_nodes.cnt);
     M.recvbuf = (double *)arena_alloc(sizeof(double) * M.g_nodes.cnt * ctx().nranks);
   }
@@ -1232,7 +1234,7 @@
   }
 }
 static void nd_residual_d(NDMG &M, NDLev &DL, bool norm, bool reduce = true) {
-  if (norm) HIPCHK(hipMemsetAsync(M.d_nrm, 0, sizeof(double), ctx().stream));
+  if (norm && !nrm_self_reset()) HIPCHK(hipMemsetAsync(M.d_nrm, 0, sizeof(double), ctx().stream));
   DL.res_restricted = false;
   {
     const size_t l = &DL - &M.dlev[0];
@@ -1623,7 +1625,7 @@
   comm_allreduce_max_dev(M.d_nrm, 2);
   const bool single = (M.dlev.size() == 1 && M.tail.empty());
   double bnorm = 1.0, p0max = 1.0;
-  if (!fixed_cycles) { const double *sc = read_scalars(M.d_nrm, 2); bnorm = sc[0]; p0max = sc[1]; }
+  if (!fixed_cycles) { const double *sc = read_scalars_reset(M.d_nrm, 2); bnorm = sc[0]; p0max = sc[1]; }
   if (P.hg_fmg && bnorm != 0.0 && !single && (fixed_cycles ? q.fmg_start : (p0max == 0.0 && bnorm < HUGE_VAL))) nd_fmg(M);
   auto correct = [&] {
     nd_restrict_down(M, 0);
@@ -1654,7 +1656,7 @@
           for (int c = 0; c < n; c++) { correct(); nd_jacobi_d(M.dlev[0], P.hg_nu1, true); nd_residual_d(M, M.dlev[0], true, false); norm_hist_push(M.d_nrm); }
         });
       },
-      [&] { return read_scalar1(M.d_nrm); });
+      [&] { return read_scalars_reset(M.d_nrm, 1)[0]; });
     if (s.overshot) { arena_release(mark); return mg_repeat_unpredicted([&] { return nd_solve(q); }); }
   }
   NDLev &DF = M.dlev[0];
diff --git a/varden_amd/csrc/mg_stop.h b/varden_amd/csrc/mg_stop.h
--- a/varden_amd/csrc/mg_stop.h
+++ b/varden_amd/csrc/mg_stop.h
@@ -5,7 +5,7 @@
 
 struct MgStop { int cycles = 0; double res = 0.0; bool conv = false, overshot = false; };
 template <class First, class Cycle, class Blind, class Read>
-MgStop mg_stop_loop(int solver, const int gn[3], bool predict, bool remember, const MgRequest &q, double bnorm, const double *d_nrm,
+MgStop mg_stop_loop(int solver, const int gn[3], bool predict, bool remember, const MgRequest &q, double bnorm, double *d_nrm,
                     First first, Cycle cycle, Blind blind, Read read) {
   MgStop s;
   s.conv = (bnorm == 0.0);
diff --git a/varden_amd/csrc/runtime.hip b/varden_amd/csrc/runtime.hip
--- a/varden_amd/csrc/runtime.hip
+++ b/varden_amd/csrc/runtime.hip
@@ -198,19 +198,22 @@
 }
 
 bool g_capturing_now();
-__global__ void k_publish(double *host_view, const double *dev, int n, unsigned long long seq) {
-  if ((int)threadIdx.x < n) host_view[threadIdx.x] = dev[threadIdx.x];
+__global__ void k_publish(double *host_view, double *dev, int n, unsigned long long seq, int reset) {
+  if ((int)threadIdx.x < n) { host_view[threadIdx.x] = dev[threadIdx.x]; if (reset) dev[threadIdx.x] = 0.0; }
   __syncthreads();
   if (threadIdx.x == 0) { __threadfence_system(); *reinterpret_cast<volatile unsigned long long *>(host_view + 64) = seq; }
 }
-const double *read_scalars(const double *dev, int n) {
+static const double *read_scalars_impl(double *dev, int n, int reset);
+const double *read_scalars(const double *dev, int n) { return read_scalars_impl(const_cast<double *>(dev), n, 0); }
+const double *read_scalars_reset(double *dev, int n) { return read_scalars_impl(dev, n, nrm_self_reset() ? 1 : 0); }
+static const double *read_scalars_impl(double *dev, int n, int reset) {
   VdnCtx &c = g_ctx;
   REQUIRE(n >= 1 && n <= 64, "read_scalars: 1..64 values");
   static unsigned long long seq = 0;
   const bool poll = sw().poll >= 0 ? sw().poll != 0 : c.nranks == 1;
   ++seq;
   dbg_sync(8);
-  hipLaunchKernelGGL(k_publish, dim3(1), dim3(64), 0, c.stream, c.h_scal_dev, dev, n, seq);
+  hipLaunchKernelGGL(k_publish, dim3(1), dim3(64), 0, c.stream, c.h_scal_dev, dev, n, seq, reset);
   if (poll && !g_capturing_now()) {
     volatile unsigned long long *flag = reinterpret_cast<volatile unsigned long long *>(c.h_scal + 64);
     for (unsigned long spins = 1;; spins++) {
@@ -228,14 +231,15 @@
   return c.h_scal;
 }
 
-__global__ void k_hist_push(double *hist, const double *nrm) {
+__global__ void k_hist_push(double *hist, double *nrm) {
   int *cnt = reinterpret_cast<int *>(hist + 64);
   const int c = *cnt;
   if (c < 64) hist[c] = *nrm;
+  *nrm = 0.0;
   *cnt = c + 1;
 }
 void norm_hist_reset() { HIPCHK(hipMemsetAsync(g_ctx.d_hist + 64, 0, sizeof(double), g_ctx.stream)); }
-void norm_hist_push(const double *d_nrm) { hipLaunchKernelGGL(k_hist_push, dim3(1), dim3(1), 0, g_ctx.stream, g_ctx.d_hist, d_nrm); }
+void norm_hist_push(double *d_nrm) { hipLaunchKernelGGL(k_hist_push, dim3(1), dim3(1), 0, g_ctx.stream, g_ctx.d_hist, d_nrm); }
 const double *norm_hist_read(int n) {
   REQUIRE(n >= 1 && n <= 64, "norm_hist_read: 1..64 entries");
   comm_allreduce_max_dev(g_ctx.d_hist, n);
@@ -357,6 +361,7 @@
     HIPCHK(hipEventCreateWithFlags(&c.ev_main, hipEventDisableTiming));
     HIPCHK(hipEventCreateWithFlags(&c.ev_halo, hipEventDisableTiming));
   }
+  if (!c.ev_phase[0]) for (hipEvent_t &e : c.ev_phase) HIPCHK(hipEventCreate(&e));
   if (c.stream == 0) c.stream = c.own_stream;
   const bool krylov = (prm->mg_bottom_solver >= 1 && prm->mg_bottom_solver <= 3) || (prm->hg_bottom_solver >= 1 && prm->hg_bottom_solver <= 3);
   if (krylov && !c.d_bstats) HIPCHK(hipMalloc((void **)&c.d_bstats, 10 * sizeof(double)));
@@ -372,6 +377,8 @@
   kept_purge(0);
   arena_destroy(); field_pool_release(); fabio_release();
   graph_cache_clear();
+  c.step_clock_pending = false;
+  for (hipEvent_t &e : c.ev_phase) if (e) { HIPCHK(hipEventDestroy(e)); e = nullptr; }
   if (c.d_hist) { HIPCHK(hipFree(c.d_hist)); c.d_hist = nullptr; }
   if (c.d_bstats) { HIPCHK(hipFree(c.d_bstats)); c.d_bstats = nullptr; }
   if (c.d_scal) { HIPCHK(hipFree(c.d_scal)); c.d_scal = nullptr; HIPCHK(hipHostFree(c.h_scal)); c.h_scal = nullptr; c.h_scal_dev = nullptr; }
@@ -389,7 +396,19 @@
 extern "C" int vdn_device_synchronize(void) { VDN_TRY HIPCHK(hipStreamSynchronize(g_ctx.stream)); VDN_CATCH }
 extern "C" int vdn_get_params(vdn_params *out) { *out = g_ctx.prm; return 0; }
 extern "C" int vdn_set_extruded_2d(int on) { g_ctx.extruded2d = on != 0; return 0; }
-extern "C" int vdn_last_step_timing(double *s) { for (int i = 0; i < 5; i++) s[i] = g_ctx.step_sec[i]; return 0; }
+void step_timing_resolve() {
+  VdnCtx &c = g_ctx;
+  if (!c.step_clock_pending) return;
+  c.step_clock_pending = false;
+  HIPCHK(hipEventSynchronize(c.ev_phase[5]));
+  auto sec = [&](int a, int b) { float ms = 0.0f; HIPCHK(hipEventElapsedTime(&ms, c.ev_phase[a], c.ev_phase[b])); return 1.0e-3 * (double)ms; };
+  c.step_sec[0] = sec(2, 3); c.step_sec[1] = sec(3, 4); c.step_sec[2] = sec(1, 2); c.step_sec[3] = sec(4, 5); c.step_sec[4] = sec(0, 5);
+}
+extern "C" int vdn_last_step_timing(double *s) {
+  try { step_timing_resolve(); } catch (const std::exception &e) { vdn_set_error("%s", e.what()); return 1; }
+  for (int i = 0; i < 5; i++) s[i] = g_ctx.step_sec[i];
+  return 0;
+}
 extern "C" int vdn_last_solver_stats(int w, int *cyc, double *r0, double *r) {
   if (w < 0 || w > 1) return 1;
   *cyc = g_ctx.solver_cycles[w]; *r0 = g_ctx.solver_res0[w]; *r = g_ctx.solver_res[w]; return 0;
diff --git a/varden_amd/csrc/vdn_internal.h b/varden_amd/csrc/vdn_internal.h
--- a/varden_amd/csrc/vdn_internal.h
+++ b/varden_amd/csrc/vdn_internal.h
@@ -80,6 +80,8 @@
   double *d_bstats = nullptr;
   double *d_hist = nullptr;
   double step_sec[5] = {0, 0, 0, 0, 0};
+  hipEvent_t ev_phase[6] = { nullptr, nullptr, nullptr, nullptr, nullptr, nullptr };
+  bool step_clock_pending = false;
   int solver_cycles[2] = {0, 0}; double solver_res0[2] = {0, 0}, solver_res[2] = {0, 0};
   std::vector<double *> slope_cache[3]; std::vector<const double *> slope_src;
   std::vector<double *> macmax_cache; std::vector<const double *> macmax_src;
@@ -107,8 +109,12 @@
 
 const double *read_scalars(const double *dev, int n);
 inline double read_scalar1(const double *dev) { return read_scalars(dev, 1)[0]; }
+inline int step_glue_old() { return (sw().sync_points >> 6) & 7; }
+inline bool nrm_self_reset() { return !(step_glue_old() & 4); }
+const double *read_scalars_reset(double *dev, int n);
+void step_timing_resolve();
 void norm_hist_reset();
-void norm_hist_push(const double *d_nrm);
+void norm_hist_push(double *d_nrm);
 const double *norm_hist_read(int n);
 int  mg_predict_get(int solver, const int n[3]);
 void mg_predict_set(int solver, const int n[3], int cycles);
diff --git a/varden_amd/csrc/vdn_switches.h b/varden_amd/csrc/vdn_switches.h
--- a/varden_amd/csrc/vdn_switches.h
+++ b/varden_amd/csrc/vdn_switches.h
@@ -14,7 +14,7 @@
   X(field_vmm, "VDN_FIELD_VMM", ON, true, "0: every state field is one hipMalloc block (rounds 1-5) instead of pooled chunks mapped into its own address range") \
   X(mlcc_trace, "VDN_MLCC_TRACE", SET, false, "1: the composite cell-centred solve prints its residual at every FAC iteration (stderr)") \
   X(keep_off, "VDN_KEEP_OFF", INT, 0, "mask of kept-descriptor families rebuilt at every call: 1 generic sets, 2 create_umac_grown, 4 composite cell-centred solve, 8 nodal prolongation") \
-  X(sync_points, "VDN_SYNC_POINTS", INT, 0, "mask of points that synchronise the device (race hunting): 1 after every batched launch, 2 after every staged upload, 4 after every exchange, 8 before a scalar read-back, 16 at arena_reset, 32 after launch_cells") \
+  X(sync_points, "VDN_SYNC_POINTS", INT, 0, "mask of points that synchronise the device (race hunting): 1 after every batched launch, 2 after every staged upload, 4 after every exchange, 8 before a scalar read-back, 16 at arena_reset, 32 after launch_cells; and of the step's glue as it was (step_glue_old in vdn_internal.h): 64 a stream drain and the host's clock at every phase boundary of advance_timestep instead of events, and a drain in the set-up of every multigrid solve, 128 macproject's fast path converts phi after the nested iteration (kk_cc_to_split) instead of prolonging into the split arrays, 256 a memset in front of every norm pass of the two multigrids instead of the reader's reset") \
   X(phase_hash, "VDN_PHASE_HASH", SET, false, "1: advance_timestep prints a checksum of its fields at every phase boundary (stderr)") \
   X(no_roctx, "VDN_NO_ROCTX", PRESENT, false, "do not bind the roctx library (no bl_prof ranges)") \
   X(poll, "VDN_POLL", INT, -1, "scalar read-back: 1 spin on the pinned sequence number, 0 hipStreamSynchronize; default: spin on one rank, synchronise on several") \
```

After: 694.7 million cells*steps/s, median of 2. About the same (+0.0%).
